# hbell99/DirectVoxGO

Measured on AMD Instinct MI355X. Metric: train rays/sec (8192-ray batch, 160^3 grid), higher is better.
Workload: dtype f32

## Files before the change

### directvoxgo_amd/_lib.py

```python
import ctypes
import os
import re

import torch

_HERE = os.path.dirname(os.path.abspath(__file__))
SO_PATH = os.environ.get('DVGO_HIP_SO') or os.path.join(_HERE, 'csrc', 'libdvgo_hip.so')
ABI_VERSION = 11
HEADER_PATH = os.path.join(os.path.dirname(_HERE), 'include', 'dvgo_hip.h')

_lib = None
_nargs = {}


class _Rec2(ctypes.Structure):
    _fields_ = [('step', ctypes.c_int32), ('exp_d', ctypes.c_float), ('alpha', ctypes.c_float), ('T', ctypes.c_float)]


_vp = ctypes.c_void_p
_i64 = ctypes.c_int64
_int = ctypes.c_int
_flt = ctypes.c_float


class _Pointer(ctypes.c_void_p):

    @staticmethod
    def from_param(x):
        if x is None or type(x) is _vp:
            return x
        if isinstance(x, torch.Tensor):
            return _vp(x.data_ptr())
        if isinstance(x, (ctypes.Array, _vp)):
            return x
        raise TypeError(f'expected a tensor, a ctypes array, a c_void_p or None, got {type(x).__name__}')


_SCALARS = {'int': ctypes.c_int, 'int32_t': ctypes.c_int32, 'int64_t': ctypes.c_int64, 'float': ctypes.c_float,
            'double': ctypes.c_double}


def declarations(text):
    text = re.sub(r'/\*.*?\*/', ' ', text, flags=re.S)
    text = re.sub(r'^\s*#.*$', ' ', text, flags=re.M)
    text = re.sub(r'typedef\s+struct\s*\{[^{}]*\}\s*\w+\s*;', ' ', text)
    text = re.sub(r'extern\s+"C"\s*\{|^\s*\}\s*$', ' ', text, flags=re.M)
    decls = {}
    for stmt in filter(None, (' '.join(s.split()) for s in text.split(';'))):
        m = re.fullmatch(r'(int|int64_t) (dvgo_\w+) ?\((.*)\)', stmt)
        if m is None or m.group(2) in decls:
            raise RuntimeError(f'dvgo_hip.h: cannot read the declaration `{stmt}`')
        argtypes = []
        for param in ([] if m.group(3).strip() == 'void' else m.group(3).split(',')):
            if re.fullmatch(r'\s*(const )?(unsigned )?\w+ ?\*( ?const ?\*)? ?\w+\s*', param):
                argtypes.append(_Pointer)
                continue
            words = param.split()
            if len(words) != 2 or words[0] not in _SCALARS or not words[1].isidentifier():
                raise RuntimeError(f'dvgo_hip.h: {m.group(2)}: cannot read the parameter `{param.strip()}`')
            argtypes.append(_SCALARS[words[0]])
        decls[m.group(2)] = (_SCALARS[m.group(1)], argtypes)
    return decls


def lib():
    global _lib
    if _lib is None:
        if not os.path.exists(SO_PATH):
            raise RuntimeError(
                f'{SO_PATH} is missing: build it with `python -m directvoxgo_amd.build` '
                '(hipcc --offload-arch=gfx950).  directvoxgo_amd has no CPU fallback.')
        if not os.path.exists(HEADER_PATH):
            raise RuntimeError(f'{HEADER_PATH} is missing: the calls into libdvgo_hip.so are typed from it '
                               '(run from a checkout: include/ beside directvoxgo_amd/)')
        handle = ctypes.CDLL(SO_PATH)
        handle.dvgo_abi_version.restype = ctypes.c_int
        v = handle.dvgo_abi_version()
        if v != ABI_VERSION:
            raise RuntimeError(f'libdvgo_hip.so ABI {v} != expected {ABI_VERSION}: rebuild')
        with open(HEADER_PATH) as f:
            decls = declarations(f.read())
        for name, (restype, argtypes) in decls.items():
            fn = getattr(handle, name, None)
            if fn is None:
                raise RuntimeError(f'{SO_PATH} does not export {name}, which include/dvgo_hip.h declares: rebuild')
            fn.restype, fn.argtypes = restype, argtypes
            _nargs[name] = len(argtypes)
        if os.environ.get('DVGO_SHADE_VARIANT'):
            handle.dvgo_shade_variant(int(os.environ['DVGO_SHADE_VARIANT']))
        _lib = handle
    return _lib


def check_input(x, name):
    if not x.is_cuda:
        raise RuntimeError(f'{name} must be a CUDA tensor')
    if not x.is_contiguous():
        raise RuntimeError(f'{name} must be contiguous')


def check_f32(x, name):
    if x.dtype != torch.float32:
        raise RuntimeError(f'{name} must be float32, got {x.dtype}')


def ptr(t):
    return _vp(t.data_ptr()) if t is not None else _vp(0)


def stream_of(t):
    return _vp(torch._C._cuda_getCurrentRawStream(t.device.index))


class _NoCtx:
    def __enter__(self):
        return self

    def __exit__(self, *exc):
        return False


_NOCTX = _NoCtx()


def device_of(t):
    if t.device.index == torch.cuda.current_device():
        return _NOCTX
    return torch.cuda.device_of(t)


_ERR = {-1: 'invalid argument', -2: 'size exceeds 32-bit launch range'}


_profile = None


def profile_start(names):
    global _profile
    _profile = {n: [] for n in names}


def profile_stop():
    global _profile
    prof, _profile = _profile, None
    torch.cuda.synchronize()
    return {n: (len(ev), sum(a.elapsed_time(b) for a, b in ev)) for n, ev in (prof or {}).items()}


def call(name, *args):
    handle = lib()
    if len(args) != _nargs.get(name):
        raise TypeError(f'{name}: {len(args)} arguments given, include/dvgo_hip.h declares {_nargs.get(name, "no such function")}')
    fn = getattr(handle, name)
    if _profile is not None and name in _profile:
        a, b = torch.cuda.Event(enable_timing=True), torch.cuda.Event(enable_timing=True)
        a.record()
        rc = fn(*args)
        b.record()
        _profile[name].append((a, b))
    else:
        rc = fn(*args)
    if rc != 0:
        raise RuntimeError(f'{name} failed: {_ERR.get(rc, "hipError %d" % rc)}')


def f3(x):
    if isinstance(x, torch.Tensor):
        x = x.detach().cpu().tolist()
    return (ctypes.c_float * 3)(*[float(v) for v in x])
```

### directvoxgo_amd/csrc/loss.hip

```cpp
#include "common.h"

__device__ __forceinline__ float block_sum_256(float v, float* red) {
#pragma unroll
  for (int d = 32; d >= 1; d >>= 1) v += __shfl_xor(v, d);
  const int lane = threadIdx.x & 63, w = threadIdx.x >> 6;
  if (lane == 0) red[w] = v;
  __syncthreads();
  const float t = red[0] + red[1] + red[2] + red[3];
  __syncthreads();
  return t;
}

__global__ void __launch_bounds__(256)
loss_rays_kernel(const float* __restrict__ rgb_marched, const float* __restrict__ alphainv_last,
                 const float* __restrict__ target, int64_t N, float inv_n_global, float w_main, float w_ent,
                 float* __restrict__ g_marched, float* __restrict__ g_last, float* __restrict__ loss_out) {
  __shared__ float red[4];
  const int64_t r = (int64_t)blockIdx.x * blockDim.x + threadIdx.x;
  float l = 0.0f;
  if (r < N) {
    float se = 0.0f;
#pragma unroll
    for (int c = 0; c < 3; ++c) {
      const float d = rgb_marched[3 * r + c] - target[3 * r + c];
      se = fmaf(d, d, se);
      g_marched[3 * r + c] = 2.0f * w_main * d * inv_n_global * (1.0f / 3.0f);
    }
    l = w_main * se * inv_n_global * (1.0f / 3.0f);
    if (w_ent > 0.0f) {
      const float x = alphainv_last[r];
      const float p = fminf(fmaxf(x, 1e-6f), 1.0f - 1e-6f);
      const float lp = logf(p), lq = logf(1.0f - p);
      l += w_ent * (-(p * lp + (1.0f - p) * lq)) * inv_n_global;
      const bool inside = (x >= 1e-6f) && (x <= 1.0f - 1e-6f);
      g_last[r] = inside ? w_ent * (lq - lp) * inv_n_global : 0.0f;
    } else {
      g_last[r] = 0.0f;
    }
  }
  const float t = block_sum_256(l, red);
  if (threadIdx.x == 0) atomicAdd(loss_out, t);
}

__global__ void __launch_bounds__(256)
loss_samples_kernel(const float* __restrict__ raw_rgb, const float* __restrict__ weights,
                    const int64_t* __restrict__ ray_id, const float* __restrict__ target, int64_t M_cap,
                    const int64_t* __restrict__ m_dev,
                    float inv_n_global, float w_per, float* __restrict__ g_raw_rgb, float* __restrict__ loss_out) {
  const int64_t M = m_dev ? (*m_dev < M_cap ? *m_dev : M_cap) : M_cap;
  __shared__ float red[4];
  float l = 0.0f;
  for (int64_t i = (int64_t)blockIdx.x * blockDim.x + threadIdx.x; i < M; i += (int64_t)gridDim.x * blockDim.x) {
    const int64_t r = ray_id[i];
    const float w = weights[i];
    float se = 0.0f;
#pragma unroll
    for (int c = 0; c < 3; ++c) {
      const float d = raw_rgb[3 * i + c] - target[3 * r + c];
      se = fmaf(d, d, se);
      g_raw_rgb[3 * i + c] = 2.0f * w_per * w * d * inv_n_global;
    }
    l += w_per * w * se * inv_n_global;
  }
  const float t = block_sum_256(l, red);
  if (threadIdx.x == 0) atomicAdd(loss_out, t);
}

__global__ void __launch_bounds__(256)
viewdir_embed_kernel(const float* __restrict__ viewdirs, const float* __restrict__ freq, int F, int64_t N,
                     float* __restrict__ emb) {
  const int E = 3 + 6 * F;
  const int64_t t = (int64_t)blockIdx.x * blockDim.x + threadIdx.x;
  if (t >= N * E) return;
  const int64_t r = t / E;
  const int e = (int)(t - r * E);
  float v;
  if (e < 3) v = viewdirs[3 * r + e];
  else {
    const int q = (e - 3) % (3 * F);
    const float a = viewdirs[3 * r + q / F] * freq[q % F];
    v = (e - 3 < 3 * F) ? sinf(a) : cosf(a);
  }
  emb[t] = v;
}

#define DVGO_MT_MAX 16
struct AdamMulti {
  float* p[DVGO_MT_MAX];
  const float* g[DVGO_MT_MAX];
  float* m[DVGO_MT_MAX];
  float* v[DVGO_MT_MAX];
  int64_t start[DVGO_MT_MAX + 1];
  int n;
};
__global__ void __launch_bounds__(256)
adam_multi_kernel(AdamMulti A, float step_size, const float* __restrict__ step_size_dev, float beta1, float beta2, float eps) {
  if (step_size_dev != nullptr) step_size = *step_size_dev;
  const int64_t t = (int64_t)blockIdx.x * blockDim.x + threadIdx.x;
  if (t >= A.start[A.n]) return;
  int k = 0;
  while (k + 1 < A.n && t >= A.start[k + 1]) ++k;
  const int64_t i = t - A.start[k];
  const float g = A.g[k][i];
  const float m = fmaf(beta1, A.m[k][i], (1.0f - beta1) * g);
  const float v = fmaf(beta2, A.v[k][i], ((1.0f - beta2) * g) * g);
  A.m[k][i] = m;
  A.v[k][i] = v;
  A.p[k][i] = A.p[k][i] - (step_size * m) / (sqrtf(v) + eps);
}

struct CopyMulti {
  const uint32_t* src[8];
  uint32_t* dst[8];
  int64_t start[9];
  int n;
};
__global__ void __launch_bounds__(256)
copy_multi_kernel(CopyMulti A) {
  const int64_t t = (int64_t)blockIdx.x * blockDim.x + threadIdx.x;
  if (t >= A.start[A.n]) return;
  int k = 0;
  while (k + 1 < A.n && t >= A.start[k + 1]) ++k;
  const int64_t i = t - A.start[k];
  A.dst[k][i] = A.src[k][i];
}

extern "C" {

int dvgo_copy_multi(void* const* dst, const void* const* src, const int64_t* n_dwords, int n_tensors, void* stream) {
  if (n_tensors < 0 || n_tensors > 8 || (n_tensors > 0 && (!dst || !src || !n_dwords))) return DVGO_EINVAL;
  CopyMulti A;
  A.n = n_tensors;
  int64_t tot = 0;
  for (int k = 0; k < n_tensors; ++k) {
    if (n_dwords[k] < 0 || (n_dwords[k] > 0 && (!dst[k] || !src[k]))) return DVGO_EINVAL;
    A.dst[k] = (uint32_t*)dst[k]; A.src[k] = (const uint32_t*)src[k];
    A.start[k] = tot;
    tot += n_dwords[k];
  }
  for (int k = n_tensors; k <= 8; ++k) A.start[k] = tot;
  if (tot == 0) return 0;
  if (!dvgo_fits(tot)) return DVGO_ERANGE;
  copy_multi_kernel<<<dvgo_blocks(tot, 256), 256, 0, (hipStream_t)stream>>>(A);
  DVGO_LAUNCH_CHECK();
  return 0;
}

int dvgo_loss_fwd_bwd(const float* rgb_marched, const float* alphainv_last, const float* target, int64_t N,
                      const float* raw_rgb, const float* weights, const int64_t* ray_id, int64_t M, const int64_t* m_dev,
                      int64_t n_rays_global, float w_main, float w_ent, float w_per, float* g_marched,
                      float* g_last, float* g_raw_rgb, float* loss_out, void* stream) {
  if (N < 0 || M < 0 || n_rays_global <= 0) return DVGO_EINVAL;
  if (!loss_out) return DVGO_EINVAL;
  hipStream_t s = (hipStream_t)stream;
  DVGO_HIP_TRY(hipMemsetAsync(loss_out, 0, sizeof(float), s));
  const float inv = 1.0f / (float)n_rays_global;
  if (N > 0) {
    if (!rgb_marched || !alphainv_last || !target || !g_marched || !g_last) return DVGO_EINVAL;
    loss_rays_kernel<<<dvgo_blocks(N, 256), 256, 0, s>>>(rgb_marched, alphainv_last, target, N, inv, w_main, w_ent,
                                                         g_marched, g_last, loss_out);
    DVGO_LAUNCH_CHECK();
  }
  if (M > 0 && w_per > 0.0f) {
    if (!raw_rgb || !weights || !ray_id || !g_raw_rgb) return DVGO_EINVAL;
    const int64_t nb = dvgo_blocks(M, 256);
    loss_samples_kernel<<<(int)(nb < 256 ? nb : (M >= (1 << 20) ? 1024 : 256)), 256, 0, s>>>(raw_rgb, weights, ray_id, target, M, m_dev, inv, w_per,
                                                            g_raw_rgb, loss_out);
    DVGO_LAUNCH_CHECK();
  }
  return 0;
}

int dvgo_viewdir_embed(const float* viewdirs, const float* freq, int n_freq, int64_t N, float* emb, void* stream) {
  if (N < 0 || n_freq < 0) return DVGO_EINVAL;
  if (N == 0) return 0;
  if (!viewdirs || !emb || (n_freq > 0 && !freq)) return DVGO_EINVAL;
  const int64_t total = N * (3 + 6 * n_freq);
  if (!dvgo_fits(total)) return DVGO_ERANGE;
  viewdir_embed_kernel<<<dvgo_blocks(total, 256), 256, 0, (hipStream_t)stream>>>(viewdirs, freq, n_freq, N, emb);
  DVGO_LAUNCH_CHECK();
  return 0;
}

int dvgo_adam_upd_multi(float* const* params, const float* const* grads, float* const* exp_avg,
                        float* const* exp_avg_sq, const int64_t* numel, int n_tensors, float step_size, float beta1,
                        float beta2, float eps, const float* step_size_dev, void* stream) {
  if (n_tensors < 0 || n_tensors > DVGO_MT_MAX) return DVGO_EINVAL;
  if (n_tensors == 0) return 0;
  if (!params || !grads || !exp_avg || !exp_avg_sq || !numel) return DVGO_EINVAL;
  AdamMulti A;
  A.n = n_tensors;
  int64_t tot = 0;
  for (int k = 0; k < n_tensors; ++k) {
    if (numel[k] < 0 || (numel[k] > 0 && (!params[k] || !grads[k] || !exp_avg[k] || !exp_avg_sq[k]))) return DVGO_EINVAL;
    A.p[k] = params[k]; A.g[k] = grads[k]; A.m[k] = exp_avg[k]; A.v[k] = exp_avg_sq[k];
    A.start[k] = tot;
    tot += numel[k];
  }
  for (int k = n_tensors; k <= DVGO_MT_MAX; ++k) A.start[k] = tot;
  if (tot == 0) return 0;
  adam_multi_kernel<<<dvgo_blocks(tot, 256), 256, 0, (hipStream_t)stream>>>(A, step_size, step_size_dev, beta1, beta2, eps);
  DVGO_LAUNCH_CHECK();
  return 0;
}

}
```

### directvoxgo_amd/csrc/shade.hip

```cpp
#include "common.h"
#include "x3.h"

#include <type_traits>


static int g_shade_experiment = 0;
static int g_shade_variant = 67;
extern "C" int dvgo_shade_wgrad_x3(const float* G1, const float* gz, const uint64_t* masks, const float* W3, const float* H1,
                                   const float* H2, const float* feat, int C, const float* emb, int E, const int64_t* ray_id,
                                   int64_t M, const int64_t* m_dev, int width, int diffuse, int n_parts, float* part, int form_b,
                                   void* stream);
extern "C" int dvgo_shade_bwd_x3(const float* g_rgb, const float* rgb, const uint64_t* masks, int64_t M, const int64_t* m_dev,
                                 const float* W1, const float* W2, const float* W3, int width, int d_in, int C, int diffuse,
                                 float* g_feat, float* G1, float* gz, void* scratch, int prebuilt, void* stream);

extern "C" int dvgo_shade_fwd_x3(const float* feat, int C, const float* emb, int E, const int64_t* ray_id, int64_t M, const int64_t* m_dev,
                                 const float* W1, const float* b1, const float* W2, const float* b2, const float* W3,
                                 const float* b3, int width, int d_in, int diffuse, float* rgb, float* H1, float* H2,
                                 uint64_t* masks, void* scratch, void* scratch_bwd, int experiment, void* stream);

#define SHADE_THREADS 768
#define SHADE_WAVES (SHADE_THREADS / 64)
#define SHADE_BWD_THREADS 1024
#define SHADE_BWD_WAVES (SHADE_BWD_THREADS / 64)

template <int WIDTH, int S1>
struct ShadeLds {
  static constexpr int T = WIDTH / 32;
  float w1a[T][S1][64];
  float w2a[T][T][16][64];
  float w3p[3][2][T * 16];
  float b1p[2][T * 16];
  float b2p[2][T * 16];
  float b3[4];
};

__device__ __forceinline__ int acc_feature(int t, int r, int h) { return 32 * t + (r & 3) + 8 * (r >> 2) + 4 * h; }

#define SHADE_STAGE_STRIDE 36
__device__ __forceinline__ void shade_store_tile(float* __restrict__ stage ,
                                                 const f32x16& acc, float* __restrict__ dst , int row_stride, int lane, int rows_valid) {
  const int smp = lane & 31, h = lane >> 5;
#pragma unroll
  for (int q = 0; q < 4; ++q)
    *reinterpret_cast<float4*>(stage + smp * SHADE_STAGE_STRIDE + 8 * q + 4 * h) =
        make_float4(acc[4 * q], acc[4 * q + 1], acc[4 * q + 2], acc[4 * q + 3]);
  const int c = lane & 7;
#pragma unroll
  for (int i = 0; i < 4; ++i) {
    const int r = (lane >> 3) + 8 * i;
    const float4 v = *reinterpret_cast<const float4*>(stage + r * SHADE_STAGE_STRIDE + 4 * c);
    if (r < rows_valid) *reinterpret_cast<float4*>(dst + (int64_t)r * row_stride + 4 * c) = v;
  }
}

template <int WIDTH, int S1>
__device__ __forceinline__ void shade_load_weights(ShadeLds<WIDTH, S1>& L, const float* __restrict__ W1,
                                                   const float* __restrict__ b1, const float* __restrict__ W2,
                                                   const float* __restrict__ b2, const float* __restrict__ W3,
                                                   const float* __restrict__ b3, int D_in) {
  constexpr int T = WIDTH / 32;
  const int tid = threadIdx.x, nt = blockDim.x;
  for (int i = tid; i < T * S1 * 64; i += nt) {
    const int l = i & 63, s = (i >> 6) % S1, t = (i >> 6) / S1;
    const int k = 2 * s + (l >> 5);
    (&L.w1a[0][0][0])[i] = (k < D_in) ? W1[(32 * t + (l & 31)) * D_in + k] : 0.0f;
  }
  for (int i = tid; i < T * T * 16 * 64; i += nt) {
    const int l = i & 63, r = (i >> 6) & 15, t = (i >> 10) % T, t2 = (i >> 10) / T;
    (&L.w2a[0][0][0][0])[i] = W2[(32 * t2 + (l & 31)) * WIDTH + acc_feature(t, r, l >> 5)];
  }
  for (int i = tid; i < 3 * 2 * T * 16; i += nt) {
    const int tr = i % (T * 16), h = (i / (T * 16)) & 1, c = i / (2 * T * 16);
    (&L.w3p[0][0][0])[i] = W3[c * WIDTH + acc_feature(tr >> 4, tr & 15, h)];
  }
  for (int i = tid; i < 2 * T * 16; i += nt) {
    const int tr = i % (T * 16), h = i / (T * 16);
    const int f = acc_feature(tr >> 4, tr & 15, h);
    (&L.b1p[0][0])[i] = b1[f];
    (&L.b2p[0][0])[i] = b2[f];
  }
  if (tid < 3) L.b3[tid] = b3[tid];
}

template <int WIDTH, int S1>
__device__ __forceinline__ void shade_tile_forward(const ShadeLds<WIDTH, S1>& L, const float (&x)[S1], int lane,
                                                   f32x16 (&acc1)[WIDTH / 32], float (&z)[3],
                                                   float* __restrict__ H2tile ,
                                                   float* __restrict__ stage, int rows_valid,
                                                   unsigned long long& mask2 ) {
  constexpr int T = WIDTH / 32;
  const int h = lane >> 5;
#pragma unroll
  for (int t = 0; t < T; ++t) {
#pragma unroll
    for (int r = 0; r < 16; ++r) acc1[t][r] = L.b1p[h][t * 16 + r];
#pragma unroll
    for (int s = 0; s < S1; ++s) acc1[t] = __builtin_amdgcn_mfma_f32_32x32x2f32(L.w1a[t][s][lane], x[s], acc1[t], 0, 0, 0);
#pragma unroll
    for (int r = 0; r < 16; ++r) acc1[t][r] = dvgo_relu(acc1[t][r]);
    __builtin_amdgcn_sched_barrier(0);
  }
  float p[3] = {0.0f, 0.0f, 0.0f};
  mask2 = 0ull;
#pragma unroll 1
  for (int t2 = 0; t2 < T; ++t2) {
    f32x16 acc2;
#pragma unroll
    for (int r = 0; r < 16; ++r) acc2[r] = L.b2p[h][t2 * 16 + r];
#pragma unroll
    for (int t = 0; t < T; ++t) {
#pragma unroll
      for (int r = 0; r < 16; ++r)
        acc2 = __builtin_amdgcn_mfma_f32_32x32x2f32(L.w2a[t2][t][r][lane], acc1[t][r], acc2, 0, 0, 0);
      __builtin_amdgcn_sched_barrier(0);
    }
#pragma unroll
    for (int r = 0; r < 16; ++r) acc2[r] = dvgo_relu(acc2[r]);
    if (H2tile != nullptr) {
      unsigned int bits = 0u;
#pragma unroll
      for (int r = 0; r < 16; ++r) bits |= dvgo_relu_bit(acc2[r]) << r;
      mask2 |= (unsigned long long)bits << (16 * t2);
      shade_store_tile(stage, acc2, H2tile + 32 * t2, WIDTH, lane, rows_valid);
    }
#pragma unroll
    for (int c = 0; c < 3; ++c) {
#pragma unroll
      for (int r = 0; r < 16; ++r) p[c] = fmaf(L.w3p[c][h][t2 * 16 + r], acc2[r], p[c]);
    }
  }
#pragma unroll
  for (int c = 0; c < 3; ++c) z[c] = p[c] + __shfl_xor(p[c], 32) + L.b3[c];
}

template <int S1>
__device__ __forceinline__ void shade_load_x(const float* __restrict__ feat, int C, int c_view0, int n_view,
                                             const float* __restrict__ emb, int E, int64_t row, int64_t ray,
                                             int lane, float (&x)[S1]) {
  const int h = lane >> 5;
  const float* fr = feat + row * C + c_view0;
  const float* er = emb + ray * E - n_view;
#pragma unroll
  for (int s = 0; s < S1; ++s) {
    const int k = 2 * s + h;
    float v = 0.0f;
    if (k < n_view) v = fr[k];
    else if (k < n_view + E) v = er[k];
    x[s] = v;
  }
}

template <int WIDTH, int S1, bool DIFFUSE>
__global__ void __launch_bounds__(SHADE_THREADS)
shade_fwd_kernel(const float* __restrict__ feat, int C, int c_view0, int n_view, const float* __restrict__ emb, int E,
                 const int64_t* __restrict__ ray_id, int64_t M_cap, const int64_t* __restrict__ m_dev, const float* __restrict__ W1,
                 const float* __restrict__ b1, const float* __restrict__ W2, const float* __restrict__ b2,
                 const float* __restrict__ W3, const float* __restrict__ b3, int D_in, float* __restrict__ rgb,
                 float* __restrict__ H1, float* __restrict__ H2, unsigned long long* __restrict__ masks, int experiment) {
  const int64_t M = m_dev ? (*m_dev < M_cap ? *m_dev : M_cap) : M_cap;
  constexpr int T = WIDTH / 32;
  __shared__ ShadeLds<WIDTH, S1> L;
  __shared__ __attribute__((aligned(16))) float s_stage[SHADE_WAVES][32 * SHADE_STAGE_STRIDE];
  shade_load_weights<WIDTH, S1>(L, W1, b1, W2, b2, W3, b3, D_in);
  __syncthreads();
  const int lane = threadIdx.x & 63, h = lane >> 5;
  float* stage = s_stage[threadIdx.x >> 6];
  const int64_t n_tiles = (M + 31) / 32;
  const int64_t gw = (int64_t)blockIdx.x * (blockDim.x >> 6) + (threadIdx.x >> 6);
  const int64_t nw = (int64_t)gridDim.x * (blockDim.x >> 6);
  for (int64_t tile = gw; tile < n_tiles; tile += nw) {
    const int64_t row = tile * 32 + (lane & 31);
    const bool valid = row < M;
    const int64_t rowc = valid ? row : (M - 1);
    float x[S1];
    if (experiment & 16) { for (int s = 0; s < S1; ++s) x[s] = 0.01f * (float)(lane + s); }
    else shade_load_x<S1>(feat, C, c_view0, n_view, emb, E, rowc, ray_id[rowc], lane, x);
    f32x16 acc1[T];
    float z[3];
    const int rows_valid = (int)(M - tile * 32 < 32 ? M - tile * 32 : 32);
    unsigned long long mask2;
    shade_tile_forward<WIDTH, S1>(L, x, lane, acc1, z, (H1 != nullptr && !(experiment & 32)) ? (H2 + tile * 32 * WIDTH) : nullptr,
                                  stage, rows_valid, mask2);
    if (valid) {
      if (h == 0) {
#pragma unroll
        for (int c = 0; c < 3; ++c) {
          const float zz = DIFFUSE ? z[c] + feat[row * C + c] : z[c];
          rgb[row * 3 + c] = 1.0f / (1.0f + expf(-zz));
        }
      }
      if (H1 != nullptr) {
        unsigned long long mask1 = 0ull;
#pragma unroll
        for (int t = 0; t < T; ++t) {
#pragma unroll
          for (int r = 0; r < 16; ++r) mask1 |= (unsigned long long)dvgo_relu_bit(acc1[t][r]) << (16 * t + r);
        }
        masks[(row * 2 + 0) * 2 + h] = mask1;
        masks[(row * 2 + 1) * 2 + h] = mask2;
      }
    }
    if (H1 != nullptr && !(experiment & 32)) {
#pragma unroll
      for (int t = 0; t < T; ++t) shade_store_tile(stage, acc1[t], H1 + tile * 32 * WIDTH + 32 * t, WIDTH, lane, rows_valid);
    }
  }
}

template <int WIDTH>
struct ShadeBwdLds {
  static constexpr int T = WIDTH / 32;
  float w2ta[T][T][16][64];
  float w1ta[T][16][64];
  float w3p[3][2][T * 16];
};

template <int WIDTH, bool DIFFUSE>
__global__ void __launch_bounds__(SHADE_BWD_THREADS)
shade_bwd_kernel(const float* __restrict__ g_rgb, const float* __restrict__ rgb,
                 const unsigned long long* __restrict__ masks, int64_t M_cap, const int64_t* __restrict__ m_dev,
                 const float* __restrict__ W1, const float* __restrict__ W2,
                 const float* __restrict__ W3, int D_in, int C, int c_view0, int n_view,
                 float* __restrict__ g_feat, float* __restrict__ G1, float* __restrict__ gz_out, int experiment) {
  const int64_t M = m_dev ? (*m_dev < M_cap ? *m_dev : M_cap) : M_cap;
  constexpr int T = WIDTH / 32;
  __shared__ ShadeBwdLds<WIDTH> L;
  __shared__ __attribute__((aligned(16))) float s_stage[SHADE_BWD_WAVES][32 * SHADE_STAGE_STRIDE];
  float* stage = s_stage[threadIdx.x >> 6];
  {
    const int tid = threadIdx.x, nt = blockDim.x;
    for (int i = tid; i < T * T * 16 * 64; i += nt) {
      const int l = i & 63, r = (i >> 6) & 15, t2 = (i >> 10) % T, tin = (i >> 10) / T;
      (&L.w2ta[0][0][0][0])[i] = W2[acc_feature(t2, r, l >> 5) * WIDTH + 32 * tin + (l & 31)];
    }
    for (int i = tid; i < T * 16 * 64; i += nt) {
      const int l = i & 63, r = (i >> 6) & 15, t = i >> 10;
      const int k = l & 31;
      (&L.w1ta[0][0][0])[i] = (k < D_in) ? W1[acc_feature(t, r, l >> 5) * D_in + k] : 0.0f;
    }
    for (int i = tid; i < 3 * 2 * T * 16; i += nt) {
      const int tr = i % (T * 16), h = (i / (T * 16)) & 1, c = i / (2 * T * 16);
      (&L.w3p[0][0][0])[i] = W3[c * WIDTH + acc_feature(tr >> 4, tr & 15, h)];
    }
  }
  __syncthreads();
  const int lane = threadIdx.x & 63, h = lane >> 5;
  const int64_t n_tiles = (M + 31) / 32;
  const int64_t gw = (int64_t)blockIdx.x * (blockDim.x >> 6) + (threadIdx.x >> 6);
  const int64_t nw = (int64_t)gridDim.x * (blockDim.x >> 6);
  for (int64_t tile = gw; tile < n_tiles; tile += nw) {
    const int64_t row = tile * 32 + (lane & 31);
    const bool valid = row < M;
    const int64_t rowc = valid ? row : (M - 1);
    float gz[3];
#pragma unroll
    for (int c = 0; c < 3; ++c) {
      const float o = rgb[rowc * 3 + c];
      gz[c] = valid ? g_rgb[rowc * 3 + c] * o * (1.0f - o) : 0.0f;
    }
    if (valid && h == 0) {
#pragma unroll
      for (int c = 0; c < 3; ++c) {
        gz_out[row * 3 + c] = gz[c];
        if (DIFFUSE) g_feat[row * C + c] = gz[c];
      }
    }
    const unsigned long long m1 = masks[(rowc * 2 + 0) * 2 + h];
    const unsigned long long m2 = masks[(rowc * 2 + 1) * 2 + h];
    f32x16 g2[T];
#pragma unroll
    for (int t2 = 0; t2 < T; ++t2) {
#pragma unroll
      for (int r = 0; r < 16; ++r) {
        const float v = fmaf(L.w3p[2][h][t2 * 16 + r], gz[2],
                             fmaf(L.w3p[1][h][t2 * 16 + r], gz[1], L.w3p[0][h][t2 * 16 + r] * gz[0]));
        g2[t2][r] = ((m2 >> (16 * t2 + r)) & 1ull) ? v : 0.0f;
      }
    }
    f32x16 gx;
#pragma unroll
    for (int r = 0; r < 16; ++r) gx[r] = 0.0f;
#pragma unroll 1
    for (int tin = 0; tin < T; ++tin) {
      f32x16 acc;
#pragma unroll
      for (int r = 0; r < 16; ++r) acc[r] = 0.0f;
#pragma unroll
      for (int t2 = 0; t2 < T; ++t2) {
#pragma unroll
        for (int r = 0; r < 16; ++r)
          acc = __builtin_amdgcn_mfma_f32_32x32x2f32(L.w2ta[tin][t2][r][lane], g2[t2][r], acc, 0, 0, 0);
        __builtin_amdgcn_sched_barrier(0);
      }
#pragma unroll
      for (int q = 0; q < 4; ++q) {
        const unsigned int mb = (unsigned int)(m1 >> (16 * tin + 4 * q)) & 15u;
        acc[4 * q + 0] = (mb & 1u) ? acc[4 * q + 0] : 0.0f;
        acc[4 * q + 1] = (mb & 2u) ? acc[4 * q + 1] : 0.0f;
        acc[4 * q + 2] = (mb & 4u) ? acc[4 * q + 2] : 0.0f;
        acc[4 * q + 3] = (mb & 8u) ? acc[4 * q + 3] : 0.0f;
      }
      if (!(experiment & 1))
        shade_store_tile(stage, acc, G1 + tile * 32 * WIDTH + 32 * tin, WIDTH, lane,
                         (int)(M - tile * 32 < 32 ? M - tile * 32 : 32));
#pragma unroll
      for (int r = 0; r < 16; ++r)
        gx = __builtin_amdgcn_mfma_f32_32x32x2f32(L.w1ta[tin][r][lane], acc[r], gx, 0, 0, 0);
    }
    if (valid) {
#pragma unroll
      for (int r = 0; r < 16; ++r) {
        const int k = (r & 3) + 8 * (r >> 2) + 4 * h;
        if (k < n_view) g_feat[row * C + c_view0 + k] = gx[r];
      }
    }
  }
}

template <int WIDTH>
struct ShadeWgradLds {
  float g1[1][32][WIDTH], h1[1][32][WIDTH], h2[1][32][WIDTH];
// ... 440 lines not shown
}
template <int OFF> __device__ __forceinline__ void lds_store_u32x4(unsigned a, u32x4 v) {
  asm volatile("ds_write_b128 %0, %1 offset:%2" :: "v"(a), "v"(v), "n"(OFF) : "memory");
}

template <int WIDTH>
struct ShadeWgradRingX3 : ShadeWgradRing<WIDTH> {
  u32x4 fb[WIDTH / 32 + 2][3][64];
};

template <int WIDTH>
__global__ void __launch_bounds__(2 * WIDTH, 2)
shade_wgrad_ring_x3_kernel(const float* __restrict__ G1, const float* __restrict__ gz, const unsigned int* __restrict__ masks,
                           const float* __restrict__ W3, const float* __restrict__ H1, const float* __restrict__ H2,
                           const float* __restrict__ feat, int C, int c_view0, int n_view, const float* __restrict__ emb, int E,
                           const int64_t* __restrict__ ray_id, int64_t M_cap, const int64_t* __restrict__ m_dev,
                           float* __restrict__ part, float* __restrict__ total, int total_size) {
#if defined(__HIP_DEVICE_COMPILE__)
  for (int i = blockIdx.x * blockDim.x + threadIdx.x; i < total_size; i += gridDim.x * blockDim.x) total[i] = 0.0f;
  int64_t M;
  {
    const int64_t m = m_dev ? (*m_dev < M_cap ? *m_dev : M_cap) : M_cap;
    M = ((int64_t)__builtin_amdgcn_readfirstlane((int)(m >> 32)) << 32) | (unsigned)__builtin_amdgcn_readfirstlane((int)m);
  }
  using Ring = ShadeWgradRingX3<WIDTH>;
  constexpr int T = WIDTH / 32, NW = T, NB = Ring::NB, NR = Ring::NR, TR = Ring::TR;
  static_assert(T == 4 || T == 2, "widths 128 and 64");
  constexpr int LPR = WIDTH / 4, RPI = 64 / LPR, IPW = TR / RPI / NW;
  constexpr int DW = NW == 4 ? 2 : NW, FPW = 4 / DW, EPW = 8 / DW;
  static_assert(IPW == 2 && NB == 2 && TR == 16, "double buffer of 16-row tiles: the wait at the top of a tile is vmcnt(0)");
  __shared__ __attribute__((aligned(16))) Ring L;
  const int tid = threadIdx.x, lane = tid & 63, h = lane >> 5, j = lane & 31;
  const int w = __builtin_amdgcn_readfirstlane(tid >> 6);
  const int dw = NW == 4 ? w - 2 : w;
  f32x16 aW2[T], aW1[2];
  float vW3[3] = {0.0f, 0.0f, 0.0f}, sgz[3] = {0.0f, 0.0f, 0.0f};
#pragma unroll
  for (int t = 0; t < T; ++t)
#pragma unroll
    for (int r = 0; r < 16; ++r) aW2[t][r] = 0.0f;
#pragma unroll
  for (int q = 0; q < 2; ++q)
#pragma unroll
    for (int r = 0; r < 16; ++r) aW1[q][r] = 0.0f;
  float sb1 = 0.0f, sb2 = 0.0f;
  const float w30 = W3[32 * w + j], w31 = W3[WIDTH + 32 * w + j], w32 = W3[2 * WIDTH + 32 * w + j];
  const int m_idx = 2 * ((j >> 2) & 1) + (w >> 1);
  const unsigned m_bit = 16 * (w & 1) + (j & 3) + 4 * (j >> 3);
  const int d_in = n_view + E;
  const int n_tiles = (int)((M + TR - 1) / TR);
  auto tile_of = [&](int k) { return (int)blockIdx.x + k * (int)gridDim.x; };
  const unsigned rows_b = (unsigned)(M * WIDTH * 4);
  const auto bG1 = __builtin_amdgcn_make_buffer_rsrc((void*)G1, 0, rows_b, 0x00020000);
  const auto bH1 = __builtin_amdgcn_make_buffer_rsrc((void*)H1, 0, rows_b, 0x00020000);
  const auto bH2 = __builtin_amdgcn_make_buffer_rsrc((void*)H2, 0, rows_b, 0x00020000);
  const auto bF = __builtin_amdgcn_make_buffer_rsrc((void*)feat, 0, (unsigned)(M * C * 4), 0x00020000);
  const auto bE = __builtin_amdgcn_make_buffer_rsrc((void*)emb, 0, DVGO_OOB, 0x00020000);
  const auto bGz = __builtin_amdgcn_make_buffer_rsrc((void*)gz, 0, (unsigned)(M * 12), 0x00020000);
  const auto bM = __builtin_amdgcn_make_buffer_rsrc((void*)masks, 0, (unsigned)(M * 32), 0x00020000);
  const auto bR = __builtin_amdgcn_make_buffer_rsrc((void*)ray_id, 0, (unsigned)(M * 8), 0x00020000);
  unsigned vo_bulk[IPW], vo_f[FPW], vo_ecol[EPW];
  int e_row[EPW];
#pragma unroll
  for (int i = 0; i < IPW; ++i) vo_bulk[i] = (unsigned)(((IPW * w + i) * RPI + lane / LPR) * WIDTH * 4 + 16 * (lane % LPR));
#pragma unroll
  for (int i = 0; i < FPW; ++i) {
    const int e = 64 * ((dw < 0 ? 0 : dw) + DW * i) + lane, row = e >> 4, col = e & 15;
    vo_f[i] = col < n_view ? (unsigned)((row * C + c_view0 + col) * 4) : DVGO_OOB;
  }
#pragma unroll
  for (int i = 0; i < EPW; ++i) {
    const int e = 64 * ((dw < 0 ? 0 : dw) + DW * i) + lane, col = e & 31;
    e_row[i] = e >> 5;
    vo_ecol[i] = col < E ? (unsigned)(col * 4) : DVGO_OOB;
  }
  const unsigned vo_gz = (lane & 3) < 3 ? (unsigned)(((lane >> 2) * 3 + (lane & 3)) * 4) : DVGO_OOB;
  const unsigned vo_m2 = (unsigned)(((lane >> 2) * 8 + 4 + (lane & 3)) * 4);
  const unsigned vo_rid = (unsigned)((lane & (TR - 1)) * 8);
  auto issue = [&](int t) {
    const int sl = t & (NB - 1);
    const unsigned r0 = (unsigned)__builtin_amdgcn_readfirstlane(tile_of(t) * TR);
#pragma unroll
    for (int i = 0; i < IPW; ++i) {
      const int rl = (IPW * w + i) * RPI;
      __builtin_amdgcn_raw_ptr_buffer_load_lds(bG1, (dvgo_lptr_t)&L.g1[sl][rl][0], 16, vo_bulk[i], r0 * (WIDTH * 4), 0, 0);
      __builtin_amdgcn_raw_ptr_buffer_load_lds(bH1, (dvgo_lptr_t)&L.h1[sl][rl][0], 16, vo_bulk[i], r0 * (WIDTH * 4), 0, 0);
      __builtin_amdgcn_raw_ptr_buffer_load_lds(bH2, (dvgo_lptr_t)&L.h2[sl][rl][0], 16, vo_bulk[i], r0 * (WIDTH * 4), 0, 0);
    }
    if (dw < 0) return;
#pragma unroll
    for (int i = 0; i < FPW; ++i)
      __builtin_amdgcn_raw_ptr_buffer_load_lds(bF, (dvgo_lptr_t)(&L.xf[sl][0][0] + 64 * (dw + DW * i)), 4, vo_f[i], r0 * (unsigned)(C * 4), 0, 0);
    unsigned rids[EPW];
#pragma unroll
    for (int i = 0; i < EPW; ++i) rids[i] = lds_u32<0>(lds_addr(&L.rid[t & (NR - 1)][e_row[i]]));
    asm volatile("s_waitcnt lgkmcnt(0)" : "+v"(rids[0]), "+v"(rids[1]), "+v"(rids[2]), "+v"(rids[3]));
#pragma unroll
    for (int i = 0; i < EPW; ++i)
      __builtin_amdgcn_raw_ptr_buffer_load_lds(bE, (dvgo_lptr_t)(&L.xe[sl][0][0] + 64 * (dw + DW * i)), 4,
                                               vo_ecol[i] + rids[i] * (unsigned)(E * 4), 0, 0, 0);
    const unsigned rn = (unsigned)__builtin_amdgcn_readfirstlane(tile_of(t + 2) * TR);
    const int rsl = (t + 2) & (NR - 1);
    auto small = [&](int which) {
      if (which == 0) __builtin_amdgcn_raw_ptr_buffer_load_lds(bGz, (dvgo_lptr_t)&L.gz[sl][0][0], 4, vo_gz, r0 * 12u, 0, 0);
      else if (which == 1) __builtin_amdgcn_raw_ptr_buffer_load_lds(bM, (dvgo_lptr_t)&L.m2[sl][0][0], 4, vo_m2, r0 * 32u, 0, 0);
      else __builtin_amdgcn_raw_ptr_buffer_load_lds(bR, (dvgo_lptr_t)&L.rid[rsl][0], 4, vo_rid, rn * 8u, 0, 0);
    };
    if (dw == 0) { small(0); small(1); } else small(2);
  };
  const unsigned a_gz = lds_addr(&L.gz[0][8 * h][0]), a_mw = lds_addr(&L.m2[0][8 * h][m_idx]);
  const unsigned a_g1 = lds_addr(&L.g1[0][8 * h][32 * w + j]), a_h1 = lds_addr(&L.h1[0][8 * h][32 * w + j]);
  const unsigned a_h2 = lds_addr(&L.h2[0][8 * h][32 * w + j]);
  const int xcol = 32 * (w & 1) + j;
  const bool x_in_f = xcol < n_view, x_ok = xcol < d_in;
  const unsigned a_x = x_in_f ? lds_addr(&L.xf[0][8 * h][xcol]) : lds_addr(&L.xe[0][8 * h][x_ok ? xcol - n_view : 0]);
  const unsigned a_fb = lds_addr(&L.fb[0][0][lane]);
  constexpr unsigned SLOT_ROWS = TR * WIDTH * 4, FB_TILE = 3 * 64 * 16, FB_PIECE = 64 * 16;
  if (tid < 64) {
#pragma unroll
    for (int t = 0; t < 2; ++t) {
      const int64_t row = (int64_t)tile_of(t) * TR + (tid & (TR - 1));
      L.rid[t][tid] = row < M ? (unsigned int)ray_id[row] : 0u;
    }
  }
  __syncthreads();
#pragma unroll
  for (int t = 0; t < NB - 1; ++t) issue(t);
  for (int k = 0; tile_of(k) < n_tiles; ++k) {
    const int sl = k & (NB - 1);
    asm volatile("s_waitcnt vmcnt(0)\n\ts_waitcnt lgkmcnt(0)\n\ts_barrier" ::: "memory");
    issue(k + NB - 1);
    const unsigned b_gz = a_gz + sl * (TR * 16), b_mw = a_mw + sl * (TR * 16), b_g1 = a_g1 + sl * SLOT_ROWS;
    const unsigned b_h1 = a_h1 + sl * SLOT_ROWS, b_h2 = a_h2 + sl * SLOT_ROWS;
    const unsigned b_x = a_x + sl * (x_in_f ? (unsigned)(TR * 16 * 4) : (unsigned)(TR * 32 * 4));
    dvgo_f32x4 gq[8];
    unsigned mw[8];
    float g1v[8], h1v[8], h2v[8], xv[8];
    constexpr int RS = WIDTH * 4 / 256;
    static_for<0, 4>([&](auto Ec) {
      constexpr int e = 2 * decltype(Ec)::value;
      const dvgo_f32x2 v = lds_f32_pair_st64<e * RS, (e + 1) * RS>(b_h1);
      h1v[e] = v.x; h1v[e + 1] = v.y;
    });
    if (w < 2) {
      if (x_in_f) static_for<0, 8>([&](auto Ec) { constexpr int e = decltype(Ec)::value; xv[e] = lds_f32<e * 16 * 4>(b_x); });
      else static_for<0, 8>([&](auto Ec) { constexpr int e = decltype(Ec)::value; xv[e] = lds_f32<e * 32 * 4>(b_x); });
    }
    static_for<0, 8>([&](auto Ec) {
      constexpr int e = decltype(Ec)::value;
      gq[e] = lds_f32x4<16 * e>(b_gz);
    });
    static_for<0, 4>([&](auto Ec) {
      constexpr int e = 2 * decltype(Ec)::value;
      const dvgo_f32x2 m = lds_f32_pair<4 * e, 4 * (e + 1)>(b_mw);
      mw[e] = __float_as_uint(m.x); mw[e + 1] = __float_as_uint(m.y);
      const dvgo_f32x2 a = lds_f32_pair_st64<e * RS, (e + 1) * RS>(b_g1);
      g1v[e] = a.x; g1v[e + 1] = a.y;
      const dvgo_f32x2 b = lds_f32_pair_st64<e * RS, (e + 1) * RS>(b_h2);
      h2v[e] = b.x; h2v[e + 1] = b.y;
    });
    asm volatile("s_waitcnt lgkmcnt(0)" : "+v"(h1v[0]), "+v"(h1v[1]), "+v"(h1v[2]), "+v"(h1v[3]), "+v"(h1v[4]), "+v"(h1v[5]),
                 "+v"(h1v[6]), "+v"(h1v[7]), "+v"(gq[0]), "+v"(gq[1]), "+v"(gq[2]), "+v"(gq[3]), "+v"(gq[4]), "+v"(gq[5]), "+v"(gq[6]),
                 "+v"(gq[7]));
    asm volatile("" : "+v"(mw[0]), "+v"(mw[1]), "+v"(mw[2]), "+v"(mw[3]), "+v"(mw[4]), "+v"(mw[5]), "+v"(mw[6]), "+v"(mw[7]),
                 "+v"(g1v[0]), "+v"(g1v[1]), "+v"(g1v[2]), "+v"(g1v[3]), "+v"(g1v[4]), "+v"(g1v[5]), "+v"(g1v[6]), "+v"(g1v[7]));
    asm volatile("" : "+v"(h2v[0]), "+v"(h2v[1]), "+v"(h2v[2]), "+v"(h2v[3]), "+v"(h2v[4]), "+v"(h2v[5]), "+v"(h2v[6]), "+v"(h2v[7]));
    {
      u32x4 p0, p1, p2;
      x3_split8(h1v, p0, p1, p2);
      lds_store_u32x4<0>(a_fb + w * FB_TILE, p0);
      lds_store_u32x4<FB_PIECE>(a_fb + w * FB_TILE, p1);
      lds_store_u32x4<2 * FB_PIECE>(a_fb + w * FB_TILE, p2);
      if (w < 2) {
        asm volatile("" : "+v"(xv[0]), "+v"(xv[1]), "+v"(xv[2]), "+v"(xv[3]), "+v"(xv[4]), "+v"(xv[5]), "+v"(xv[6]), "+v"(xv[7]));
#pragma unroll
        for (int e = 0; e < 8; ++e) xv[e] = x_ok ? xv[e] : 0.0f;
        x3_split8(xv, p0, p1, p2);
        lds_store_u32x4<0>(a_fb + (T + w) * FB_TILE, p0);
        lds_store_u32x4<FB_PIECE>(a_fb + (T + w) * FB_TILE, p1);
        lds_store_u32x4<2 * FB_PIECE>(a_fb + (T + w) * FB_TILE, p2);
      }
    }
    u32x4 a2f[3], a1f[3];
    {
      float a2[8];
#pragma unroll
      for (int e = 0; e < 8; ++e) {
        const float g2v = fmaf(w32, gq[e].z, fmaf(w31, gq[e].y, w30 * gq[e].x));
        a2[e] = __uint_as_float(__float_as_uint(g2v) & (unsigned)__builtin_amdgcn_sbfe((int)mw[e], m_bit, 1u));
        sb2 += a2[e]; sb1 += g1v[e];
        vW3[0] = fmaf(gq[e].x, h2v[e], vW3[0]); vW3[1] = fmaf(gq[e].y, h2v[e], vW3[1]); vW3[2] = fmaf(gq[e].z, h2v[e], vW3[2]);
      }
      if (w == 0) {
#pragma unroll
        for (int e = 0; e < 8; ++e) { sgz[0] += gq[e].x; sgz[1] += gq[e].y; sgz[2] += gq[e].z; }
      }
      x3_split8(a2, a2f[0], a2f[1], a2f[2]);
      x3_split8(g1v, a1f[0], a1f[1], a1f[2]);
    }
    asm volatile("s_waitcnt lgkmcnt(0)\n\ts_barrier" ::: "memory");
    u32x4 fr[2][2][3];
    auto read_pair = [&](auto Pc, u32x4 (&f)[2][3]) {
      constexpr int p = decltype(Pc)::value;
#pragma unroll
      for (int q = 0; q < 3; ++q) {
        f[0][q] = lds_u32x4<(2 * p) * FB_TILE>(a_fb + q * FB_PIECE);
        f[1][q] = lds_u32x4<(2 * p + 1) * FB_TILE>(a_fb + q * FB_PIECE);
      }
    };
    auto wait_pair = [&](u32x4 (&f)[2][3]) {
      asm volatile("s_waitcnt lgkmcnt(0)" : "+v"(f[0][0]), "+v"(f[0][1]), "+v"(f[0][2]), "+v"(f[1][0]), "+v"(f[1][1]), "+v"(f[1][2]));
    };
    auto mfma_pair = [&](f32x16& accA, f32x16& accB, const u32x4 (&a)[3], const u32x4 (&f)[2][3]) {
#define X3D_MF(ACC, A, B) ACC = __builtin_amdgcn_mfma_f32_32x32x16_bf16(__builtin_bit_cast(bf16x8, A), __builtin_bit_cast(bf16x8, B), ACC, 0, 0, 0)
      X3D_MF(accA, a[2], f[0][0]); X3D_MF(accB, a[2], f[1][0]);
      X3D_MF(accA, a[1], f[0][1]); X3D_MF(accB, a[1], f[1][1]);
      X3D_MF(accA, a[0], f[0][2]); X3D_MF(accB, a[0], f[1][2]);
      X3D_MF(accA, a[1], f[0][0]); X3D_MF(accB, a[1], f[1][0]);
      X3D_MF(accA, a[0], f[0][1]); X3D_MF(accB, a[0], f[1][1]);
      X3D_MF(accA, a[0], f[0][0]); X3D_MF(accB, a[0], f[1][0]);
#undef X3D_MF
    };
    constexpr int NP = T / 2 + 1;
    read_pair(std::integral_constant<int, 0>{}, fr[0]);
    static_for<0, NP>([&](auto Pc) {
      constexpr int p = decltype(Pc)::value;
      wait_pair(fr[p & 1]);
      if constexpr (p + 1 < NP) read_pair(std::integral_constant<int, p + 1>{}, fr[(p + 1) & 1]);
      if constexpr (p < T / 2) mfma_pair(aW2[2 * p], aW2[2 * p + 1], a2f, fr[p & 1]);
      else mfma_pair(aW1[0], aW1[1], a1f, fr[p & 1]);
      __builtin_amdgcn_sched_barrier(0);
    });
  }
  asm volatile("s_waitcnt vmcnt(0)" ::: "memory");
  float* p = part + (int64_t)blockIdx.x * (WIDTH * WIDTH + WIDTH * 64 + 32 * WIDTH + 3 * WIDTH);
  float* pW2 = p;
  float* pW1 = pW2 + WIDTH * WIDTH;
  float* pW3 = pW1 + WIDTH * 64;
  float* pb = pW3 + 32 * WIDTH;
#pragma unroll
  for (int r = 0; r < 16; ++r) {
    const int i = (r & 3) + 8 * (r >> 2) + 4 * h;
#pragma unroll
    for (int t = 0; t < T; ++t) pW2[(32 * w + i) * WIDTH + 32 * t + j] = aW2[t][r];
    pW1[(32 * w + i) * 64 + j] = aW1[0][r];
    pW1[(32 * w + i) * 64 + 32 + j] = aW1[1][r];
  }
#pragma unroll
  for (int c = 0; c < 3; ++c) {
    const float v = vW3[c] + __shfl_xor(vW3[c], 32);
    if (h == 0) pW3[c * WIDTH + 32 * w + j] = v;
    sgz[c] += __shfl_xor(sgz[c], 32);
  }
  sb1 += __shfl_xor(sb1, 32); sb2 += __shfl_xor(sb2, 32);
  if (h == 0) {
    pb[32 * w + j] = sb1;
    pb[WIDTH + 32 * w + j] = sb2;
    if (j < 8) pb[2 * WIDTH + 8 * w + j] = (w == 0 && j < 3) ? sgz[j] : 0.0f;
    if (T == 2 && j >= 16) pb[2 * WIDTH + 16 * w + j] = 0.0f;
  }
#endif
}
#undef DVGO_OOB

#define SHADE_REDUCE_SLICES 16
__global__ void __launch_bounds__(256)
shade_wgrad_reduce_kernel(const float* __restrict__ part, int n_parts, int n, int W, int d_in, float* __restrict__ out) {
  const int i = blockIdx.x * blockDim.x + threadIdx.x;
  if (i >= n) return;
  int o;
  const int nW2 = W * W, nW1 = W * 64, nW3 = 32 * W;
  if (i < nW2) o = i;
  else if (i < nW2 + nW1) {
    const int r = (i - nW2) >> 6, c = (i - nW2) & 63;
    o = c < d_in ? nW2 + r * d_in + c : -1;
  } else if (i < nW2 + nW1 + nW3) {
    const int e = i - nW2 - nW1;
    o = e < 3 * W ? nW2 + W * d_in + e : -1;
  } else {
    const int e = i - nW2 - nW1 - nW3, base = nW2 + W * d_in + 3 * W;
    if (e < 2 * W) o = base + e;
    else {
      const int c = e - 2 * W;
      o = c < 3 ? base + 2 * W + c : (c >= 8 && c < 11) ? base + 2 * W + c - 8 : -1;
    }
  }
  if (o < 0) return;
  const int per = (n_parts + SHADE_REDUCE_SLICES - 1) / SHADE_REDUCE_SLICES;
  const int p0 = blockIdx.y * per, p1 = min(n_parts, p0 + per);
  float a0 = 0.0f, a1 = 0.0f, a2 = 0.0f, a3 = 0.0f;
  int p = p0;
  for (; p + 4 <= p1; p += 4) {
    a0 += part[(int64_t)p * n + i];
    a1 += part[(int64_t)(p + 1) * n + i];
    a2 += part[(int64_t)(p + 2) * n + i];
    a3 += part[(int64_t)(p + 3) * n + i];
  }
  for (; p < p1; ++p) a0 += part[(int64_t)p * n + i];
  if (p1 > p0) atomicAdd(out + o, (a0 + a1) + (a2 + a3));
}

extern "C" {

int dvgo_shade_fwd(const float* feat, int C, const float* emb, int E, const int64_t* ray_id, int64_t M, const int64_t* m_dev,
                   const float* W1, const float* b1, const float* W2, const float* b2, const float* W3,
                   const float* b3, int width, int d_in, int diffuse, float* rgb, float* H1, float* H2,
                   uint64_t* masks, void* scratch, void* scratch_bwd, void* stream) {
  if (M < 0 || C <= 0 || E < 0) return DVGO_EINVAL;
  if (M == 0) return 0;
  if (!feat || !emb || !ray_id || !W1 || !b1 || !W2 || !b2 || !W3 || !b3 || !rgb) return DVGO_EINVAL;
  if ((H1 == nullptr) != (H2 == nullptr) || (H1 == nullptr) != (masks == nullptr)) return DVGO_EINVAL;
  const int c_view0 = diffuse ? 3 : 0;
  const int n_view = C - c_view0;
  if (n_view < 0 || d_in != n_view + E) return DVGO_EINVAL;
  if ((width != 128 && width != 64) || d_in > 40) return DVGO_ERANGE;
  if ((g_shade_variant & 1) && scratch != nullptr)
    return dvgo_shade_fwd_x3(feat, C, emb, E, ray_id, M, m_dev, W1, b1, W2, b2, W3, b3, width, d_in, diffuse, rgb, H1, H2, masks,
                             scratch, (g_shade_variant & 2) ? scratch_bwd : nullptr, g_shade_experiment, stream);
  hipStream_t s = (hipStream_t)stream;
  const int64_t n_tiles = (M + 31) / 32;
  const int64_t cap = width == 128 ? 256 : 512;
  int blocks = (int)((n_tiles + SHADE_WAVES - 1) / SHADE_WAVES < cap ? (n_tiles + SHADE_WAVES - 1) / SHADE_WAVES : cap);
#define DVGO_SHADE(W, S1, DIFF)                                                                           \
  shade_fwd_kernel<W, S1, DIFF><<<blocks, SHADE_THREADS, 0, s>>>(feat, C, c_view0, n_view, emb, E, ray_id, M, m_dev, W1, b1, W2, \
                                                          b2, W3, b3, d_in, rgb, H1, H2, (unsigned long long*)masks, g_shade_experiment)
  if (width == 128) {
    if (d_in <= 36) { if (diffuse) DVGO_SHADE(128, 18, true); else DVGO_SHADE(128, 18, false); }
    else            { if (diffuse) DVGO_SHADE(128, 20, true); else DVGO_SHADE(128, 20, false); }
  } else {
    if (d_in <= 12) { if (diffuse) DVGO_SHADE(64, 6, true); else DVGO_SHADE(64, 6, false); }
    else            { if (diffuse) DVGO_SHADE(64, 20, true); else DVGO_SHADE(64, 20, false); }
  }
#undef DVGO_SHADE
  DVGO_LAUNCH_CHECK();
  return 0;
}

int dvgo_shade_experiment(int flags) { g_shade_experiment = flags; return 0; }

int dvgo_shade_variant(int flags) { const int old = g_shade_variant; if (flags >= 0) g_shade_variant = flags; return old; }

int dvgo_shade_bwd(const float* g_rgb, const float* rgb, const uint64_t* masks, int64_t M, const int64_t* m_dev,
                   const float* W1, const float* W2, const float* W3, int width, int d_in, int C, int diffuse,
                   float* g_feat, float* G1, float* gz, void* scratch, int prebuilt, void* stream) {
  if (M < 0 || C <= 0) return DVGO_EINVAL;
  if (M == 0) return 0;
  if (!g_rgb || !rgb || !masks || !W1 || !W2 || !W3 || !g_feat || !G1 || !gz) return DVGO_EINVAL;
  const int c_view0 = diffuse ? 3 : 0;
  const int n_view = C - c_view0;
  if ((width != 128 && width != 64) || n_view < 0 || n_view > 32 || d_in < n_view) return DVGO_ERANGE;
  if ((g_shade_variant & 2) && scratch != nullptr)
    return dvgo_shade_bwd_x3(g_rgb, rgb, masks, M, m_dev, W1, W2, W3, width, d_in, C, diffuse, g_feat, G1, gz, scratch, prebuilt, stream);
  hipStream_t s = (hipStream_t)stream;
  const int64_t n_tiles = (M + 31) / 32;
  const int64_t cap = width == 128 ? 256 : 512;
  int blocks = (int)((n_tiles + SHADE_BWD_WAVES - 1) / SHADE_BWD_WAVES < cap ? (n_tiles + SHADE_BWD_WAVES - 1) / SHADE_BWD_WAVES : cap);
#define DVGO_SHADE_BWD(W, DIFF)                                                                                                       \
  shade_bwd_kernel<W, DIFF><<<blocks, SHADE_BWD_THREADS, 0, s>>>(g_rgb, rgb, (const unsigned long long*)masks, M, m_dev, W1, W2, W3, d_in, C, c_view0, \
                                                            n_view, g_feat, G1, gz, g_shade_experiment)
  if (width == 128) { if (diffuse) DVGO_SHADE_BWD(128, true); else DVGO_SHADE_BWD(128, false); }
  else              { if (diffuse) DVGO_SHADE_BWD(64, true); else DVGO_SHADE_BWD(64, false); }
#undef DVGO_SHADE_BWD
  DVGO_LAUNCH_CHECK();
  return 0;
}

int dvgo_shade_wgrad(const float* G1, const float* gz, const uint64_t* masks, const float* W3, const float* H1,
                     const float* H2, const float* feat, int C, const float* emb, int E, const int64_t* ray_id, int64_t M,
                     const int64_t* m_dev, int width, int diffuse, int n_parts, float* part, float* total, void* stream) {
  if (M < 0 || n_parts <= 0 || C <= 0 || E < 0) return DVGO_EINVAL;
  if (!G1 || !gz || !masks || !W3 || !H1 || !H2 || !feat || !emb || !ray_id || !part || !total) return DVGO_EINVAL;
  const int c_view0 = diffuse ? 3 : 0;
  const int n_view = C - c_view0;
  if ((width != 128 && width != 64) || n_view < 0 || n_view + E > 40) return DVGO_ERANGE;
  bool ring = false;
  if (g_shade_variant & (4 | 32)) {
    const int form_b = (g_shade_variant & 32) ? 2 : (g_shade_variant & 16) ? 1 : 0;
    if (!form_b && n_parts > 256) n_parts = 256;
    const int rc = dvgo_shade_wgrad_x3(G1, gz, masks, W3, H1, H2, feat, C, emb, E, ray_id, M, m_dev, width, diffuse, n_parts, part,
                                       form_b, stream);
    if (rc != 0) return rc;
  } else if (!(g_shade_variant & 8) && n_view <= 16 && E <= 32 && (n_view + E <= 32 || (n_view % 4 == 0 && n_view >= 8)) &&
             M * width * 4 < ((int64_t)1 << 31) && M * C * 4 < ((int64_t)1 << 31)) {
    if (n_parts > 512) n_parts = 512;
    ring = true;
    const int tsz = width * width + width * (n_view + E) + 5 * width + 3;
    if ((g_shade_variant & 64) && width == 128)
      shade_wgrad_ring_x3_kernel<128><<<n_parts, 256, 0, (hipStream_t)stream>>>(
          G1, gz, (const unsigned int*)masks, W3, H1, H2, feat, C, c_view0, n_view, emb, E, ray_id, M, m_dev, part, total, tsz);
    else if (g_shade_variant & 64)
      shade_wgrad_ring_x3_kernel<64><<<n_parts, 128, 0, (hipStream_t)stream>>>(
          G1, gz, (const unsigned int*)masks, W3, H1, H2, feat, C, c_view0, n_view, emb, E, ray_id, M, m_dev, part, total, tsz);
    else if (width == 128)
      shade_wgrad_ring_kernel<128><<<n_parts, 256, 0, (hipStream_t)stream>>>(
          G1, gz, (const unsigned int*)masks, W3, H1, H2, feat, C, c_view0, n_view, emb, E, ray_id, M, m_dev, part, total, tsz);
    else
      shade_wgrad_ring_kernel<64><<<n_parts, 128, 0, (hipStream_t)stream>>>(
          G1, gz, (const unsigned int*)masks, W3, H1, H2, feat, C, c_view0, n_view, emb, E, ray_id, M, m_dev, part, total, tsz);
  } else if (width == 128)
    shade_wgrad_kernel<128><<<n_parts, 256, 0, (hipStream_t)stream>>>(
        G1, gz, (const unsigned int*)masks, W3, H1, H2, feat, C, c_view0, n_view, emb, E, ray_id, M, m_dev, part);
  else
    shade_wgrad_kernel<64><<<n_parts, 128, 0, (hipStream_t)stream>>>(
        G1, gz, (const unsigned int*)masks, W3, H1, H2, feat, C, c_view0, n_view, emb, E, ray_id, M, m_dev, part);
  DVGO_LAUNCH_CHECK();
  const int psize = width * width + width * 64 + 32 * width + 3 * width;
  const int d_in = n_view + E;
  const int tsize = width * width + width * d_in + 3 * width + 2 * width + 3;
  if (!ring && hipMemsetAsync(total, 0, (size_t)tsize * sizeof(float), (hipStream_t)stream) != hipSuccess) return DVGO_EINVAL;
  shade_wgrad_reduce_kernel<<<dim3((psize + 255) / 256, SHADE_REDUCE_SLICES), 256, 0, (hipStream_t)stream>>>(part, n_parts, psize,
                                                                                                       width, d_in, total);
  DVGO_LAUNCH_CHECK();
  return 0;
}

}
```

### directvoxgo_amd/csrc/shade_x3.hip

```cpp
#include "common.h"
#include "x3.h"

#ifndef X3_THREADS
#define X3_THREADS 512
#endif
#define X3_WAVES (X3_THREADS / 64)
#ifndef X3_BWD_THREADS
#define X3_BWD_THREADS 512
#endif
#define X3_BWD_WAVES (X3_BWD_THREADS / 64)
#define X3_STAGE_ROWS 16
#define X3_STAGE_STRIDE 36

__device__ __forceinline__ int x3_acc_feature(int t, int r, int h) { return 32 * t + (r & 3) + 8 * (r >> 2) + 4 * h; }

__device__ __forceinline__ void x3_split1(float v, unsigned short& s0, unsigned short& s1, unsigned short& s2) {
  const unsigned int h = x3_pack(v, 0.f) & 0xffffu;
  const float r = v - __uint_as_float(h << 16);
  const unsigned int m = x3_pack(r, 0.f) & 0xffffu;
  const float q = r - __uint_as_float(m << 16);
  s0 = (unsigned short)h; s1 = (unsigned short)m; s2 = (unsigned short)(x3_pack(q, 0.f) & 0xffffu);
}

template <int WIDTH, int KS1>
struct X3Img {
  static constexpr int T = WIDTH / 32;
  u32x4 w1s[T][KS1][3][64];
  u32x4 w2s[T][2 * T][3][64];
  float w3p[3][2][T * 16];
  float b1p[2][T * 16];
  float b2p[2][T * 16];
  float b3[4];
};

template <int WIDTH, int KS1>
struct X3Lds : X3Img<WIDTH, KS1> {
  float stage[X3_WAVES][X3_STAGE_ROWS * X3_STAGE_STRIDE];
};

template <typename Img>
__device__ __forceinline__ void x3_copy_image(Img* __restrict__ dst , const void* __restrict__ src) {
  static_assert(sizeof(Img) % 16 == 0, "16-byte pieces");
  const u32x4* g = reinterpret_cast<const u32x4*>(src);
  u32x4* l = reinterpret_cast<u32x4*>(dst);
  for (int i = threadIdx.x; i < (int)(sizeof(Img) / 16); i += blockDim.x) l[i] = g[i];
}

__device__ __forceinline__ void x3_store_tile(float* __restrict__ stage, const f32x16& acc, float* __restrict__ dst, int row_stride,
                                              int lane, int rows_valid) {
  const int smp = lane & 31, h = lane >> 5;
#pragma unroll
  for (int half = 0; half < 2; ++half) {
    if ((smp >> 4) == half) {
#pragma unroll
      for (int q = 0; q < 4; ++q)
        *reinterpret_cast<float4*>(stage + (smp & 15) * X3_STAGE_STRIDE + 8 * q + 4 * h) =
            make_float4(acc[4 * q], acc[4 * q + 1], acc[4 * q + 2], acc[4 * q + 3]);
    }
    const int c = lane & 7;
#pragma unroll
    for (int i = 0; i < 2; ++i) {
      const int rl = (lane >> 3) + 8 * i;
      const float4 v = *reinterpret_cast<const float4*>(stage + rl * X3_STAGE_STRIDE + 4 * c);
      const int r = 16 * half + rl;
      if (r < rows_valid) *reinterpret_cast<float4*>(dst + (int64_t)r * row_stride + 4 * c) = v;
    }
  }
}

template <int WIDTH, int KS1>
__device__ __forceinline__ void
x3_prep_fwd_body(X3Img<WIDTH, KS1>* __restrict__ Lp, const float* __restrict__ W1, const float* __restrict__ b1,
                 const float* __restrict__ W2, const float* __restrict__ b2, const float* __restrict__ W3,
                 const float* __restrict__ b3, int D_in, const int tid, const int nt) {
  constexpr int T = WIDTH / 32;
  X3Img<WIDTH, KS1>& L = *Lp;
  for (int i = tid; i < T * KS1 * 64 * 8; i += nt) {
    const int j = i & 7, l = (i >> 3) & 63, s = (i >> 9) % KS1, t = (i >> 9) / KS1;
    const int k = 16 * s + 8 * (l >> 5) + j;
    const float v = (k < D_in) ? W1[(32 * t + (l & 31)) * D_in + k] : 0.0f;
    unsigned short p0, p1, p2;
    x3_split1(v, p0, p1, p2);
    reinterpret_cast<unsigned short*>(&L.w1s[t][s][0][l])[j] = p0;
    reinterpret_cast<unsigned short*>(&L.w1s[t][s][1][l])[j] = p1;
    reinterpret_cast<unsigned short*>(&L.w1s[t][s][2][l])[j] = p2;
  }
  for (int i = tid; i < T * 2 * T * 64 * 8; i += nt) {
    const int j = i & 7, l = (i >> 3) & 63, ks = (i >> 9) % (2 * T), t2 = (i >> 9) / (2 * T);
    const int k = 16 * ks + 8 * (j >> 2) + 4 * (l >> 5) + (j & 3);
    const float v = W2[(32 * t2 + (l & 31)) * WIDTH + k];
    unsigned short p0, p1, p2;
    x3_split1(v, p0, p1, p2);
    reinterpret_cast<unsigned short*>(&L.w2s[t2][ks][0][l])[j] = p0;
    reinterpret_cast<unsigned short*>(&L.w2s[t2][ks][1][l])[j] = p1;
    reinterpret_cast<unsigned short*>(&L.w2s[t2][ks][2][l])[j] = p2;
  }
  for (int i = tid; i < 3 * 2 * T * 16; i += nt) {
    const int tr = i % (T * 16), h = (i / (T * 16)) & 1, c = i / (2 * T * 16);
    (&L.w3p[0][0][0])[i] = W3[c * WIDTH + x3_acc_feature(tr >> 4, tr & 15, h)];
  }
  for (int i = tid; i < 2 * T * 16; i += nt) {
    const int tr = i % (T * 16), h = i / (T * 16);
    const int f = x3_acc_feature(tr >> 4, tr & 15, h);
    (&L.b1p[0][0])[i] = b1[f];
    (&L.b2p[0][0])[i] = b2[f];
  }
  if (tid < 4) L.b3[tid] = tid < 3 ? b3[tid] : 0.0f;
}

template <int WIDTH, int KS1, bool DIFFUSE>
__global__ void __launch_bounds__(X3_THREADS)
shade_fwd_x3_kernel(const float* __restrict__ feat, int C, int c_view0, int n_view, const float* __restrict__ emb, int E,
                    const int64_t* __restrict__ ray_id, int64_t M_cap, const int64_t* __restrict__ m_dev,
                    const void* __restrict__ image, float* __restrict__ rgb,
                    float* __restrict__ H1, float* __restrict__ H2, unsigned long long* __restrict__ masks, int experiment) {
  const int64_t M = m_dev ? (*m_dev < M_cap ? *m_dev : M_cap) : M_cap;
  constexpr int T = WIDTH / 32;
  __shared__ __attribute__((aligned(16))) X3Lds<WIDTH, KS1> L;
  x3_copy_image<X3Img<WIDTH, KS1>>(&L, image);
  __syncthreads();
  const int lane = threadIdx.x & 63, h = lane >> 5;
  float* stage = L.stage[threadIdx.x >> 6];
  const bool train = H1 != nullptr;
  const int64_t n_tiles = (M + 31) / 32;
  const int64_t gw = (int64_t)blockIdx.x * (blockDim.x >> 6) + (threadIdx.x >> 6);
  const int64_t nw = (int64_t)gridDim.x * (blockDim.x >> 6);
  const int d_in = n_view + E;
  const int64_t last = M > 0 ? M - 1 : 0;
  auto row_of = [&](int64_t tile) { const int64_t r = tile * 32 + (lane & 31); return r < M ? r : last; };
  float xin[KS1][8];
  auto load_inputs = [&](int64_t tile, int64_t rid) {
    const float* fr = feat + row_of(tile) * C + c_view0;
    const float* er = emb + rid * E - n_view;
#pragma unroll
    for (int s = 0; s < KS1; ++s)
#pragma unroll
      for (int j = 0; j < 8; ++j) {
        const int k = 16 * s + 8 * h + j;
        const int kc = k < d_in ? k : d_in - 1;
        xin[s][j] = *((kc < n_view) ? fr + kc : er + kc);
      }
  };
  int64_t rid_n = 0;
  if (gw < n_tiles) { load_inputs(gw, ray_id[row_of(gw)]); rid_n = ray_id[row_of(gw + nw)]; }
  for (int64_t tile = gw; tile < n_tiles; tile += nw) {
    const int64_t row = tile * 32 + (lane & 31);
    const bool valid = row < M;
    const int rows_valid = (int)(M - tile * 32 < 32 ? M - tile * 32 : 32);
    u32x4 x3[KS1][3];
#pragma unroll
    for (int s = 0; s < KS1; ++s) {
      float v[8];
#pragma unroll
      for (int j = 0; j < 8; ++j) v[j] = (16 * s + 8 * h + j) < d_in ? xin[s][j] : 0.0f;
      x3_split8(v, x3[s][0], x3[s][1], x3[s][2]);
    }
    load_inputs(tile + nw, rid_n);
    rid_n = ray_id[row_of(tile + 2 * nw)];
    u32x4 h3[2 * T][3];
    unsigned long long mask1 = 0ull;
#pragma unroll
    for (int t = 0; t < T; ++t) {
      f32x16 acc;
#pragma unroll
      for (int r = 0; r < 16; ++r) acc[r] = L.b1p[h][t * 16 + r];
#pragma unroll
      for (int s = 0; s < KS1; ++s)
        x3_mfma6(acc, L.w1s[t][s][0][lane], L.w1s[t][s][1][lane], L.w1s[t][s][2][lane], x3[s][0], x3[s][1], x3[s][2]);
#pragma unroll
      for (int r = 0; r < 16; ++r) acc[r] = dvgo_relu(acc[r]);
      if (train) {
        unsigned int bits = 0u;
#pragma unroll
        for (int r = 0; r < 16; ++r) bits |= dvgo_relu_bit(acc[r]) << r;
        mask1 |= (unsigned long long)bits << (16 * t);
        if (!(experiment & 512)) x3_store_tile(stage, acc, H1 + tile * 32 * WIDTH + 32 * t, WIDTH, lane, rows_valid);
      }
#pragma unroll
      for (int s2 = 0; s2 < 2; ++s2) {
        float v[8];
#pragma unroll
        for (int j = 0; j < 8; ++j) v[j] = acc[8 * s2 + j];
        x3_split8(v, h3[2 * t + s2][0], h3[2 * t + s2][1], h3[2 * t + s2][2]);
      }
      __builtin_amdgcn_sched_barrier(0);
    }
    float p[3] = {0.0f, 0.0f, 0.0f};
    unsigned long long mask2 = 0ull;
#pragma unroll 1
    for (int t2 = 0; t2 < T; ++t2) {
      f32x16 acc2;
#pragma unroll
      for (int r = 0; r < 16; ++r) acc2[r] = L.b2p[h][t2 * 16 + r];
      u32x4 a[2][3];
#pragma unroll
      for (int q = 0; q < 3; ++q) a[0][q] = L.w2s[t2][0][q][lane];
#pragma unroll
      for (int ks = 0; ks < 2 * T; ++ks) {
        if (ks + 1 < 2 * T) {
#pragma unroll
          for (int q = 0; q < 3; ++q) a[(ks + 1) & 1][q] = L.w2s[t2][ks + 1][q][lane];
        }
        x3_mfma6(acc2, a[ks & 1][0], a[ks & 1][1], a[ks & 1][2], h3[ks][0], h3[ks][1], h3[ks][2]);
        __builtin_amdgcn_sched_barrier(0);
      }
#pragma unroll
      for (int r = 0; r < 16; ++r) acc2[r] = dvgo_relu(acc2[r]);
      if (train) {
        unsigned int bits = 0u;
#pragma unroll
        for (int r = 0; r < 16; ++r) bits |= dvgo_relu_bit(acc2[r]) << r;
        mask2 |= (unsigned long long)bits << (16 * t2);
        if (!(experiment & 512)) x3_store_tile(stage, acc2, H2 + tile * 32 * WIDTH + 32 * t2, WIDTH, lane, rows_valid);
      }
#pragma unroll
      for (int c = 0; c < 3; ++c) {
#pragma unroll
        for (int r = 0; r < 16; ++r) p[c] = fmaf(L.w3p[c][h][t2 * 16 + r], acc2[r], p[c]);
      }
    }
    float z[3];
#pragma unroll
    for (int c = 0; c < 3; ++c) z[c] = p[c] + __shfl_xor(p[c], 32) + L.b3[c];
    if (valid) {
      if (h == 0) {
#pragma unroll
        for (int c = 0; c < 3; ++c) {
          const float zz = DIFFUSE ? z[c] + feat[row * C + c] : z[c];
          rgb[row * 3 + c] = 1.0f / (1.0f + expf(-zz));
        }
      }
      if (train) {
        masks[(row * 2 + 0) * 2 + h] = mask1;
        masks[(row * 2 + 1) * 2 + h] = mask2;
      }
    }
  }
}

template <int WIDTH>
struct X3BwdImg {
  static constexpr int T = WIDTH / 32;
  u32x4 w2t[T][2 * T][3][64];
  u32x4 w1t[2 * T][3][64];
  float w3p[3][2][T * 16];
};

template <int WIDTH>
struct X3BwdLds : X3BwdImg<WIDTH> {
  float stage[X3_BWD_WAVES][X3_STAGE_ROWS * X3_STAGE_STRIDE];
};

template <int WIDTH>
__device__ __forceinline__ void
x3_prep_bwd_body(X3BwdImg<WIDTH>* __restrict__ Lp, const float* __restrict__ W1, const float* __restrict__ W2,
                 const float* __restrict__ W3, int D_in, const int tid, const int nt) {
  constexpr int T = WIDTH / 32;
  X3BwdImg<WIDTH>& L = *Lp;
  for (int i = tid; i < T * 2 * T * 64 * 8; i += nt) {
    const int j = i & 7, l = (i >> 3) & 63, ks = (i >> 9) % (2 * T), tin = (i >> 9) / (2 * T);
    const int f_out = 16 * ks + 8 * (j >> 2) + 4 * (l >> 5) + (j & 3);
    unsigned short p0, p1, p2;
    x3_split1(W2[f_out * WIDTH + 32 * tin + (l & 31)], p0, p1, p2);
    reinterpret_cast<unsigned short*>(&L.w2t[tin][ks][0][l])[j] = p0;
    reinterpret_cast<unsigned short*>(&L.w2t[tin][ks][1][l])[j] = p1;
    reinterpret_cast<unsigned short*>(&L.w2t[tin][ks][2][l])[j] = p2;
  }
  for (int i = tid; i < 2 * T * 64 * 8; i += nt) {
    const int j = i & 7, l = (i >> 3) & 63, ks = i >> 9;
    const int f = 16 * ks + 8 * (j >> 2) + 4 * (l >> 5) + (j & 3), k = l & 31;
    unsigned short p0, p1, p2;
    x3_split1((k < D_in) ? W1[f * D_in + k] : 0.0f, p0, p1, p2);
    reinterpret_cast<unsigned short*>(&L.w1t[ks][0][l])[j] = p0;
    reinterpret_cast<unsigned short*>(&L.w1t[ks][1][l])[j] = p1;
    reinterpret_cast<unsigned short*>(&L.w1t[ks][2][l])[j] = p2;
  }
  for (int i = tid; i < 3 * 2 * T * 16; i += nt) {
    const int tr = i % (T * 16), h = (i / (T * 16)) & 1, c = i / (2 * T * 16);
    (&L.w3p[0][0][0])[i] = W3[c * WIDTH + x3_acc_feature(tr >> 4, tr & 15, h)];
  }
}

template <int WIDTH, int KS1>
__global__ void __launch_bounds__(256)
x3_prep_fwd_kernel(X3Img<WIDTH, KS1>* __restrict__ Lp, X3BwdImg<WIDTH>* __restrict__ Lb, const float* __restrict__ W1,
                   const float* __restrict__ b1, const float* __restrict__ W2, const float* __restrict__ b2,
                   const float* __restrict__ W3, const float* __restrict__ b3, int D_in) {
  if (blockIdx.x < 32) x3_prep_fwd_body<WIDTH, KS1>(Lp, W1, b1, W2, b2, W3, b3, D_in, blockIdx.x * blockDim.x + threadIdx.x, 32 * blockDim.x);
  else x3_prep_bwd_body<WIDTH>(Lb, W1, W2, W3, D_in, (blockIdx.x - 32) * blockDim.x + threadIdx.x, 32 * blockDim.x);
}

template <int WIDTH>
__global__ void __launch_bounds__(256)
x3_prep_bwd_kernel(X3BwdImg<WIDTH>* __restrict__ Lp, const float* __restrict__ W1, const float* __restrict__ W2,
                   const float* __restrict__ W3, int D_in) {
  x3_prep_bwd_body<WIDTH>(Lp, W1, W2, W3, D_in, blockIdx.x * blockDim.x + threadIdx.x, gridDim.x * blockDim.x);
}

template <int WIDTH, bool DIFFUSE>
__global__ void __launch_bounds__(X3_BWD_THREADS)
shade_bwd_x3_kernel(const float* __restrict__ g_rgb, const float* __restrict__ rgb,
                    const unsigned long long* __restrict__ masks, int64_t M_cap, const int64_t* __restrict__ m_dev,
                    const void* __restrict__ image, int C, int c_view0,
                    int n_view, float* __restrict__ g_feat, float* __restrict__ G1, float* __restrict__ gz_out) {
  const int64_t M = m_dev ? (*m_dev < M_cap ? *m_dev : M_cap) : M_cap;
  constexpr int T = WIDTH / 32;
  __shared__ __attribute__((aligned(16))) X3BwdLds<WIDTH> L;
  x3_copy_image<X3BwdImg<WIDTH>>(&L, image);
  __syncthreads();
  const int lane = threadIdx.x & 63, h = lane >> 5;
  float* stage = L.stage[threadIdx.x >> 6];
  const int64_t n_tiles = (M + 31) / 32;
  const int64_t gw = (int64_t)blockIdx.x * (blockDim.x >> 6) + (threadIdx.x >> 6);
  const int64_t nw = (int64_t)gridDim.x * (blockDim.x >> 6);
  const int64_t last = M > 0 ? M - 1 : 0;
  float o_n[3], g_n[3];
  unsigned long long m1_n = 0ull, m2_n = 0ull;
  auto load_rows = [&](int64_t tile) {
    const int64_t r = tile * 32 + (lane & 31);
    const int64_t rc = r < M ? r : last;
#pragma unroll
    for (int c = 0; c < 3; ++c) { o_n[c] = rgb[rc * 3 + c]; g_n[c] = g_rgb[rc * 3 + c]; }
    m1_n = masks[(rc * 2 + 0) * 2 + h];
    m2_n = masks[(rc * 2 + 1) * 2 + h];
  };
  if (gw < n_tiles) load_rows(gw);
  for (int64_t tile = gw; tile < n_tiles; tile += nw) {
    const int64_t row = tile * 32 + (lane & 31);
    const bool valid = row < M;
    const int rows_valid = (int)(M - tile * 32 < 32 ? M - tile * 32 : 32);
    float gz[3];
#pragma unroll
    for (int c = 0; c < 3; ++c) gz[c] = valid ? g_n[c] * o_n[c] * (1.0f - o_n[c]) : 0.0f;
    const unsigned long long m1 = m1_n, m2 = m2_n;
    load_rows(tile + nw);
    if (valid && h == 0) {
#pragma unroll
      for (int c = 0; c < 3; ++c) {
        gz_out[row * 3 + c] = gz[c];
        if (DIFFUSE) g_feat[row * C + c] = gz[c];
      }
    }
    u32x4 g3[2 * T][3];
#pragma unroll
    for (int t2 = 0; t2 < T; ++t2) {
#pragma unroll
      for (int s2 = 0; s2 < 2; ++s2) {
        float v[8];
#pragma unroll
        for (int j = 0; j < 8; ++j) {
          const int r = 8 * s2 + j;
          const float w = fmaf(L.w3p[2][h][t2 * 16 + r], gz[2],
                               fmaf(L.w3p[1][h][t2 * 16 + r], gz[1], L.w3p[0][h][t2 * 16 + r] * gz[0]));
          v[j] = ((m2 >> (16 * t2 + r)) & 1ull) ? w : 0.0f;
        }
        x3_split8(v, g3[2 * t2 + s2][0], g3[2 * t2 + s2][1], g3[2 * t2 + s2][2]);
      }
    }
    f32x16 gx;
#pragma unroll
    for (int r = 0; r < 16; ++r) gx[r] = 0.0f;
#pragma unroll 1
    for (int tin = 0; tin < T; ++tin) {
      f32x16 acc;
#pragma unroll
      for (int r = 0; r < 16; ++r) acc[r] = 0.0f;
#pragma unroll
      for (int ks = 0; ks < 2 * T; ++ks) {
        x3_mfma6(acc, L.w2t[tin][ks][0][lane], L.w2t[tin][ks][1][lane], L.w2t[tin][ks][2][lane], g3[ks][0], g3[ks][1], g3[ks][2]);
        if (ks & 1) __builtin_amdgcn_sched_barrier(0);
      }
#pragma unroll
      for (int q = 0; q < 4; ++q) {
        const unsigned int mb = (unsigned int)(m1 >> (16 * tin + 4 * q)) & 15u;
        acc[4 * q + 0] = (mb & 1u) ? acc[4 * q + 0] : 0.0f;
        acc[4 * q + 1] = (mb & 2u) ? acc[4 * q + 1] : 0.0f;
        acc[4 * q + 2] = (mb & 4u) ? acc[4 * q + 2] : 0.0f;
        acc[4 * q + 3] = (mb & 8u) ? acc[4 * q + 3] : 0.0f;
      }
      x3_store_tile(stage, acc, G1 + tile * 32 * WIDTH + 32 * tin, WIDTH, lane, rows_valid);
#pragma unroll
      for (int s2 = 0; s2 < 2; ++s2) {
        float v[8];
#pragma unroll
        for (int j = 0; j < 8; ++j) v[j] = acc[8 * s2 + j];
        u32x4 b0, b1, b2;
        x3_split8(v, b0, b1, b2);
        const int ks = 2 * tin + s2;
        x3_mfma6(gx, L.w1t[ks][0][lane], L.w1t[ks][1][lane], L.w1t[ks][2][lane], b0, b1, b2);
      }
    }
    if (valid) {
#pragma unroll
      for (int r = 0; r < 16; ++r) {
        const int k = (r & 3) + 8 * (r >> 2) + 4 * h;
        if (k < n_view) g_feat[row * C + c_view0 + k] = gx[r];
      }
    }
  }
}

template <int WIDTH>
struct X3WgradLds {
  static constexpr int T = WIDTH / 32;
  float g1[2][32][WIDTH], h1[2][32][WIDTH], h2[2][32][WIDTH];
  float x[2][32][40];
  float gz[2][32][4];
  unsigned int m2[2][32][2][2];
  u32x4 fb[T + 1][2][3][64];
};

typedef const __attribute__((address_space(1))) void* x3_gptr_t;
typedef __attribute__((address_space(3))) void* x3_lptr_t;

template <int WIDTH>
__global__ void __launch_bounds__(WIDTH * 4)
shade_wgrad_x3_kernel(const float* __restrict__ G1, const float* __restrict__ gz, const unsigned int* __restrict__ masks,
                      const float* __restrict__ W3, const float* __restrict__ H1, const float* __restrict__ H2,
                      const float* __restrict__ feat, int C, int c_view0, int n_view, const float* __restrict__ emb, int E,
                      const int64_t* __restrict__ ray_id, int64_t M_cap, const int64_t* __restrict__ m_dev,
                      float* __restrict__ part ) {
  const int64_t M = m_dev ? (*m_dev < M_cap ? *m_dev : M_cap) : M_cap;
  constexpr int T = WIDTH / 32;
  constexpr int NW = 2 * T;
  constexpr int NT = NW * 64;
  constexpr int TPR = NT / 32;
  constexpr int NXI = 40 / TPR > 0 ? (40 + TPR - 1) / TPR : 1;
  constexpr int LPR = WIDTH / 4;
  constexpr int RPI = 64 / LPR;
  constexpr int IPW = 32 / RPI / NW;
  __shared__ __attribute__((aligned(16))) X3WgradLds<WIDTH> L;
  const int tid = threadIdx.x, lane = tid & 63, h = lane >> 5, i = lane & 31, w = tid >> 6;
  const int ot = w >> 1, ks = w & 1;
  f32x16 aW2[T], aW1;
#pragma unroll
  for (int t = 0; t < T; ++t)
#pragma unroll
    for (int r = 0; r < 16; ++r) aW2[t][r] = 0.0f;
#pragma unroll
  for (int r = 0; r < 16; ++r) aW1[r] = 0.0f;
  float vW3[3] = {0.0f, 0.0f, 0.0f}, vW1[8];
#pragma unroll
  for (int kk = 0; kk < 8; ++kk) vW1[kk] = 0.0f;
  float sb1 = 0.0f, sb2 = 0.0f, gz_acc = 0.0f;
  const float w30 = W3[32 * ot + i], w31 = W3[WIDTH + 32 * ot + i], w32 = W3[2 * WIDTH + 32 * ot + i];
  const int m_half = (i >> 2) & 1, m_word = ot >> 1, m_bit = 16 * (ot & 1) + (i & 3) + 4 * (i >> 3);
  const int d_in = n_view + E;
  const int64_t n_tiles = (M + 31) / 32;

  float px[NXI], pgz;
  unsigned int pm2;
  bool pvalid, pgvalid;
  const int xrow = tid / TPR, xcol = tid - xrow * TPR;
  auto issue = [&](int64_t tile, int buf) {
    const int64_t r0 = tile * 32;
    {
      const int64_t row = r0 + xrow;
      const int64_t rc = row < M ? row : M - 1;
      const float* fr = feat + rc * C + c_view0;
      const float* er = emb + ray_id[rc] * E - n_view;
#pragma unroll
      for (int q = 0; q < NXI; ++q) {
        const int k = xcol + TPR * q;
        const int kc = k < d_in ? k : d_in - 1;
        px[q] = *((kc < n_view) ? fr + kc : er + kc);
      }
      pvalid = row < M;
    }
    {
      const int64_t row = r0 + ((tid & 127) >> 2);
      const int64_t rc = row < M ? row : M - 1;
      pgz = gz[rc * 3 + ((tid & 3) < 3 ? (tid & 3) : 0)];
      pgvalid = (tid & 3) < 3 && row < M;
      pm2 = masks[rc * 8 + 4 + (tid & 3)];
    }
#pragma unroll
    for (int q = 0; q < IPW; ++q) {
      const int rl = (IPW * w + q) * RPI;
      const int64_t row = r0 + rl + lane / LPR;
      const int64_t off = (row < M ? row : M - 1) * WIDTH + 4 * (lane % LPR);
      __builtin_amdgcn_global_load_lds((x3_gptr_t)(G1 + off), (x3_lptr_t)&L.g1[buf][rl][0], 16, 0, 0);
      __builtin_amdgcn_global_load_lds((x3_gptr_t)(H1 + off), (x3_lptr_t)&L.h1[buf][rl][0], 16, 0, 0);
      __builtin_amdgcn_global_load_lds((x3_gptr_t)(H2 + off), (x3_lptr_t)&L.h2[buf][rl][0], 16, 0, 0);
    }
  };

  int buf = 0;
// ... 317 lines not shown
  constexpr int T = WIDTH / 32;
  const int lane = threadIdx.x & 63, h = lane >> 5, i = lane & 31;
  const int ot = __builtin_amdgcn_readfirstlane(threadIdx.x >> 6);
  const unsigned int Mu = (unsigned int)M;
  const auto bH1 = __builtin_amdgcn_make_buffer_rsrc((void*)H1, 0, Mu * (WIDTH * 4u), 0x00020000);
  const auto bH2 = __builtin_amdgcn_make_buffer_rsrc((void*)H2, 0, Mu * (WIDTH * 4u), 0x00020000);
  const auto bGz = __builtin_amdgcn_make_buffer_rsrc((void*)gz, 0, Mu * 12u, 0x00020000);
  const auto bM = __builtin_amdgcn_make_buffer_rsrc((void*)masks, 0, Mu * 32u, 0x00020000);
  f32x16 aW2[T];
#pragma unroll
  for (int t = 0; t < T; ++t)
#pragma unroll
    for (int r = 0; r < 16; ++r) aW2[t][r] = 0.0f;
  float vW3[3] = {0.0f, 0.0f, 0.0f}, g3[3] = {0.0f, 0.0f, 0.0f}, sb2 = 0.0f;
  const float w30 = W3[32 * ot + i], w31 = W3[WIDTH + 32 * ot + i], w32 = W3[2 * WIDTH + 32 * ot + i];
  const unsigned int m_bit = 16 * (ot & 1) + (i & 3) + 4 * (i >> 3);
  int vo_h = (8 * h * WIDTH + i) * 4;
  int vo_hw = (8 * h * WIDTH + T * i) * 4;
  int vo_gz = 8 * h * 12;
  int vo_m = (8 * h * 8 + 4 + 2 * ((i >> 2) & 1) + (ot >> 1)) * 4;
  const int n_ks = (int)((M + 15) >> 4);
  float rh1[T][8], rh2[8];
  u32x3 rgz[8];
  unsigned int rm[8];
  auto ld_small = [&](int k) {
#pragma unroll
    for (int e = 0; e < 8; ++e) {
      rgz[e] = __builtin_amdgcn_raw_buffer_load_b96(bGz, vo_gz + e * 12, k * (16 * 12), 0);
      rm[e] = __builtin_amdgcn_raw_buffer_load_b32(bM, vo_m + e * 32, k * (16 * 32), 0);
      rh2[e] = __builtin_bit_cast(float, __builtin_amdgcn_raw_buffer_load_b32(bH2, vo_h + e * (WIDTH * 4), k * (16 * WIDTH * 4) + ot * 128, 0));
    }
  };
  auto ld_h1 = [&](int e, int k) {
    if constexpr (T == 4) {
      const u32x4 v = __builtin_amdgcn_raw_buffer_load_b128(bH1, vo_hw + e * (WIDTH * 4), k * (16 * WIDTH * 4), 0);
#pragma unroll
      for (int t = 0; t < T; ++t) rh1[t][e] = __uint_as_float(v[t]);
    } else {
      const u32x2 v = __builtin_amdgcn_raw_buffer_load_b64(bH1, vo_hw + e * (WIDTH * 4), k * (16 * WIDTH * 4), 0);
#pragma unroll
      for (int t = 0; t < T; ++t) rh1[t][e] = __uint_as_float(v[t]);
    }
  };
  int ks = blockIdx.x;
  if (ks < n_ks) {
    __builtin_amdgcn_sched_barrier(0);
    ld_small(ks);
    __builtin_amdgcn_sched_barrier(0);
#pragma unroll
    for (int e = 0; e < 8; ++e) ld_h1(e, ks);
    __builtin_amdgcn_sched_barrier(0);
  }
  for (; ks < n_ks; ks += gridDim.x) {
    const int kn = ks + (int)gridDim.x < n_ks ? ks + (int)gridDim.x : n_ks - 1;
    asm volatile("" : "+v"(vo_h), "+v"(vo_hw), "+v"(vo_gz), "+v"(vo_m));
    float a2[8];
#pragma unroll
    for (int e = 0; e < 8; ++e) {
      const float g0 = __uint_as_float(rgz[e][0]), g1 = __uint_as_float(rgz[e][1]), g2 = __uint_as_float(rgz[e][2]);
      const float g2v = fmaf(w32, g2, fmaf(w31, g1, w30 * g0));
      a2[e] = __uint_as_float(__float_as_uint(g2v) & (unsigned int)__builtin_amdgcn_sbfe((int)rm[e], m_bit, 1u));
      sb2 += a2[e];
      const float hv = rh2[e];
      vW3[0] = fmaf(g0, hv, vW3[0]); vW3[1] = fmaf(g1, hv, vW3[1]); vW3[2] = fmaf(g2, hv, vW3[2]);
    }
    if (ot == 0) {
      asm volatile("" : "+v"(g3[0]), "+v"(g3[1]), "+v"(g3[2]));
#pragma unroll
      for (int e = 0; e < 8; ++e) {
        g3[0] += __uint_as_float(rgz[e][0]); g3[1] += __uint_as_float(rgz[e][1]); g3[2] += __uint_as_float(rgz[e][2]);
      }
    }
    asm volatile("" : "+v"(a2[0]), "+v"(a2[1]), "+v"(a2[2]), "+v"(a2[3]), "+v"(a2[4]), "+v"(a2[5]), "+v"(a2[6]), "+v"(a2[7]),
                      "+v"(vW3[0]), "+v"(vW3[1]), "+v"(vW3[2]), "+v"(sb2), "+v"(g3[0]), "+v"(g3[1]), "+v"(g3[2]));
    if (!(EXP & 2)) ld_small(kn);
    __builtin_amdgcn_sched_barrier(0);
    u32x4 a2f[3];
    x3_split8(a2, a2f[0], a2f[1], a2f[2]);
    u32x4 bf[2][3];
    {
      float v[8];
#pragma unroll
      for (int e = 0; e < 8; ++e) v[e] = rh1[0][e];
      x3_split8_free(v, bf[0][0], bf[0][1], bf[0][2]);
    }
#pragma unroll
    for (int t = 0; t < T; ++t) {
      if (t + 1 < T) {
        float v[8];
#pragma unroll
        for (int e = 0; e < 8; ++e) v[e] = rh1[t + 1][e];
        if (!(EXP & 4)) x3_split8_free(v, bf[(t + 1) & 1][0], bf[(t + 1) & 1][1], bf[(t + 1) & 1][2]);
        else {
#pragma unroll
          for (int q = 0; q < 3; ++q)
#pragma unroll
            for (int c = 0; c < 4; ++c) bf[(t + 1) & 1][q][c] = __float_as_uint(v[(c + q) & 7]) ^ __float_as_uint(v[c + 4]);
        }
      }
      if (!(EXP & 1)) x3_mfma6(aW2[t], a2f[0], a2f[1], a2f[2], bf[t & 1][0], bf[t & 1][1], bf[t & 1][2]);
      else { aW2[t][0] += __uint_as_float(bf[t & 1][0][0] ^ bf[t & 1][1][1] ^ bf[t & 1][2][2] ^ a2f[0][0] ^ a2f[1][0] ^ a2f[2][0]); }
      if (t + 1 < T) {
#pragma unroll
        for (int g = 0; g < 6; ++g) {
          __builtin_amdgcn_sched_group_barrier(0x008, 1, 0);
          __builtin_amdgcn_sched_group_barrier(0x002, 8, 0);
        }
      }
      __builtin_amdgcn_sched_barrier(0);
      if (t + 2 == T) {
        asm volatile("" : "+v"(bf[(t + 1) & 1][0]), "+v"(bf[(t + 1) & 1][1]), "+v"(bf[(t + 1) & 1][2]));
        if (!(EXP & 2)) {
#pragma unroll
          for (int e = 0; e < 8; ++e) ld_h1(e, kn);
        }
        __builtin_amdgcn_sched_barrier(0);
      }
    }
  }
  float* p = part + (int64_t)blockIdx.x * X3C_PART(WIDTH);
  float* pW2 = p;
  float* pW3 = pW2 + WIDTH * WIDTH + WIDTH * 64;
  float* pb = pW3 + 32 * WIDTH;
#pragma unroll
  for (int r = 0; r < 16; ++r) {
    const int oi = (r & 3) + 8 * (r >> 2) + 4 * h;
#pragma unroll
    for (int t = 0; t < T; ++t) pW2[(32 * ot + oi) * WIDTH + T * i + t] = aW2[t][r];
  }
#pragma unroll
  for (int c = 0; c < 3; ++c) {
    float v = vW3[c];
    v += __shfl_xor(v, 32);
    if (h == 0) pW3[c * WIDTH + 32 * ot + i] = v;
  }
  float s2 = sb2;
  s2 += __shfl_xor(s2, 32);
  if (h == 0) pb[WIDTH + 32 * ot + i] = s2;
  if (ot == 0) {
#pragma unroll
    for (int c = 0; c < 3; ++c) {
      const float v = g3[c] + __shfl_xor(g3[c], 32);
      if (lane == 0) pb[2 * WIDTH + c] = v;
    }
  }
  for (int q = threadIdx.x; q < WIDTH; q += WIDTH * 2)
    if (q >= 3) pb[2 * WIDTH + q] = 0.0f;
#endif
}

template <int WIDTH>
__global__ void __launch_bounds__(256, 2)
shade_wgrad_c1_kernel(const float* __restrict__ G1, const float* __restrict__ feat, int C, int c_view0, int n_view,
                      const float* __restrict__ emb, int E, const int64_t* __restrict__ ray_id, int64_t M_cap,
                      const int64_t* __restrict__ m_dev, float* __restrict__ part) {
#if defined(__HIP_DEVICE_COMPILE__)
  const int64_t M = m_dev ? (*m_dev < M_cap ? *m_dev : M_cap) : M_cap;
  constexpr int T = WIDTH / 32, TA = T / 2;
  __shared__ float red[2][TA * 2 * 16 * 64 + 64 * TA];
  const int lane = threadIdx.x & 63, h = lane >> 5, i = lane & 31;
  const int w = __builtin_amdgcn_readfirstlane(threadIdx.x >> 6);
  const int half = w & 1, grp = w >> 1;
  const unsigned int Mu = (unsigned int)M;
  const auto bG1 = __builtin_amdgcn_make_buffer_rsrc((void*)G1, 0, Mu * (WIDTH * 4u), 0x00020000);
  const auto bF = __builtin_amdgcn_make_buffer_rsrc((void*)feat, 0, Mu * (unsigned int)(C * 4), 0x00020000);
  const auto bE = __builtin_amdgcn_make_buffer_rsrc((void*)emb, 0, 0x80000000u, 0x00020000);
  const auto bR = __builtin_amdgcn_make_buffer_rsrc((void*)ray_id, 0, Mu * 8u, 0x00020000);
  f32x16 aW1[TA][2];
  float sb1[TA];
#pragma unroll
  for (int t = 0; t < TA; ++t) {
    sb1[t] = 0.0f;
#pragma unroll
    for (int q = 0; q < 2; ++q)
#pragma unroll
      for (int r = 0; r < 16; ++r) aW1[t][q][r] = 0.0f;
  }
  const int d_in = n_view + E;
  const bool from_feat = i < n_view;
  const int kf = i < n_view ? i : (n_view > 0 ? n_view - 1 : 0);
  const int ke0 = (i < n_view ? n_view : (i < d_in ? i : d_in - 1)) - n_view;
  const int ke1 = (32 + i < d_in ? 32 + i : d_in - 1) - n_view;
  int vo_g = (8 * h * WIDTH + T * i + TA * half) * 4;
  int vo_f = (8 * h * C + c_view0 + kf) * 4;
  int vo_r = 8 * h * 8;
  const int n_ks = (int)((M + 15) >> 4);
  const int stride = 2 * (int)gridDim.x;
  float rg[TA][8], rf[8], re0[8], re1[8];
  int rid[8];
  auto ld_rid = [&](int k) {
#pragma unroll
    for (int e = 0; e < 8; ++e) rid[e] = __builtin_amdgcn_raw_buffer_load_b32(bR, vo_r + e * 8, k * (16 * 8), 0);
  };
  auto ld_g = [&](int k) {
#pragma unroll
    for (int e = 0; e < 8; ++e) {
      if constexpr (TA == 2) {
        const u32x2 v = __builtin_amdgcn_raw_buffer_load_b64(bG1, vo_g + e * (WIDTH * 4), k * (16 * WIDTH * 4), 0);
        rg[0][e] = __uint_as_float(v[0]); rg[1][e] = __uint_as_float(v[1]);
      } else {
        rg[0][e] = __builtin_bit_cast(float, __builtin_amdgcn_raw_buffer_load_b32(bG1, vo_g + e * (WIDTH * 4), k * (16 * WIDTH * 4), 0));
      }
    }
  };
  auto ld_x = [&](int k) {
#pragma unroll
    for (int e = 0; e < 8; ++e) {
      rf[e] = __builtin_bit_cast(float, __builtin_amdgcn_raw_buffer_load_b32(bF, vo_f + e * (C * 4), k * (16 * C * 4), 0));
      const int vo_e = rid[e] * (E * 4);
      re0[e] = __builtin_bit_cast(float, __builtin_amdgcn_raw_buffer_load_b32(bE, vo_e + ke0 * 4, 0, 0));
      re1[e] = __builtin_bit_cast(float, __builtin_amdgcn_raw_buffer_load_b32(bE, vo_e + ke1 * 4, 0, 0));
    }
  };
  auto clampk = [&](int k) { return k < n_ks ? k : (n_ks > 0 ? n_ks - 1 : 0); };
  int ks = 2 * (int)blockIdx.x + grp;
  if (ks < n_ks) {
    __builtin_amdgcn_sched_barrier(0);
    ld_rid(ks);
    __builtin_amdgcn_sched_barrier(0);
    ld_g(ks);
    __builtin_amdgcn_sched_barrier(0);
    ld_x(ks);
    __builtin_amdgcn_sched_barrier(0);
    ld_rid(clampk(ks + stride));
    __builtin_amdgcn_sched_barrier(0);
  }
  for (; ks < n_ks; ks += stride) {
    const int kn = clampk(ks + stride), kn2 = clampk(ks + 2 * stride);
    asm volatile("" : "+v"(vo_g), "+v"(vo_f), "+v"(vo_r));
    u32x4 af[TA][3];
#pragma unroll
    for (int t = 0; t < TA; ++t) {
      float a1[8];
#pragma unroll
      for (int e = 0; e < 8; ++e) { a1[e] = rg[t][e]; sb1[t] += a1[e]; }
      x3_split8_free(a1, af[t][0], af[t][1], af[t][2]);
    }
    if constexpr (TA == 2)
      asm volatile("" : "+v"(af[0][0]), "+v"(af[0][1]), "+v"(af[0][2]), "+v"(af[1][0]), "+v"(af[1][1]), "+v"(af[1][2]), "+v"(sb1[0]), "+v"(sb1[1]));
    else
      asm volatile("" : "+v"(af[0][0]), "+v"(af[0][1]), "+v"(af[0][2]), "+v"(sb1[0]));
    ld_g(kn);
    __builtin_amdgcn_sched_barrier(0);
    u32x4 b0, b1, b2, c0, c1, c2;
    {
      float x0[8], x1[8];
#pragma unroll
      for (int e = 0; e < 8; ++e) { x0[e] = from_feat ? rf[e] : re0[e]; x1[e] = re1[e]; }
      x3_split8(x0, b0, b1, b2);
      x3_split8(x1, c0, c1, c2);
    }
    asm volatile("" : "+v"(b0), "+v"(b1), "+v"(b2), "+v"(c0), "+v"(c1), "+v"(c2));
    ld_x(kn);
    __builtin_amdgcn_sched_barrier(0);
    ld_rid(kn2);
    __builtin_amdgcn_sched_barrier(0);
#pragma unroll
    for (int t = 0; t < TA; ++t) {
      x3_mfma6(aW1[t][0], af[t][0], af[t][1], af[t][2], b0, b1, b2);
      x3_mfma6(aW1[t][1], af[t][0], af[t][1], af[t][2], c0, c1, c2);
    }
  }
  if (grp == 1) {
#pragma unroll
    for (int t = 0; t < TA; ++t) {
#pragma unroll
      for (int q = 0; q < 2; ++q)
#pragma unroll
        for (int r = 0; r < 16; ++r) red[half][((t * 2 + q) * 16 + r) * 64 + lane] = aW1[t][q][r];
      red[half][TA * 2 * 16 * 64 + 64 * t + lane] = sb1[t];
    }
  }
  __syncthreads();
  if (grp == 0) {
    float* p = part + (int64_t)blockIdx.x * X3C_PART(WIDTH);
    float* pW1 = p + WIDTH * WIDTH;
    float* pb = pW1 + WIDTH * 64 + 32 * WIDTH;
#pragma unroll
    for (int t = 0; t < TA; ++t) {
      const int tile = TA * half + t;
#pragma unroll
      for (int r = 0; r < 16; ++r) {
        const int oi = (r & 3) + 8 * (r >> 2) + 4 * h;
#pragma unroll
        for (int q = 0; q < 2; ++q)
          pW1[(T * oi + tile) * 64 + 32 * q + i] = aW1[t][q][r] + red[half][((t * 2 + q) * 16 + r) * 64 + lane];
      }
      float s1 = sb1[t] + red[half][TA * 2 * 16 * 64 + 64 * t + lane];
      s1 += __shfl_xor(s1, 32);
      if (h == 0) pb[T * i + tile] = s1;
    }
  }
#endif
}

extern "C" {

int64_t dvgo_shade_scratch_bytes(int width) {
  if (width == 128) return (int64_t)sizeof(X3Img<128, 3>) > (int64_t)sizeof(X3BwdImg<128>) ? sizeof(X3Img<128, 3>) : sizeof(X3BwdImg<128>);
  if (width == 64) return (int64_t)sizeof(X3Img<64, 3>) > (int64_t)sizeof(X3BwdImg<64>) ? sizeof(X3Img<64, 3>) : sizeof(X3BwdImg<64>);
  return 0;
}

int dvgo_shade_fwd_x3(const float* feat, int C, const float* emb, int E, const int64_t* ray_id, int64_t M, const int64_t* m_dev,
                      const float* W1, const float* b1, const float* W2, const float* b2, const float* W3,
                      const float* b3, int width, int d_in, int diffuse, float* rgb, float* H1, float* H2,
                      uint64_t* masks, void* scratch, void* scratch_bwd, int experiment, void* stream) {
  if (M < 0 || C <= 0 || E < 0) return DVGO_EINVAL;
  if (M == 0) return 0;
  if (!feat || !emb || !ray_id || !W1 || !b1 || !W2 || !b2 || !W3 || !b3 || !rgb || !scratch) return DVGO_EINVAL;
  if ((H1 == nullptr) != (H2 == nullptr) || (H1 == nullptr) != (masks == nullptr)) return DVGO_EINVAL;
  const int c_view0 = diffuse ? 3 : 0;
  const int n_view = C - c_view0;
  if (n_view < 0 || d_in != n_view + E) return DVGO_EINVAL;
  if ((width != 128 && width != 64) || d_in > 48) return DVGO_ERANGE;
  hipStream_t s = (hipStream_t)stream;
  const int64_t n_tiles = (M + 31) / 32;
  const int64_t cap = 256;
  const int blocks = (int)((n_tiles + X3_WAVES - 1) / X3_WAVES < cap ? (n_tiles + X3_WAVES - 1) / X3_WAVES : cap);
#define DVGO_SHADE_X3(W, KS, DIFF)                                                                                       \
  do {                                                                                                                   \
    x3_prep_fwd_kernel<W, KS><<<scratch_bwd ? 64 : 32, 256, 0, s>>>((X3Img<W, KS>*)scratch, (X3BwdImg<W>*)scratch_bwd, W1, b1, W2, b2, W3, b3, d_in); \
    shade_fwd_x3_kernel<W, KS, DIFF><<<blocks, X3_THREADS, 0, s>>>(feat, C, c_view0, n_view, emb, E, ray_id, M, m_dev, scratch, rgb, \
                                                                    H1, H2, (unsigned long long*)masks, experiment);     \
  } while (0)
  if (width == 128) {
    if (diffuse) DVGO_SHADE_X3(128, 3, true); else DVGO_SHADE_X3(128, 3, false);
  } else {
    if (d_in <= 16) { if (diffuse) DVGO_SHADE_X3(64, 1, true); else DVGO_SHADE_X3(64, 1, false); }
    else            { if (diffuse) DVGO_SHADE_X3(64, 3, true); else DVGO_SHADE_X3(64, 3, false); }
  }
#undef DVGO_SHADE_X3
  DVGO_LAUNCH_CHECK();
  return 0;
}

int dvgo_shade_bwd_x3(const float* g_rgb, const float* rgb, const uint64_t* masks, int64_t M, const int64_t* m_dev,
                      const float* W1, const float* W2, const float* W3, int width, int d_in, int C, int diffuse,
                      float* g_feat, float* G1, float* gz, void* scratch, int prebuilt, void* stream) {
  if (M < 0 || C <= 0) return DVGO_EINVAL;
  if (M == 0) return 0;
  if (!g_rgb || !rgb || !masks || !W1 || !W2 || !W3 || !g_feat || !G1 || !gz || !scratch) return DVGO_EINVAL;
  const int c_view0 = diffuse ? 3 : 0;
  const int n_view = C - c_view0;
  if ((width != 128 && width != 64) || n_view < 0 || n_view > 32 || d_in < n_view) return DVGO_ERANGE;
  hipStream_t s = (hipStream_t)stream;
  const int64_t n_tiles = (M + 31) / 32;
  const int64_t cap = 256;
  const int blocks = (int)((n_tiles + X3_BWD_WAVES - 1) / X3_BWD_WAVES < cap ? (n_tiles + X3_BWD_WAVES - 1) / X3_BWD_WAVES : cap);
#define DVGO_SHADE_BWD_X3(W, DIFF)                                                                                        \
  do {                                                                                                                    \
    if (!prebuilt) x3_prep_bwd_kernel<W><<<32, 256, 0, s>>>((X3BwdImg<W>*)scratch, W1, W2, W3, d_in);                   \
    shade_bwd_x3_kernel<W, DIFF><<<blocks, X3_BWD_THREADS, 0, s>>>(g_rgb, rgb, (const unsigned long long*)masks, M, m_dev, scratch, C, \
                                                                c_view0, n_view, g_feat, G1, gz);                         \
  } while (0)
  if (width == 128) { if (diffuse) DVGO_SHADE_BWD_X3(128, true); else DVGO_SHADE_BWD_X3(128, false); }
  else              { if (diffuse) DVGO_SHADE_BWD_X3(64, true); else DVGO_SHADE_BWD_X3(64, false); }
#undef DVGO_SHADE_BWD_X3
  DVGO_LAUNCH_CHECK();
  return 0;
}

int dvgo_shade_wgrad_x3(const float* G1, const float* gz, const uint64_t* masks, const float* W3, const float* H1,
                        const float* H2, const float* feat, int C, const float* emb, int E, const int64_t* ray_id, int64_t M,
                        const int64_t* m_dev, int width, int diffuse, int n_parts, float* part, int form_b, void* stream) {
  if (M < 0 || n_parts <= 0 || C <= 0 || E < 0) return DVGO_EINVAL;
  if (!G1 || !gz || !masks || !W3 || !H1 || !H2 || !feat || !emb || !ray_id || !part) return DVGO_EINVAL;
  const int c_view0 = diffuse ? 3 : 0;
  const int n_view = C - c_view0;
  if ((width != 128 && width != 64) || n_view < 0 || n_view + E > 40) return DVGO_ERANGE;
  if (form_b == 2) {
    if (M * width * 4 >= ((int64_t)1 << 32) || M * C * 4 >= ((int64_t)1 << 32) || M * 32 >= ((int64_t)1 << 32)) return DVGO_ERANGE;
    if (width == 128) {
      shade_wgrad_c2_kernel<128><<<n_parts, 256, 0, (hipStream_t)stream>>>(gz, (const unsigned int*)masks, W3, H1, H2, M, m_dev, part);
      shade_wgrad_c1_kernel<128><<<n_parts, 256, 0, (hipStream_t)stream>>>(G1, feat, C, c_view0, n_view, emb, E, ray_id, M, m_dev, part);
    } else {
      shade_wgrad_c2_kernel<64><<<n_parts, 128, 0, (hipStream_t)stream>>>(gz, (const unsigned int*)masks, W3, H1, H2, M, m_dev, part);
      shade_wgrad_c1_kernel<64><<<n_parts, 256, 0, (hipStream_t)stream>>>(G1, feat, C, c_view0, n_view, emb, E, ray_id, M, m_dev, part);
    }
  } else if (form_b && width == 128)
    shade_wgrad_x3b_kernel<128><<<n_parts, 256, 0, (hipStream_t)stream>>>(G1, gz, (const unsigned int*)masks, W3, H1, H2, feat, C,
                                                                          c_view0, n_view, emb, E, ray_id, M, m_dev, part);
  else if (form_b)
    shade_wgrad_x3b_kernel<64><<<n_parts, 128, 0, (hipStream_t)stream>>>(G1, gz, (const unsigned int*)masks, W3, H1, H2, feat, C,
                                                                         c_view0, n_view, emb, E, ray_id, M, m_dev, part);
  else if (width == 128)
    shade_wgrad_x3_kernel<128><<<n_parts, 512, 0, (hipStream_t)stream>>>(G1, gz, (const unsigned int*)masks, W3, H1, H2, feat, C,
                                                                         c_view0, n_view, emb, E, ray_id, M, m_dev, part);
  else
    shade_wgrad_x3_kernel<64><<<n_parts, 256, 0, (hipStream_t)stream>>>(G1, gz, (const unsigned int*)masks, W3, H1, H2, feat, C,
                                                                        c_view0, n_view, emb, E, ray_id, M, m_dev, part);
  DVGO_LAUNCH_CHECK();
  return 0;
}

}
```

### directvoxgo_amd/csrc/x3.h

```cpp
#pragma once
#include "common.h"

using f32x16 = __attribute__((ext_vector_type(16))) float;
using bf16x8 = __attribute__((ext_vector_type(8))) __bf16;
using u32x4 = __attribute__((ext_vector_type(4))) unsigned int;

__device__ __forceinline__ unsigned int x3_pack(float a, float b) {
  typedef __attribute__((ext_vector_type(2))) __bf16 bf16x2;
  typedef __attribute__((ext_vector_type(2))) float f32x2;
  f32x2 v; v[0] = a; v[1] = b;
  return __builtin_bit_cast(unsigned int, __builtin_convertvector(v, bf16x2));
}

__device__ __forceinline__ void x3_split8(const float (&v)[8], u32x4& s0, u32x4& s1, u32x4& s2) {
#pragma unroll
  for (int p = 0; p < 4; ++p) {
    const float a = v[2 * p], b = v[2 * p + 1];
    const unsigned int h = x3_pack(a, b);
    const float ra = a - __uint_as_float(h << 16), rb = b - __uint_as_float(h & 0xffff0000u);
    const unsigned int m = x3_pack(ra, rb);
    const float qa = ra - __uint_as_float(m << 16), qb = rb - __uint_as_float(m & 0xffff0000u);
    s0[p] = h; s1[p] = m; s2[p] = x3_pack(qa, qb);
  }
}

__device__ __forceinline__ float x3_sub(float a, float b) {
  float r;
  asm("v_sub_f32 %0, %1, %2" : "=v"(r) : "v"(a), "v"(b));
  return r;
}
__device__ __forceinline__ void x3_split8_free(const float (&v)[8], u32x4& s0, u32x4& s1, u32x4& s2) {
#pragma unroll
  for (int p = 0; p < 4; ++p) {
    const float a = v[2 * p], b = v[2 * p + 1];
    const unsigned int h = x3_pack(a, b);
    const float ra = x3_sub(a, __uint_as_float(h << 16)), rb = x3_sub(b, __uint_as_float(h & 0xffff0000u));
    const unsigned int m = x3_pack(ra, rb);
    const float qa = x3_sub(ra, __uint_as_float(m << 16)), qb = x3_sub(rb, __uint_as_float(m & 0xffff0000u));
    s0[p] = h; s1[p] = m; s2[p] = x3_pack(qa, qb);
  }
}

__device__ __forceinline__ void x3_mfma6(f32x16& acc, const u32x4 a0, const u32x4 a1, const u32x4 a2, const u32x4 b0,
                                         const u32x4 b1, const u32x4 b2) {
#define X3_MF(A, B) acc = __builtin_amdgcn_mfma_f32_32x32x16_bf16(__builtin_bit_cast(bf16x8, A), __builtin_bit_cast(bf16x8, B), acc, 0, 0, 0)
  X3_MF(a2, b0); X3_MF(a1, b1); X3_MF(a0, b2);
  X3_MF(a1, b0); X3_MF(a0, b1);
  X3_MF(a0, b0);
#undef X3_MF
}
```

### directvoxgo_amd/shade.py

```python

import torch
import torch.nn as nn

from . import _lib as L
from ._lib import _i64, _int, ptr, stream_of

N_PARTS = 512


class defer_wgrad:
    _active = None
    _streams = {}

    def __init__(self, side_stream=True):
        self.side_stream = side_stream

    def __enter__(self):
        self.pending = []
        defer_wgrad._active = self
        return self

    def __exit__(self, *exc):
        defer_wgrad._active = None
        return False

    def submit(self, params, fn, device):
        if not self.side_stream:
            self.pending.append((params, fn, None, None))
            return
        side = defer_wgrad._streams.get(device)
        if side is None:
            side = defer_wgrad._streams[device] = torch.cuda.Stream(device=device)
        main = torch.cuda.current_stream(device)
        side.wait_stream(main)
        with torch.cuda.stream(side):
            grads = fn()
            done = torch.cuda.Event()
            done.record(side)
        self.pending.append((params, fn, grads, done))

    @torch.no_grad()
    def flush(self):
        for params, fn, grads, done in self.pending:
            if grads is None:
                grads = fn()
            else:
                torch.cuda.current_stream(grads[0].device).wait_event(done)
            for p, g in zip(params, grads):
                if p.requires_grad:
                    p.grad = g if p.grad is None else p.grad + g
        self.pending = []


@torch.no_grad()
def viewdir_embed(viewdirs, viewfreq):
    N, F = viewdirs.shape[0], viewfreq.shape[0]
    emb = torch.empty((N, 3 + 6 * F), dtype=torch.float32, device=viewdirs.device)
    with L.device_of(viewdirs):
        L.call('dvgo_viewdir_embed', ptr(viewdirs.contiguous()), ptr(viewfreq), _int(F), _i64(N), ptr(emb),
               stream_of(viewdirs))
    return emb


def head_layers(rgbnet):
    layers = head_layers_any_din(rgbnet)
    if layers is None or layers[0].in_features > 40:
        return None
    return layers


def _scratch(width, device):
    lib = L.lib()
    n = int(lib.dvgo_shade_scratch_bytes(int(width)))
    return torch.empty(n, dtype=torch.uint8, device=device) if n > 0 else None


def _unpack_record(tot, width, d_in):
    o = 0
    gW2 = tot[o:o + width * width].view(width, width); o += width * width
    gW1 = tot[o:o + width * d_in].view(width, d_in); o += width * d_in
    gW3 = tot[o:o + 3 * width].view(3, width); o += 3 * width
    gb1, gb2, gb3 = tot[o:o + width], tot[o + width:o + 2 * width], tot[o + 2 * width:o + 2 * width + 3]
    return gW1, gb1, gW2, gb2, gW3, gb3


def _weight_grads(params, wgrad, device, k, n, g_first=None):
    grads = [g_first] + [None] * (n - 1)
    if defer_wgrad._active is not None:
        defer_wgrad._active.submit(params, wgrad, device)
    else:
        grads[k:k + 6] = wgrad()
    return tuple(grads)


class _Shade(torch.autograd.Function):
    @staticmethod
    def forward(ctx, feat, emb, ray_id, W1, b1, W2, b2, W3, b3, diffuse, train, m_dev):
        M, C = feat.shape
        E = emb.shape[1]
        width, d_in = W1.shape
        feat, emb = feat.contiguous(), emb.contiguous()
        train = bool(train) and any(ctx.needs_input_grad)
        rgb = torch.empty((M, 3), dtype=torch.float32, device=feat.device)
        H1 = torch.empty((M, width), dtype=torch.float32, device=feat.device) if train else None
        H2 = torch.empty((M, width), dtype=torch.float32, device=feat.device) if train else None
        masks = torch.empty((M, 4), dtype=torch.int64, device=feat.device) if train else None
        scratch = _scratch(width, feat.device)
        scratch_bwd = _scratch(width, feat.device) if (train and (L.lib().dvgo_shade_variant(-1) & 2)) else None
        with L.device_of(feat):
            L.call('dvgo_shade_fwd', ptr(feat), _int(C), ptr(emb), _int(E), ptr(ray_id), _i64(M), ptr(m_dev), ptr(W1.contiguous()),
                   ptr(b1.contiguous()), ptr(W2.contiguous()), ptr(b2.contiguous()), ptr(W3.contiguous()),
                   ptr(b3.contiguous()), _int(width), _int(d_in), _int(1 if diffuse else 0), ptr(rgb), ptr(H1), ptr(H2),
                   ptr(masks), ptr(scratch), ptr(scratch_bwd), stream_of(feat))
        ctx.scratch_bwd = scratch_bwd if (train and (L.lib().dvgo_shade_variant(-1) & 1)) else None
        if train:
            ctx.save_for_backward(feat, emb, ray_id, W1, W2, W3, rgb, H1, H2, masks)
            ctx.diffuse = diffuse
            ctx.m_dev = m_dev
            ctx.params = (W1, b1, W2, b2, W3, b3)
            ctx.w_versions = (W1._version, W2._version, W3._version)
        return rgb

    @staticmethod
    @torch.autograd.function.once_differentiable
    def backward(ctx, g_rgb):
        feat, emb, ray_id, W1, W2, W3, rgb, H1, H2, masks = ctx.saved_tensors
        diffuse, m_dev = ctx.diffuse, ctx.m_dev
        M, C = feat.shape
        width, d_in = W1.shape
        g_feat = torch.empty_like(feat)
        G1 = torch.empty_like(H1)
        gz = torch.empty_like(rgb)
        prebuilt = ctx.scratch_bwd is not None and W1._version == ctx.w_versions[0] and W2._version == ctx.w_versions[1] \
            and W3._version == ctx.w_versions[2]
        scratch = ctx.scratch_bwd if prebuilt else _scratch(width, feat.device)
        ctx.scratch_bwd = None
        with L.device_of(feat):
            L.call('dvgo_shade_bwd', ptr(g_rgb.contiguous()), ptr(rgb), ptr(masks), _i64(M), ptr(m_dev), ptr(W1.contiguous()),
                   ptr(W2.contiguous()), ptr(W3.contiguous()), _int(width), _int(d_in), _int(C), _int(1 if diffuse else 0),
                   ptr(g_feat), ptr(G1), ptr(gz), ptr(scratch), _int(1 if prebuilt else 0), stream_of(feat))

        def wgrad():
            n_parts = max(1, min(N_PARTS, (M + 255) // 256))
            psize = width * width + width * 64 + 32 * width + 3 * width
            part = torch.empty((n_parts, psize), dtype=torch.float32, device=feat.device)
            tsize = width * width + width * d_in + 5 * width + 3
            tot = torch.empty(tsize, dtype=torch.float32, device=feat.device)
            with L.device_of(feat):
                L.call('dvgo_shade_wgrad', ptr(G1), ptr(gz), ptr(masks), ptr(W3.contiguous()), ptr(H1), ptr(H2), ptr(feat), _int(C), ptr(emb),
                       _int(emb.shape[1]), ptr(ray_id), _i64(M), ptr(m_dev), _int(width), _int(1 if diffuse else 0), _int(n_parts),
                       ptr(part), ptr(tot), stream_of(feat))
            return _unpack_record(tot, width, d_in)

        return _weight_grads(ctx.params, wgrad, feat.device, 3, 12, g_feat if ctx.needs_input_grad[0] else None)


def shade(rgbnet, feat, emb, ray_id, diffuse, m_dev=None):
    layers = head_layers(rgbnet)
    if layers is None or not feat.is_cuda:
        return None
    l1, l2, l3 = layers
    c0 = 3 if diffuse else 0
    if l1.in_features != feat.shape[1] - c0 + emb.shape[1]:
        return None
    return _Shade.apply(feat, emb, ray_id, l1.weight, l1.bias, l2.weight, l2.bias, l3.weight, l3.bias, diffuse,
                        torch.is_grad_enabled(), m_dev)


def posenc_supported(rgbnet, n_freq, emb_dim):
    layers = head_layers_any_din(rgbnet)
    return (layers is not None and layers[0].out_features == 128 and 1 <= n_freq
            and layers[0].in_features == 3 + 6 * n_freq + emb_dim <= 96)


def head_layers_any_din(rgbnet):
    if not isinstance(rgbnet, nn.Sequential) or len(rgbnet) != 4:
        return None
    a, r, mid, c = rgbnet
    if not (isinstance(a, nn.Linear) and isinstance(r, nn.ReLU) and isinstance(c, nn.Linear)):
        return None
    if not (isinstance(mid, nn.Sequential) and len(mid) == 2 and isinstance(mid[0], nn.Linear) and isinstance(mid[1], nn.ReLU)):
        return None
    width = a.out_features
    if width not in (128, 64) or mid[0].in_features != width or mid[0].out_features != width or c.in_features != width \
            or c.out_features != 3:
        return None
    return a, mid[0], c


class _ShadePosenc(torch.autograd.Function):

    @staticmethod
    def forward(ctx, pts, emb, ray_id, freq, W1, b1, W2, b2, W3, b3, train):
        M = pts.shape[0]
        P, E = freq.shape[0], emb.shape[1]
        width, d_in = W1.shape
        pts, emb, freq = pts.contiguous(), emb.contiguous(), freq.contiguous()
        train = bool(train) and any(ctx.needs_input_grad)
        dev = pts.device
        rgb = torch.empty((M, 3), dtype=torch.float32, device=dev)
        H1 = torch.empty((M, width), dtype=torch.float32, device=dev) if train else None
        H2 = torch.empty((M, width), dtype=torch.float32, device=dev) if train else None
        masks = torch.empty((M, 4), dtype=torch.int64, device=dev) if train else None
        with L.device_of(pts):
            L.call('dvgo_shade_pe_fwd', ptr(pts), ptr(freq), _int(P), ptr(emb), _int(E), ptr(ray_id), _i64(M), ptr(W1.contiguous()),
                   ptr(b1.contiguous()), ptr(W2.contiguous()), ptr(b2.contiguous()), ptr(W3.contiguous()), ptr(b3.contiguous()),
                   _int(width), _int(d_in), ptr(rgb), ptr(H1), ptr(H2), ptr(masks), stream_of(pts))
        if train:
            ctx.save_for_backward(pts, emb, ray_id, freq, W2, W3, rgb, H1, H2, masks)
            ctx.params = (W1, b1, W2, b2, W3, b3)
            ctx.d_in = d_in
        return rgb

    @staticmethod
    @torch.autograd.function.once_differentiable
    def backward(ctx, g_rgb):
        pts, emb, ray_id, freq, W2, W3, rgb, H1, H2, masks = ctx.saved_tensors
        M, width, d_in = pts.shape[0], H1.shape[1], ctx.d_in
        G1 = torch.empty_like(H1)
        gz = torch.empty_like(rgb)
        with L.device_of(pts):
            L.call('dvgo_shade_pe_bwd', ptr(g_rgb.contiguous()), ptr(rgb), ptr(masks), _i64(M), ptr(W2.contiguous()),
                   ptr(W3.contiguous()), _int(width), ptr(G1), ptr(gz), stream_of(pts))

        def wgrad():
            rec = int(L.lib().dvgo_shade_pe_record_size(width, d_in))
            n_parts = max(1, min(N_PARTS, (M + 31) // 32))
            part = torch.empty((n_parts, rec), dtype=torch.float32, device=pts.device)
            tot = torch.empty(rec, dtype=torch.float32, device=pts.device)
            with L.device_of(pts):
                L.call('dvgo_shade_pe_wgrad', ptr(G1), ptr(gz), ptr(masks), ptr(W3.contiguous()), ptr(H1), ptr(H2), ptr(pts),
                       ptr(freq), _int(freq.shape[0]), ptr(emb), _int(emb.shape[1]), ptr(ray_id), _i64(M), _int(width),
                       _int(d_in), _int(n_parts), ptr(part), ptr(tot), stream_of(pts))
            return _unpack_record(tot, width, d_in)

        return _weight_grads(ctx.params, wgrad, pts.device, 4, 11)


def shade_posenc(rgbnet, pts, emb, ray_id, posfreq):
    if not pts.is_cuda or not posenc_supported(rgbnet, posfreq.shape[0], emb.shape[1]):
        return None
    l1, l2, l3 = head_layers_any_din(rgbnet)
    return _ShadePosenc.apply(pts, emb, ray_id, posfreq, l1.weight, l1.bias, l2.weight, l2.bias, l3.weight, l3.bias,
                              torch.is_grad_enabled())


@torch.no_grad()
def march_positions(start, dirs, ray_id, step_id, stepdist):
    M = ray_id.shape[0]
    pts = torch.empty((M, 3), dtype=torch.float32, device=start.device)
    with L.device_of(start):
        L.call('dvgo_march_positions', ptr(start), ptr(dirs), ptr(ray_id), ptr(step_id), _i64(M), L._flt(float(stepdist)), ptr(pts),
               stream_of(start))
    return pts
```

### directvoxgo_amd/voxel_model.py

```python
import numpy as np
import torch
import torch.nn as nn
import torch.nn.functional as F

from .fused import composite, composite_depth, fused_march
from .ops import Alphas2Weights, MaskCache, Raw2Alpha, grid_sample, segment_coo, total_variation_add_grad
from .shade import shade, shade_posenc, viewdir_embed


def _as_f32(x):
    return torch.as_tensor(np.asarray(x, dtype=np.float32) if not isinstance(x, torch.Tensor) else x.detach().cpu(),
                           dtype=torch.float32)


class _LinearSplitK(torch.autograd.Function):
    CHUNK = 8192

    @staticmethod
    def forward(ctx, x, weight, bias):
        ctx.save_for_backward(x, weight)
        return torch.addmm(bias, x, weight.t())

    @staticmethod
    def backward(ctx, g):
        x, weight = ctx.saved_tensors
        g = g.contiguous()
        gx = g @ weight if ctx.needs_input_grad[0] else None
        M, chunk = x.shape[0], _LinearSplitK.CHUNK
        main = (M // chunk) * chunk
        gw = None
        if main:
            S = main // chunk
            gw = torch.bmm(g[:main].view(S, chunk, -1).transpose(1, 2), x[:main].view(S, chunk, -1)).sum(0)
        if main < M:
            tail = g[main:].t() @ x[main:]
            gw = tail if gw is None else gw + tail
        return gx, gw, g.sum(0)


def mlp_forward(net, x):
    for mod in net:
        if isinstance(mod, nn.Sequential):
            x = mlp_forward(mod, x)
        elif isinstance(mod, nn.Linear) and x.shape[0] >= 4 * _LinearSplitK.CHUNK and x.requires_grad | mod.weight.requires_grad:
            x = _LinearSplitK.apply(x.contiguous(), mod.weight, mod.bias)
        else:
            x = mod(x)
    return x


def make_rgbnet(dim0, width, depth):
    net = nn.Sequential(
        nn.Linear(dim0, width), nn.ReLU(inplace=True),
        *[nn.Sequential(nn.Linear(width, width), nn.ReLU(inplace=True)) for _ in range(depth - 2)],
        nn.Linear(width, 3))
    nn.init.constant_(net[-1].bias, 0)
    return net


def _freqs(n):
    return torch.FloatTensor([(2 ** i) for i in range(n)])


def _posenc(x, freq):
    emb = (x.unsqueeze(-1) * freq).flatten(-2)
    return torch.cat([x, emb.sin(), emb.cos()], -1)


def _result(alphainv_last, weights, rgb_marched, alpha, rgb, ray_id):
    return {'alphainv_last': alphainv_last, 'weights': weights, 'rgb_marched': rgb_marched,
            'raw_alpha': alpha, 'raw_rgb': rgb, 'ray_id': ray_id}


class VoxelModel(nn.Module):

    rgbnet_direct = True
    uses_posenc = False

    def can_keep_count_on_device(self):
        return False

    def _set_box(self, xyz_min, xyz_max):
        xyz_min, xyz_max = _as_f32(xyz_min), _as_f32(xyz_max)
        self.register_buffer('xyz_min', xyz_min.clone())
        self.register_buffer('xyz_max', xyz_max.clone())
        self._xyz_min_cpu, self._xyz_max_cpu = xyz_min.clone(), xyz_max.clone()

    def _alloc_k0(self, ws, device=None):
        g = torch.zeros([1, self.k0_dim, *ws], device=device)
        if self.channels_last and self.k0_dim > 1:
            g = g.contiguous(memory_format=torch.channels_last_3d)
        return g

    def _grid_xyz(self, ws, device):
        return torch.stack(torch.meshgrid(
            *[torch.linspace(float(self._xyz_min_cpu[a]), float(self._xyz_max_cpu[a]), ws[a], device=device)
              for a in range(3)], indexing='ij'), -1)

    def _resize_grids(self):
        ws = tuple(int(v) for v in self.world_size)
        self.density = nn.Parameter(F.interpolate(self.density.data, size=ws, mode='trilinear', align_corners=True))
        k0 = F.interpolate(self.k0.data.contiguous(), size=ws, mode='trilinear', align_corners=True)
        if self.channels_last and self.k0_dim > 1:
            k0 = k0.contiguous(memory_format=torch.channels_last_3d)
        self.k0 = nn.Parameter(k0)
        return ws

    def _pooled_alpha(self):
        return F.max_pool3d(self.activate_density(self.density), kernel_size=3, padding=1, stride=1)

    def _alpha_mask(self):
        return self._pooled_alpha()[0, 0] > self.fast_color_thres

    def _coarse_mask(self, ws, device):
        coarse = MaskCache(path=self.mask_cache_path, mask_cache_thres=self.mask_cache_thres).to(device)
        return coarse(self._grid_xyz(ws, device))

    def _set_mask_cache(self, mask):
        self.mask_cache = MaskCache(path=None, mask=mask.cpu(), xyz_min=self._xyz_min_cpu,
                                    xyz_max=self._xyz_max_cpu).to(self.density.device)
        self._cfg_cache = {}

    def _init_mask_cache(self, ws, mask_cache_path, mask_cache_thres):
        self.mask_cache_path, self.mask_cache_thres = mask_cache_path, mask_cache_thres
        if mask_cache_path:
            mask = self._coarse_mask(ws, torch.device('cuda', torch.cuda.current_device()))
        else:
            mask = torch.ones(ws, dtype=torch.bool)
        self._set_mask_cache(mask)

    def _init_colour(self, ws, rgbnet_dim, feat_dim, viewbase_pe, rgbnet_width, rgbnet_depth):
        if rgbnet_dim <= 0:
            self.k0_dim, self.rgbnet = 3, None
        else:
            self.k0_dim = rgbnet_dim
            self.register_buffer('viewfreq', _freqs(viewbase_pe))
            self.rgbnet = make_rgbnet(feat_dim + (3 + 3 * viewbase_pe * 2), rgbnet_width, rgbnet_depth)
        self.k0 = nn.Parameter(self._alloc_k0(ws))

    def _fused_head(self, viewdirs):
        return self.fused and self.fused_shade and viewdirs.is_cuda and viewdirs.dim() == 2

    def _shade(self, k0, viewdirs, ray_id, m_dev=None):
        if self.rgbnet is None:
            return torch.sigmoid(k0)
        if self.rgbnet_direct:
            k0_view = k0
        else:
            k0_view = k0[:, 3:]
            k0_diffuse = k0[:, :3]
        if self._fused_head(viewdirs):
            rgb = shade(self.rgbnet, k0, viewdir_embed(viewdirs, self.viewfreq), ray_id, diffuse=not self.rgbnet_direct,
                        m_dev=m_dev)
            if rgb is not None:
                return rgb
        assert m_dev is None, 'capacity mode needs the fused colour head'
        viewdirs_emb = _posenc(viewdirs, self.viewfreq).flatten(0, -2)[ray_id]
        rgb_logit = mlp_forward(self.rgbnet, torch.cat([k0_view, viewdirs_emb], -1))
        if self.rgbnet_direct:
            return torch.sigmoid(rgb_logit)
        return torch.sigmoid(rgb_logit + k0_diffuse)

    def _shade_posenc(self, pts, viewdirs, ray_id):
        if self._fused_head(viewdirs):
            rgb = shade_posenc(self.rgbnet, pts, viewdir_embed(viewdirs, self.viewfreq), ray_id, self.posfreq)
            if rgb is not None:
                return rgb
        viewdirs_emb = _posenc(viewdirs, self.viewfreq).flatten(0, -2)[ray_id]
        return torch.sigmoid(mlp_forward(self.rgbnet, torch.cat([_posenc(pts, self.posfreq), viewdirs_emb], -1)))

    def _tv_weights(self, weight):
        w = weight * float(self.world_size.max()) / 128
        return w, w, w

    def density_total_variation_add_grad(self, weight, dense_mode, x_range=None):
        total_variation_add_grad(self.density, self.density.grad, *self._tv_weights(weight), dense_mode, x_range)

    def k0_total_variation_add_grad(self, weight, dense_mode, x_range=None):
        total_variation_add_grad(self.k0, self.k0.grad, *self._tv_weights(weight), dense_mode, x_range)

    def activate_density(self, density, interval=None):
        interval = interval if interval is not None else self.voxel_size_ratio
        shape = density.shape
        return Raw2Alpha.apply(density.flatten().contiguous(), self.act_shift, interval).reshape(shape)

    def grid_sampler(self, xyz, *grids, **_unused):
        ret = [grid_sample(g, xyz, self.xyz_min, self.xyz_max) for g in grids]
        return ret[0] if len(ret) == 1 else ret

    def forward(self, rays_o, rays_d, viewdirs, global_step=None, **render_kwargs):
        assert len(rays_o.shape) == 2 and rays_o.shape[-1] == 3, 'Only suuport point queries in [N, 3] format'
        if self.fused:
            cfg = self._march_cfg(render_kwargs['near'], render_kwargs['far'], render_kwargs['stepsize'])
            return self._forward_fused(rays_o, rays_d, viewdirs, cfg, **render_kwargs)
        ray_pts, ray_id, step_id = self.sample_ray(rays_o=rays_o, rays_d=rays_d, is_train=global_step is not None,
                                                   **render_kwargs)
        if self.mask_cache is not None:
            mask = self.mask_cache(ray_pts)
            ray_pts, ray_id, step_id = ray_pts[mask], ray_id[mask], step_id[mask]
        return self._forward_unfused(len(rays_o), viewdirs, render_kwargs['stepsize'], render_kwargs['bg'],
                                     render_kwargs.get('render_depth', False), ray_pts, ray_id, step_id)

    def _forward_fused(self, rays_o, rays_d, viewdirs, cfg, bg, render_depth=False, _capacity=False, **_unused):
        N = len(rays_o)
        _capacity = bool(_capacity) and self.can_keep_count_on_device() and viewdirs.is_cuda and viewdirs.dim() == 2
        if self.uses_posenc:
            weights, alpha, alphainv_last, pts, ray_id, step_id, off3 = fused_march(
                self.density, self.k0.detach()[:, :0], rays_o, rays_d, cfg, positions=True)
            m_dev = None
            rgb = self._shade_posenc(pts, viewdirs, ray_id)
        else:
            weights, alpha, alphainv_last, k0, ray_id, step_id, off3 = fused_march(
                self.density, self.k0, rays_o, rays_d, cfg, capacity=_capacity)
            m_dev = off3[N:] if _capacity else None
            rgb = self._shade(k0, viewdirs, ray_id, m_dev)
        rgb_marched = composite(weights, rgb, alphainv_last, ray_id, off3, bg, m_dev)
        ret = _result(alphainv_last, weights, rgb_marched, alpha, rgb, ray_id)
        if _capacity:
            ret['n_samples'] = m_dev
        if render_depth:
            ret['depth'] = composite_depth(weights.detach(), step_id, off3, N)
        return ret

    def _forward_unfused(self, N, viewdirs, stepsize, bg, render_depth, pts, ray_id, *carried):
        alpha = self.activate_density(self.grid_sampler(pts, self.density), stepsize * self.voxel_size_ratio)
        if self.fast_color_thres > 0:
            mask = alpha > self.fast_color_thres
            pts, ray_id, *carried = [x[mask] for x in (pts, ray_id, *carried)]
            alpha = alpha[mask]
        weights, alphainv_last = Alphas2Weights.apply(alpha, ray_id, N)
        if self.fast_color_thres > 0:
            mask = weights > self.fast_color_thres
            weights, alpha = weights[mask], alpha[mask]
            pts, ray_id, *carried = [x[mask] for x in (pts, ray_id, *carried)]
        if self.uses_posenc:
            rgb = self._shade_posenc(pts, viewdirs, ray_id)
        else:
            rgb = self._shade(self.grid_sampler(pts, self.k0), viewdirs, ray_id)
        return self._sum_rays(N, weights, alpha, alphainv_last, rgb, ray_id, bg, render_depth, *carried)

    def _sum_rays(self, N, weights, alpha, alphainv_last, rgb, ray_id, bg, render_depth, step_id):
        rgb_marched = segment_coo(src=(weights.unsqueeze(-1) * rgb), index=ray_id,
                                  out=torch.zeros([N, 3], device=weights.device), reduce='sum')
        rgb_marched = rgb_marched + alphainv_last.unsqueeze(-1) * bg
        ret = _result(alphainv_last, weights, rgb_marched, alpha, rgb, ray_id)
        if render_depth:
            with torch.no_grad():
                ret['depth'] = segment_coo(src=(weights * step_id), index=ray_id,
                                           out=torch.zeros([N], device=weights.device), reduce='sum')
        return ret
```

### include/dvgo_hip.h

```cpp
#ifndef DVGO_HIP_H
#define DVGO_HIP_H

#include <stdint.h>

#ifdef __cplusplus
extern "C" {
#endif

#define DVGO_EINVAL (-1)
#define DVGO_ERANGE (-2)

#define DVGO_ABI_VERSION 11
int dvgo_abi_version(void);

#define DVGO_TUNE_FEAT_BWD    0
#define DVGO_TUNE_DENSITY_BWD 1
#define DVGO_TUNE_DENSITY_FWD 2
#define DVGO_TUNE_GATHER      3
#define DVGO_TUNE_EXPERIMENT  4
#define DVGO_TUNE_COUNT       8
int dvgo_set_tuning(int key, int value);

int dvgo_infer_t_minmax(const float* rays_o, const float* rays_d,
                        const float* xyz_min, const float* xyz_max,
                        float near, float far, int64_t n_rays,
                        float* t_min, float* t_max, void* stream);

int dvgo_infer_n_samples(const float* t_min, const float* t_max, float stepdist,
                         int64_t n_rays, int64_t* n_samples, void* stream);

int dvgo_infer_ray_start_dir(const float* rays_o, const float* rays_d, const float* t_min,
                             int64_t n_rays, float* rays_start, float* rays_dir, void* stream);

int dvgo_sample_pts_prepare(const float* rays_o, const float* rays_d,
                            const float* xyz_min, const float* xyz_max,
                            float near, float far, float stepdist, int64_t n_rays,
                            float* t_min, float* t_max,
                            int64_t* n_steps,
                            int64_t* n_steps_cumsum,
                            float* rays_start, float* rays_dir,
                            void* stream);

int dvgo_sample_pts_fill(const float* rays_start, const float* rays_dir,
                         const float* xyz_min, const float* xyz_max,
                         const int64_t* n_steps_cumsum, int64_t n_rays,
                         float stepdist, int64_t total_len,
                         float* rays_pts,
                         uint8_t* mask_outbbox,
                         int64_t* ray_id, int64_t* step_id,
                         void* stream);

int dvgo_sample_ndc_pts_on_rays(const float* rays_o, const float* rays_d,
                                const float* xyz_min, const float* xyz_max,
                                int n_samples, int64_t n_rays,
                                float* rays_pts, uint8_t* mask_outbbox, void* stream);

int dvgo_maskcache_lookup(const uint8_t* world, const float* xyz,
                          const float* xyz2ijk_scale, const float* xyz2ijk_shift,
                          int sz_i, int sz_j, int sz_k, int64_t n_pts,
                          uint8_t* out, void* stream);

int dvgo_raw2alpha(const float* density, float shift, float interval, int64_t n_pts,
                   float* exp_d, float* alpha, void* stream);
int dvgo_raw2alpha_backward(const float* exp_d, const float* grad_back, float interval,
                            int64_t n_pts, float* grad, void* stream);

int dvgo_alpha2weight(const float* alpha, const int64_t* ray_id, int64_t n_pts, int64_t n_rays,
                      float* weight, float* T, float* alphainv_last,
                      int64_t* i_start, int64_t* i_end, void* stream);
int dvgo_alpha2weight_backward(const float* alpha, const float* weight, const float* T,
                               const float* alphainv_last, const int64_t* i_start,
                               const int64_t* i_end, int64_t n_rays, int64_t n_pts,
                               const float* grad_weights, const float* grad_last,
                               float* grad , void* stream);

int dvgo_grid_sample_fwd(const float* grid, int C, int X, int Y, int Z,
                         int64_t sC, int64_t sX, int64_t sY, int64_t sZ,
                         const float* xyz, const float* xyz_min, const float* xyz_max,
                         int64_t M, float* out, void* stream);
int dvgo_grid_sample_bwd(const float* grad_out, int C, int X, int Y, int Z,
                         int64_t sC, int64_t sX, int64_t sY, int64_t sZ,
                         const float* xyz, const float* xyz_min, const float* xyz_max,
                         int64_t M, float* grad_grid, void* stream);

int dvgo_segment_sum(const float* src, const int64_t* index, int64_t M, int C,
                     int64_t N, float* out, void* stream);

typedef struct { int32_t step; float exp_d; float alpha; float T; } dvgo_rec2_t;

int dvgo_march_density(float* rays_start, float* rays_dir,
                       int64_t* n_steps, const int64_t* n_steps_cumsum, int64_t rec_stride,
                       int64_t n_rays,
                       const float* xyz_min, const float* xyz_max, float stepdist,
                       const uint8_t* mask, int mX, int mY, int mZ,
                       const float* xyz2ijk_scale, const float* xyz2ijk_shift,
                       const float* density, int X, int Y, int Z,
                       float act_shift, float interval, float fast_color_thres,
                       dvgo_rec2_t* rec2,
                       int32_t* n2, int32_t* n3, float* alphainv_last,
                       int32_t* brick_cnt ,
                       const float* rays_o, const float* rays_d, float near, float far
                                          ,
                       int32_t* tail_ticket ,
                       int64_t* off3, int n_bricks, int32_t* brick_off, int32_t* brick_cursor, int32_t* extra_off,
                       int32_t* active, int32_t* extra_brick, int n_extra_max, int slice_len,
                       void* stream);

int dvgo_march_hit(const float* rays_start, const float* rays_dir, const int64_t* n_steps, int64_t n_rays,
                   const float* xyz_min, const float* xyz_max, float stepdist,
                   const uint8_t* mask, int mX, int mY, int mZ,
                   const float* xyz2ijk_scale, const float* xyz2ijk_shift, uint8_t* hit, void* stream);

int dvgo_exclusive_scan_i32(const int32_t* counts, int64_t n, int64_t* offsets, void* stream);

int dvgo_march_gather(const dvgo_rec2_t* rec2, const int32_t* n2, const int64_t* n_steps, const int64_t* n_steps_cumsum,
                      int64_t rec_stride, const int64_t* off3, int64_t n_rays, int64_t M3,
                      const float* rays_start, const float* rays_dir, float stepdist,
                      const float* xyz_min, const float* xyz_max,
                      const float* k0, int C, int X, int Y, int Z,
                      int64_t sC, int64_t sX, int64_t sY, int64_t sZ,
                      int64_t* ray_id, int64_t* step_id, float* weights, float* alpha,
                      float* feat, void* stream);

int dvgo_march_composite(const float* weights, const float* rgb ,
                         const int64_t* step_id, const int64_t* off3, int64_t n_rays,
                         const float* alphainv_last, float bg,
                         float* rgb_marched , float* depth ,
                         void* stream);

int dvgo_march_composite_bwd(const float* grad_rgb_marched , const float* weights,
                             const float* rgb, const int64_t* ray_id, int64_t M3, const int64_t* m_dev, int64_t n_rays,
                             float bg, float* grad_weights , float* grad_rgb ,
                             float* grad_last, int accumulate, void* stream);

int dvgo_march_feat_bwd(const float* grad_feat, const float* grad_extra, const int64_t* ray_id, const int64_t* step_id,
                        int64_t M3, const float* rays_start, const float* rays_dir, float stepdist,
                        const float* xyz_min, const float* xyz_max,
                        int C, int X, int Y, int Z, int64_t sC, int64_t sX, int64_t sY, int64_t sZ,
                        float* grad_k0, void* stream);

int dvgo_march_density_bwd(const dvgo_rec2_t* rec2, const int32_t* n2, const int64_t* n_steps,
                           const int64_t* n_steps_cumsum, int64_t rec_stride, const int64_t* off3,
                           int64_t n_rays,
                           const float* rays_start, const float* rays_dir, float stepdist,
                           const float* xyz_min, const float* xyz_max,
                           const float* alphainv_last, float interval,
                           const float* grad_weights , const float* grad_last ,
                           int X, int Y, int Z, float* grad_density, int64_t grad_stride, float* grad_kept,
                           int32_t* brick_cursor, void* brick_recs,
                           void* stream);

int dvgo_march_ray_bwd(const dvgo_rec2_t* rec2, const int32_t* n2, const int64_t* n_steps,
                       const int64_t* n_steps_cumsum, int64_t rec_stride, const int64_t* off3, int64_t n_rays,
                       const float* rays_start, const float* rays_dir, float stepdist,
                       const float* xyz_min, const float* xyz_max, const float* alphainv_last, float interval,
                       const float* rays_o, const float* rays_d, float near, float far,
                       const float* density, int X, int Y, int Z,
                       const float* k0, int C, int64_t sC, int64_t sX, int64_t sY, int64_t sZ,
                       const float* grad_weights , const float* grad_last ,
                       const float* grad_feat , float* grad_o, float* grad_d, void* stream);

int dvgo_n_bricks(int X, int Y, int Z);
int dvgo_brick_slice(void);
int dvgo_brick_scan(int32_t* brick_cnt, int n_bricks, int32_t* brick_off, int32_t* brick_cursor, int32_t* extra_off,
                    int32_t* active, int32_t* extra_brick , int n_extra_max, int slice_len, void* stream);
int dvgo_march_scans(const int32_t* n3, int64_t n_rays, int64_t* off3, int32_t* brick_cnt, int n_bricks,
                     int32_t* brick_off, int32_t* brick_cursor, int32_t* extra_off, int32_t* active, int32_t* extra_brick,
                     int n_extra_max, int slice_len, void* stream);
int dvgo_brick_accumulate(const int32_t* brick_off, const int32_t* extra_off, const int32_t* active,
                          const int32_t* extra_brick, int32_t* arrive, float* scratch, int64_t n_extra_max, int slice_len,
                          const void* recs, const float* rays_start, const float* rays_dir,
                          float stepdist, const float* xyz_min, const float* xyz_max, const float* grad_feat,
                          int C, int X, int Y, int Z, float* grad_k0, float* grad_density,
                          float* p_k0, float* m_k0, float* v_k0, float step_size_k0, int masked_k0,
                          float* p_density, float* m_density, float* v_density, float step_size_density,
                          int masked_density, float beta1, float beta2, float eps,
                          const float* step_sizes_dev ,
                          float* tiles, int tiles_mode
                                      ,
                          void* stream);

int dvgo_grid_grad_split(const float* G, int64_t n_vox, int row_stride, int C, float* grad_k0, float* grad_density,
                         void* stream);

int dvgo_view_weight_accumulate(const float* rays_o, const float* rays_d, int64_t n_rays, const float* xyz_min,
                                const float* xyz_max, float near, float far, float step, int n_samples, int X, int Y,
                                int Z, float* acc, void* stream);
int dvgo_view_count_commit(float* acc, float* count, int64_t n_vox, void* stream);
int dvgo_rays_of_view(int H, int W, const float* K4, const float* c2w, int inverse_y, int flip_x, int flip_y, int center,
                      int ndc, float ndc_focal, float ndc_near, int64_t p0, int64_t n,
                      float* rays_o, float* rays_d, float* viewdirs, void* stream);
int dvgo_maskout_near_cam(float* density, const float* grid_x, const float* grid_y, const float* grid_z, int X, int Y, int Z,
                          const float* cam_o, int n_cam, float near, float value, void* stream);

int dvgo_shade_fwd(const float* feat, int C, const float* emb, int E, const int64_t* ray_id, int64_t M, const int64_t* m_dev,
                   const float* W1, const float* b1, const float* W2, const float* b2,
                   const float* W3, const float* b3, int width, int d_in, int diffuse,
                   float* rgb, float* H1, float* H2, uint64_t* masks,
                   void* scratch ,
                   void* scratch_bwd ,
                   void* stream);

int64_t dvgo_shade_scratch_bytes(int width);
int dvgo_shade_variant(int flags);

int dvgo_shade_bwd(const float* g_rgb, const float* rgb, const uint64_t* masks, int64_t M, const int64_t* m_dev,
                   const float* W1, const float* W2, const float* W3, int width, int d_in, int C, int diffuse,
                   float* g_feat, float* G1, float* gz, void* scratch,
                   int prebuilt ,
                   void* stream);

int dvgo_shade_wgrad(const float* G1, const float* gz, const uint64_t* masks, const float* W3,
                     const float* H1, const float* H2, const float* feat, int C, const float* emb, int E, const int64_t* ray_id, int64_t M,
                     const int64_t* m_dev, int width, int diffuse, int n_parts, float* part, float* total, void* stream);

int dvgo_march_positions(const float* rays_start, const float* rays_dir, const int64_t* ray_id, const int64_t* step_id,
                         int64_t M, float stepdist, float* pts, void* stream);
int dvgo_shade_pe_fwd(const float* pts, const float* freq, int P, const float* emb, int E, const int64_t* ray_id, int64_t M,
                      const float* W1, const float* b1, const float* W2, const float* b2, const float* W3, const float* b3,
                      int width, int d_in, float* rgb, float* H1, float* H2, uint64_t* masks, void* stream);
int dvgo_shade_pe_bwd(const float* g_rgb, const float* rgb, const uint64_t* masks, int64_t M, const float* W2,
                      const float* W3, int width, float* G1, float* gz, void* stream);
int64_t dvgo_shade_pe_record_size(int width, int d_in);
int dvgo_shade_pe_wgrad(const float* G1, const float* gz, const uint64_t* masks, const float* W3, const float* H1,
                        const float* H2, const float* pts, const float* freq, int P, const float* emb, int E,
                        const int64_t* ray_id, int64_t M, int width, int d_in, int n_parts, float* part, float* total,
                        void* stream);

int dvgo_adam_upd(float* param, const float* grad, float* exp_avg, float* exp_avg_sq,
                  const float* perlr , int64_t n, float step_size,
                  float beta1, float beta2, float eps, int mode, void* stream);

int dvgo_adam_rows(const float* G, int64_t n_vox, int row_stride, int C,
                   float* p_k0, float* m_k0, float* v_k0, float step_size_k0, int mode_k0,
                   float* p_density, float* m_density, float* v_density, float step_size_density, int mode_density,
                   float beta1, float beta2, float eps, void* stream);

int dvgo_total_variation_add_grad(const float* param, float* grad, float wx, float wy, float wz,
                                  int64_t C, int64_t sz_i, int64_t sz_j, int64_t sz_k,
                                  int64_t sC, int64_t sI, int64_t sJ, int64_t sK,
                                  int dense_mode, void* stream);
int dvgo_total_variation_add_grad_slab(const float* param, float* grad, float wx, float wy, float wz,
                                       int64_t C, int64_t sz_i, int64_t sz_j, int64_t sz_k, int64_t sC,
                                       int64_t sI, int64_t sJ, int64_t sK, int dense_mode, int64_t i_lo, int64_t i_hi,
                                       void* stream);

int dvgo_loss_fwd_bwd(const float* rgb_marched, const float* alphainv_last, const float* target, int64_t N,
                      const float* raw_rgb, const float* weights, const int64_t* ray_id, int64_t M, const int64_t* m_dev,
                      int64_t n_rays_global, float w_main, float w_ent, float w_per,
                      float* g_marched, float* g_last, float* g_raw_rgb, float* loss_out, void* stream);
int dvgo_copy_multi(void* const* dst, const void* const* src, const int64_t* n_dwords, int n_tensors, void* stream);
int dvgo_viewdir_embed(const float* viewdirs, const float* freq, int n_freq, int64_t N, float* emb, void* stream);
int dvgo_adam_upd_multi(float* const* params, const float* const* grads, float* const* exp_avg,
                        float* const* exp_avg_sq, const int64_t* numel, int n_tensors, float step_size,
                        float beta1, float beta2, float eps,
                        const float* step_size_dev , void* stream);

int64_t dvgo_image_metrics_workspace_bytes(int64_t n, int H, int W, int filter_size);
int dvgo_image_metrics(const float* img0, const float* img1, int64_t n, int H, int W, const double* taps, int filter_size,
                       double c1, double c2, double* ssim_sum, double* sse, float* ssim_map,
                       void* workspace, int64_t workspace_bytes, void* stream);

int dvgo_mesh_field(const float* density, int X, int Y, int Z, const uint8_t* mask, int MX, int MY, int MZ,
                    const float* mask_scale, const float* mask_shift, int Rx, int Ry, int Rz, const float* g0,
                    const float* gs, const float* box_min, const float* spacing, int copy, float iso, float* field,
                    void* stream);
int dvgo_mesh_count(const float* field, int Px, int Py, int Pz, float iso, uint8_t* edge_mask, uint32_t* partials,
                    uint32_t* bases, void* stream);
int dvgo_mesh_emit(const float* field, const uint8_t* edge_mask, const uint32_t* bases, int Px, int Py, int Pz,
                   float iso, const float* box_min, const float* spacing, int64_t n_verts, int64_t n_faces,
                   float* verts, float* normals, int32_t* faces, void* stream);

int dvgo_contract_count(const float* rays_o, const float* rays_d, int64_t n_rays, const float* center,
                        const float* radius, const float* t_tab, int n_max, float bg_len, int l2, float thres,
                        const uint8_t* mask, int mi, int mj, int mk, const float* mask_scale,
                        const float* mask_shift, int32_t* counts, void* stream);
int dvgo_contract_emit(const float* rays_o, const float* rays_d, int64_t n_rays, const float* center,
                       const float* radius, const float* t_tab, int n_max, float bg_len, int l2, float thres,
                       const uint8_t* mask, int mi, int mj, int mk, const float* mask_scale, const float* mask_shift,
                       const int64_t* offsets, float* q, int64_t* ray_id, int64_t* step_id, float* t,
                       void* stream);
int dvgo_distortion_fwd_bwd(const float* w, const float* s, const int64_t* ray_id, int64_t m, int64_t n_rays,
                            int64_t n_norm, int n_max, float* grad, double* partials, unsigned int* ticket,
                            float* loss, void* stream);

int dvgo_triplane_fwd(const float* xy, int H_xy, int W_xy, int64_t sC_xy, int64_t sH_xy, int64_t sW_xy,
                      const float* yz, int H_yz, int W_yz, int64_t sC_yz, int64_t sH_yz, int64_t sW_yz,
                      const float* zx, int H_zx, int W_zx, int64_t sC_zx, int64_t sH_zx, int64_t sW_zx,
                      int C, const float* xyz, const float* xyz_min, const float* xyz_max, int64_t M, int sum,
                      float* out, void* stream);
int dvgo_triplane_bwd(const float* grad_out,
                      float* g_xy, int H_xy, int W_xy, int64_t sC_xy, int64_t sH_xy, int64_t sW_xy,
                      float* g_yz, int H_yz, int W_yz, int64_t sC_yz, int64_t sH_yz, int64_t sW_yz,
                      float* g_zx, int H_zx, int W_zx, int64_t sC_zx, int64_t sH_zx, int64_t sW_zx,
                      int C, const float* xyz, const float* xyz_min, const float* xyz_max, int64_t M, int sum,
                      int run, void* stream);

int dvgo_grid_sample_bwd_xyz(const float* grid, int C, int X, int Y, int Z,
                             int64_t sC, int64_t sX, int64_t sY, int64_t sZ,
                             const float* grad_out, const float* xyz, const float* xyz_min, const float* xyz_max,
                             int64_t M, float* grad_xyz, void* stream);

int dvgo_liif_gather(const float* xy, int H_xy, int W_xy, int64_t sC_xy, int64_t sH_xy, int64_t sW_xy,
                     const float* yz, int H_yz, int W_yz, int64_t sC_yz, int64_t sH_yz, int64_t sW_yz,
                     const float* zx, int H_zx, int W_zx, int64_t sC_zx, int64_t sH_zx, int64_t sW_zx,
                     int C, const float* xyz, const float* xyz_min, const float* xyz_max, int64_t M,
                     int Wx, int Wy, int Wz, int cell_decode, int local_ensemble, float* inp, float* wgt, void* stream);
int dvgo_liif_scatter(const float* grad_inp,
                      float* g_xy, int H_xy, int W_xy, int64_t sC_xy, int64_t sH_xy, int64_t sW_xy,
                      float* g_yz, int H_yz, int W_yz, int64_t sC_yz, int64_t sH_yz, int64_t sW_yz,
                      float* g_zx, int H_zx, int W_zx, int64_t sC_zx, int64_t sH_zx, int64_t sW_zx,
                      int C, const float* xyz, const float* xyz_min, const float* xyz_max, int64_t M,
                      int Wx, int Wy, int Wz, int cell_decode, int local_ensemble, int run, void* stream);
int dvgo_liif_blend_fwd(const float* pred, const float* wgt, int C, int64_t M, int E, int sum, float* out, void* stream);
int dvgo_liif_blend_bwd(const float* grad_out, const float* wgt, int C, int64_t M, int E, int sum, float* grad_pred,
                        void* stream);

int dvgo_plane_rows_fwd(const float* xy, int H_xy, int W_xy, int64_t sC_xy, int64_t sH_xy, int64_t sW_xy,
                        const float* yz, int H_yz, int W_yz, int64_t sC_yz, int64_t sH_yz, int64_t sW_yz,
                        const float* zx, int H_zx, int W_zx, int64_t sC_zx, int64_t sH_zx, int64_t sW_zx,
                        int C, const float* xyz, const float* xyz_min, const float* xyz_max, int64_t M,
                        int Wx, int Wy, int Wz, int P, int cell_decode, float* inp, void* stream);
int dvgo_plane_rows_bwd(const float* grad_inp,
                        float* g_xy, int H_xy, int W_xy, int64_t sC_xy, int64_t sH_xy, int64_t sW_xy,
                        float* g_yz, int H_yz, int W_yz, int64_t sC_yz, int64_t sH_yz, int64_t sW_yz,
                        float* g_zx, int H_zx, int W_zx, int64_t sC_zx, int64_t sH_zx, int64_t sW_zx,
                        int C, const float* xyz, const float* xyz_min, const float* xyz_max, int64_t M,
                        int Wx, int Wy, int Wz, int P, int cell_decode, int run, void* stream);

int dvgo_vm_fwd(const float* xy, int H_xy, int W_xy, int64_t sC_xy, int64_t sH_xy, int64_t sW_xy,
                const float* yz, int H_yz, int W_yz, int64_t sC_yz, int64_t sH_yz, int64_t sW_yz,
                const float* zx, int H_zx, int W_zx, int64_t sC_zx, int64_t sH_zx, int64_t sW_zx,
                const float* l_xy, int N_xy, int64_t lC_xy, int64_t lN_xy,
                const float* l_yz, int N_yz, int64_t lC_yz, int64_t lN_yz,
                const float* l_zx, int N_zx, int64_t lC_zx, int64_t lN_zx,
                int R, const float* xyz, const float* xyz_min, const float* xyz_max, int64_t M, float* out, void* stream);
int dvgo_vm_bwd(const float* grad_out,
                const float* xy, int H_xy, int W_xy, int64_t sC_xy, int64_t sH_xy, int64_t sW_xy,
                const float* yz, int H_yz, int W_yz, int64_t sC_yz, int64_t sH_yz, int64_t sW_yz,
                const float* zx, int H_zx, int W_zx, int64_t sC_zx, int64_t sH_zx, int64_t sW_zx,
                const float* l_xy, int N_xy, int64_t lC_xy, int64_t lN_xy,
                const float* l_yz, int N_yz, int64_t lC_yz, int64_t lN_yz,
                const float* l_zx, int N_zx, int64_t lC_zx, int64_t lN_zx,
                float* g_xy, float* g_yz, float* g_zx, float* gl_xy, float* gl_yz, float* gl_zx,
                int R, const float* xyz, const float* xyz_min, const float* xyz_max, int64_t M, int run, int mode,
                void* stream);

int dvgo_plane_reg_add_grad(const float* const* params, float* const* grads, const int64_t* sizes,
                            const int64_t* strides, const float* weights, int n_tensors, int dense_mode, void* stream);

#define DVGO_HASH_MAX_LEVELS 32
int dvgo_hash_fwd(const float* table, int F, int L, const int32_t* res, const int64_t* offsets, const float* xyz,
                  const float* xyz_min, const float* xyz_max, int64_t M, float* out, void* stream);
int dvgo_hash_bwd(const float* grad_out, float* grad_table, int F, int L, const int32_t* res, const int64_t* offsets,
                  const float* xyz, const float* xyz_min, const float* xyz_max, int64_t M, int run, int mode, void* stream);

#ifdef __cplusplus
}
#endif
#endif
```

Baseline: 3.159 million.

## Precompute per-ray bf16x3 embedding fragments for fused shading forward

The view-direction embedding kernel now also writes, once per ray, the three-way bf16 split fragments of the MLP input. The x3 shading forward kernel loads these fragments by ray id instead of gathering and splitting the embedding for every sample. Only the feature slice is split per sample, using vector loads. This removes repeated per-sample split arithmetic and scattered embedding loads, at the cost of an extra fragment buffer, more layout constraints (16-byte alignment, n_view limits) and wave-level syncs in the tile store.

```diff
diff --git a/directvoxgo_amd/_lib.py b/directvoxgo_amd/_lib.py
--- a/directvoxgo_amd/_lib.py
+++ b/directvoxgo_amd/_lib.py
@@ -147,17 +147,21 @@
     return {n: (len(ev), sum(a.elapsed_time(b) for a, b in ev)) for n, ev in (prof or {}).items()}
 
 
+_TIMED_AS = {'dvgo_shade_fwd_frags': 'dvgo_shade_fwd'}
+
+
 def call(name, *args):
     handle = lib()
     if len(args) != _nargs.get(name):
         raise TypeError(f'{name}: {len(args)} arguments given, include/dvgo_hip.h declares {_nargs.get(name, "no such function")}')
     fn = getattr(handle, name)
-    if _profile is not None and name in _profile:
+    timed = _TIMED_AS.get(name, name)
+    if _profile is not None and timed in _profile:
         a, b = torch.cuda.Event(enable_timing=True), torch.cuda.Event(enable_timing=True)
         a.record()
         rc = fn(*args)
         b.record()
-        _profile[name].append((a, b))
+        _profile[timed].append((a, b))
     else:
         rc = fn(*args)
     if rc != 0:
diff --git a/directvoxgo_amd/csrc/loss.hip b/directvoxgo_amd/csrc/loss.hip
--- a/directvoxgo_amd/csrc/loss.hip
+++ b/directvoxgo_amd/csrc/loss.hip
@@ -1,4 +1,5 @@
 #include "common.h"
+#include "x3.h"
 
 __device__ __forceinline__ float block_sum_256(float v, float* red) {
 #pragma unroll
@@ -66,6 +67,14 @@
   if (threadIdx.x == 0) atomicAdd(loss_out, t);
 }
 
+__device__ __forceinline__ float viewdir_embed_value(const float* __restrict__ viewdirs, const float* __restrict__ freq, int F,
+                                                     int64_t r, int e) {
+  if (e < 3) return viewdirs[3 * r + e];
+  const int q = (e - 3) % (3 * F);
+  const float a = viewdirs[3 * r + q / F] * freq[q % F];
+  return (e - 3 < 3 * F) ? sinf(a) : cosf(a);
+}
+
 __global__ void __launch_bounds__(256)
 viewdir_embed_kernel(const float* __restrict__ viewdirs, const float* __restrict__ freq, int F, int64_t N,
                      float* __restrict__ emb) {
@@ -73,15 +82,31 @@
   const int64_t t = (int64_t)blockIdx.x * blockDim.x + threadIdx.x;
   if (t >= N * E) return;
   const int64_t r = t / E;
-  const int e = (int)(t - r * E);
-  float v;
-  if (e < 3) v = viewdirs[3 * r + e];
-  else {
-    const int q = (e - 3) % (3 * F);
-    const float a = viewdirs[3 * r + q / F] * freq[q % F];
-    v = (e - 3 < 3 * F) ? sinf(a) : cosf(a);
-  }
-  emb[t] = v;
+  emb[t] = viewdir_embed_value(viewdirs, freq, F, r, (int)(t - r * E));
+}
+
+template <bool COMPUTE>
+__global__ void __launch_bounds__(256)
+embed_frags_kernel(const float* __restrict__ viewdirs, const float* __restrict__ freq, int F, const float* __restrict__ emb_in,
+                   int E, int64_t N, int n_view, int ks1, float* __restrict__ emb, unsigned int* __restrict__ frags) {
+  const int64_t t = (int64_t)blockIdx.x * blockDim.x + threadIdx.x;
+  if (t >= N * ks1 * 8) return;
+  const int64_t r = t / (8 * ks1);
+  const int k0 = 2 * (int)(t - r * 8 * ks1);
+  float v[2];
+#pragma unroll
+  for (int j = 0; j < 2; ++j) {
+    const int e = k0 + j - n_view;
+    v[j] = 0.0f;
+    if (e >= 0 && e < E) {
+      if (COMPUTE) emb[r * E + e] = v[j] = viewdir_embed_value(viewdirs, freq, F, r, e);
+      else v[j] = emb_in[r * E + e];
+    }
+  }
+  unsigned int w0, w1, w2;
+  x3_split2(v[0], v[1], w0, w1, w2);
+  unsigned int* f = frags + ((t >> 2) * 3) * 4 + (t & 3);
+  f[0] = w0; f[4] = w1; f[8] = w2;
 }
 
 #define DVGO_MT_MAX 16
@@ -182,6 +207,33 @@
   return 0;
 }
 
+static bool embed_frags_ok(int64_t N, int E, int n_view, int ks1, const void* emb, const void* frags) {
+  return N >= 0 && E >= 0 && n_view >= 0 && (ks1 == 1 || ks1 == 3) && n_view + E <= 16 * ks1 && (N == 0 || (emb && frags)) &&
+         (((uintptr_t)frags) & 15u) == 0;
+}
+
+int dvgo_viewdir_embed_frags(const float* viewdirs, const float* freq, int n_freq, int64_t N, int n_view, int ks1, float* emb,
+                             void* frags, void* stream) {
+  if (n_freq < 0 || !embed_frags_ok(N, 3 + 6 * n_freq, n_view, ks1, emb, frags)) return DVGO_EINVAL;
+  if (N == 0) return 0;
+  if (!viewdirs || (n_freq > 0 && !freq)) return DVGO_EINVAL;
+  if (!dvgo_fits(N * ks1 * 8)) return DVGO_ERANGE;
+  embed_frags_kernel<true><<<dvgo_blocks(N * ks1 * 8, 256), 256, 0, (hipStream_t)stream>>>(viewdirs, freq, n_freq, nullptr, 3 + 6 * n_freq, N,
+                                                                                         n_view, ks1, emb, (unsigned int*)frags);
+  DVGO_LAUNCH_CHECK();
+  return 0;
+}
+
+int dvgo_shade_embed_frags(const float* emb, int E, int64_t N, int n_view, int ks1, void* frags, void* stream) {
+  if (!embed_frags_ok(N, E, n_view, ks1, emb, frags)) return DVGO_EINVAL;
+  if (N == 0) return 0;
+  if (!dvgo_fits(N * ks1 * 8)) return DVGO_ERANGE;
+  embed_frags_kernel<false><<<dvgo_blocks(N * ks1 * 8, 256), 256, 0, (hipStream_t)stream>>>(nullptr, nullptr, 0, emb, E, N, n_view, ks1, nullptr,
+                                                                                          (unsigned int*)frags);
+  DVGO_LAUNCH_CHECK();
+  return 0;
+}
+
 int dvgo_adam_upd_multi(float* const* params, const float* const* grads, float* const* exp_avg,
                         float* const* exp_avg_sq, const int64_t* numel, int n_tensors, float step_size, float beta1,
                         float beta2, float eps, const float* step_size_dev, void* stream) {
diff --git a/directvoxgo_amd/csrc/shade.hip b/directvoxgo_amd/csrc/shade.hip
--- a/directvoxgo_amd/csrc/shade.hip
+++ b/directvoxgo_amd/csrc/shade.hip
@@ -14,10 +14,10 @@
                                  const float* W1, const float* W2, const float* W3, int width, int d_in, int C, int diffuse,
                                  float* g_feat, float* G1, float* gz, void* scratch, int prebuilt, void* stream);
 
-extern "C" int dvgo_shade_fwd_x3(const float* feat, int C, const float* emb, int E, const int64_t* ray_id, int64_t M, const int64_t* m_dev,
-                                 const float* W1, const float* b1, const float* W2, const float* b2, const float* W3,
-                                 const float* b3, int width, int d_in, int diffuse, float* rgb, float* H1, float* H2,
-                                 uint64_t* masks, void* scratch, void* scratch_bwd, int experiment, void* stream);
+extern "C" int dvgo_shade_fwd_x3f(const float* feat, int C, const float* emb, int E, const void* frags, const int64_t* ray_id,
+                                  int64_t M, const int64_t* m_dev, const float* W1, const float* b1, const float* W2, const float* b2,
+                                  const float* W3, const float* b3, int width, int d_in, int diffuse, float* rgb, float* H1,
+                                  float* H2, uint64_t* masks, void* scratch, void* scratch_bwd, int experiment, void* stream);
 
 #define SHADE_THREADS 768
 #define SHADE_WAVES (SHADE_THREADS / 64)
@@ -1064,10 +1064,10 @@
 
 extern "C" {
 
-int dvgo_shade_fwd(const float* feat, int C, const float* emb, int E, const int64_t* ray_id, int64_t M, const int64_t* m_dev,
-                   const float* W1, const float* b1, const float* W2, const float* b2, const float* W3,
-                   const float* b3, int width, int d_in, int diffuse, float* rgb, float* H1, float* H2,
-                   uint64_t* masks, void* scratch, void* scratch_bwd, void* stream) {
+int dvgo_shade_fwd_frags(const float* feat, int C, const float* emb, int E, const void* emb_frags, const int64_t* ray_id, int64_t M,
+                         const int64_t* m_dev, const float* W1, const float* b1, const float* W2, const float* b2, const float* W3,
+                         const float* b3, int width, int d_in, int diffuse, float* rgb, float* H1, float* H2,
+                         uint64_t* masks, void* scratch, void* scratch_bwd, void* stream) {
   if (M < 0 || C <= 0 || E < 0) return DVGO_EINVAL;
   if (M == 0) return 0;
   if (!feat || !emb || !ray_id || !W1 || !b1 || !W2 || !b2 || !W3 || !b3 || !rgb) return DVGO_EINVAL;
@@ -1077,8 +1077,9 @@
   if (n_view < 0 || d_in != n_view + E) return DVGO_EINVAL;
   if ((width != 128 && width != 64) || d_in > 40) return DVGO_ERANGE;
   if ((g_shade_variant & 1) && scratch != nullptr)
-    return dvgo_shade_fwd_x3(feat, C, emb, E, ray_id, M, m_dev, W1, b1, W2, b2, W3, b3, width, d_in, diffuse, rgb, H1, H2, masks,
-                             scratch, (g_shade_variant & 2) ? scratch_bwd : nullptr, g_shade_experiment, stream);
+    return dvgo_shade_fwd_x3f(feat, C, emb, E, (g_shade_variant & 128) ? nullptr : emb_frags, ray_id, M, m_dev, W1, b1, W2, b2, W3, b3,
+                              width, d_in, diffuse, rgb, H1, H2, masks, scratch, (g_shade_variant & 2) ? scratch_bwd : nullptr,
+                              g_shade_experiment, stream);
   hipStream_t s = (hipStream_t)stream;
   const int64_t n_tiles = (M + 31) / 32;
   const int64_t cap = width == 128 ? 256 : 512;
@@ -1096,6 +1097,14 @@
 #undef DVGO_SHADE
   DVGO_LAUNCH_CHECK();
   return 0;
+}
+
+int dvgo_shade_fwd(const float* feat, int C, const float* emb, int E, const int64_t* ray_id, int64_t M, const int64_t* m_dev,
+                   const float* W1, const float* b1, const float* W2, const float* b2, const float* W3,
+                   const float* b3, int width, int d_in, int diffuse, float* rgb, float* H1, float* H2,
+                   uint64_t* masks, void* scratch, void* scratch_bwd, void* stream) {
+  return dvgo_shade_fwd_frags(feat, C, emb, E, nullptr, ray_id, M, m_dev, W1, b1, W2, b2, W3, b3, width, d_in, diffuse, rgb, H1, H2,
+                              masks, scratch, scratch_bwd, stream);
 }
 
 int dvgo_shade_experiment(int flags) { g_shade_experiment = flags; return 0; }
diff --git a/directvoxgo_amd/csrc/shade_x3.hip b/directvoxgo_amd/csrc/shade_x3.hip
--- a/directvoxgo_amd/csrc/shade_x3.hip
+++ b/directvoxgo_amd/csrc/shade_x3.hip
@@ -46,6 +46,12 @@
   for (int i = threadIdx.x; i < (int)(sizeof(Img) / 16); i += blockDim.x) l[i] = g[i];
 }
 
+__device__ __forceinline__ void x3_wave_sync() {
+  __builtin_amdgcn_fence(__ATOMIC_RELEASE, "wavefront");
+  __builtin_amdgcn_wave_barrier();
+  __builtin_amdgcn_fence(__ATOMIC_ACQUIRE, "wavefront");
+}
+
 __device__ __forceinline__ void x3_store_tile(float* __restrict__ stage, const f32x16& acc, float* __restrict__ dst, int row_stride,
                                               int lane, int rows_valid) {
   const int smp = lane & 31, h = lane >> 5;
@@ -57,6 +63,7 @@
         *reinterpret_cast<float4*>(stage + (smp & 15) * X3_STAGE_STRIDE + 8 * q + 4 * h) =
             make_float4(acc[4 * q], acc[4 * q + 1], acc[4 * q + 2], acc[4 * q + 3]);
     }
+    x3_wave_sync();
     const int c = lane & 7;
 #pragma unroll
     for (int i = 0; i < 2; ++i) {
@@ -65,6 +72,7 @@
       const int r = 16 * half + rl;
       if (r < rows_valid) *reinterpret_cast<float4*>(dst + (int64_t)r * row_stride + 4 * c) = v;
     }
+    x3_wave_sync();
   }
 }
 
@@ -108,9 +116,12 @@
   if (tid < 4) L.b3[tid] = tid < 3 ? b3[tid] : 0.0f;
 }
 
-template <int WIDTH, int KS1, bool DIFFUSE>
+__host__ __device__ __forceinline__ int64_t x3_frag_index(int64_t ray, int ks1, int s, int h) { return ((ray * ks1 + s) * 2 + h) * 3; }
+
+template <int WIDTH, int KS1, bool DIFFUSE, bool FRAGS>
 __global__ void __launch_bounds__(X3_THREADS)
 shade_fwd_x3_kernel(const float* __restrict__ feat, int C, int c_view0, int n_view, const float* __restrict__ emb, int E,
+                    const u32x4* __restrict__ frags,
                     const int64_t* __restrict__ ray_id, int64_t M_cap, const int64_t* __restrict__ m_dev,
                     const void* __restrict__ image, float* __restrict__ rgb,
                     float* __restrict__ H1, float* __restrict__ H2, unsigned long long* __restrict__ masks, int experiment) {
@@ -128,12 +139,12 @@
   const int d_in = n_view + E;
   const int64_t last = M > 0 ? M - 1 : 0;
   auto row_of = [&](int64_t tile) { const int64_t r = tile * 32 + (lane & 31); return r < M ? r : last; };
-  float xin[KS1][8];
+  float xin[FRAGS ? 1 : KS1][8];
   auto load_inputs = [&](int64_t tile, int64_t rid) {
     const float* fr = feat + row_of(tile) * C + c_view0;
     const float* er = emb + rid * E - n_view;
 #pragma unroll
-    for (int s = 0; s < KS1; ++s)
+    for (int s = 0; s < (FRAGS ? 0 : KS1); ++s)
 #pragma unroll
       for (int j = 0; j < 8; ++j) {
         const int k = 16 * s + 8 * h + j;
@@ -141,22 +152,53 @@
         xin[s][j] = *((kc < n_view) ? fr + kc : er + kc);
       }
   };
+  const bool f_lo = 8 * h < n_view, f_hi = 8 * h + 4 < n_view;
+  const int fo_lo = f_lo ? 8 * h : 0, fo_hi = f_hi ? 8 * h + 4 : 0;
+  float4 fq[2];
+  u32x4 x3[KS1][3];
+  auto load_feat = [&](int64_t tile) {
+    const float* fr = feat + row_of(tile) * C + c_view0;
+    fq[0] = *reinterpret_cast<const float4*>(fr + fo_lo);
+    fq[1] = *reinterpret_cast<const float4*>(fr + fo_hi);
+  };
+  auto load_frags = [&](int64_t rid) {
+    const u32x4* fp = frags + x3_frag_index(rid, KS1, 0, h);
+#pragma unroll
+    for (int s = 0; s < KS1; ++s)
+#pragma unroll
+      for (int q = 0; q < 3; ++q) x3[s][q] = fp[6 * s + q];
+  };
   int64_t rid_n = 0;
-  if (gw < n_tiles) { load_inputs(gw, ray_id[row_of(gw)]); rid_n = ray_id[row_of(gw + nw)]; }
+  if (gw < n_tiles) {
+    if (FRAGS) { load_feat(gw); load_frags(ray_id[row_of(gw)]); }
+    else load_inputs(gw, ray_id[row_of(gw)]);
+    rid_n = ray_id[row_of(gw + nw)];
+  }
   for (int64_t tile = gw; tile < n_tiles; tile += nw) {
     const int64_t row = tile * 32 + (lane & 31);
     const bool valid = row < M;
     const int rows_valid = (int)(M - tile * 32 < 32 ? M - tile * 32 : 32);
-    u32x4 x3[KS1][3];
-#pragma unroll
-    for (int s = 0; s < KS1; ++s) {
-      float v[8];
-#pragma unroll
-      for (int j = 0; j < 8; ++j) v[j] = (16 * s + 8 * h + j) < d_in ? xin[s][j] : 0.0f;
-      x3_split8(v, x3[s][0], x3[s][1], x3[s][2]);
-    }
-    load_inputs(tile + nw, rid_n);
-    rid_n = ray_id[row_of(tile + 2 * nw)];
+    if (FRAGS) {
+      const float v[8] = {fq[0].x, fq[0].y, fq[0].z, fq[0].w, fq[1].x, fq[1].y, fq[1].z, fq[1].w};
+      u32x4 f3[3];
+      x3_split8(v, f3[0], f3[1], f3[2]);
+#pragma unroll
+      for (int q = 0; q < 3; ++q) {
+        x3[0][q][0] = f_lo ? f3[q][0] : x3[0][q][0]; x3[0][q][1] = f_lo ? f3[q][1] : x3[0][q][1];
+        x3[0][q][2] = f_hi ? f3[q][2] : x3[0][q][2]; x3[0][q][3] = f_hi ? f3[q][3] : x3[0][q][3];
+      }
+      load_feat(tile + nw);
+    } else {
+#pragma unroll
+      for (int s = 0; s < KS1; ++s) {
+        float v[8];
+#pragma unroll
+        for (int j = 0; j < 8; ++j) v[j] = (16 * s + 8 * h + j) < d_in ? xin[FRAGS ? 0 : s][j] : 0.0f;
+        x3_split8(v, x3[s][0], x3[s][1], x3[s][2]);
+      }
+      load_inputs(tile + nw, rid_n);
+      rid_n = ray_id[row_of(tile + 2 * nw)];
+    }
     u32x4 h3[2 * T][3];
     unsigned long long mask1 = 0ull;
 #pragma unroll
@@ -183,6 +225,11 @@
         for (int j = 0; j < 8; ++j) v[j] = acc[8 * s2 + j];
         x3_split8(v, h3[2 * t + s2][0], h3[2 * t + s2][1], h3[2 * t + s2][2]);
       }
+      __builtin_amdgcn_sched_barrier(0);
+    }
+    if (FRAGS) {
+      load_frags(rid_n);
+      rid_n = ray_id[row_of(tile + 2 * nw)];
       __builtin_amdgcn_sched_barrier(0);
     }
     float p[3] = {0.0f, 0.0f, 0.0f};
@@ -1106,10 +1153,21 @@
   return 0;
 }
 
-int dvgo_shade_fwd_x3(const float* feat, int C, const float* emb, int E, const int64_t* ray_id, int64_t M, const int64_t* m_dev,
-                      const float* W1, const float* b1, const float* W2, const float* b2, const float* W3,
-                      const float* b3, int width, int d_in, int diffuse, float* rgb, float* H1, float* H2,
-                      uint64_t* masks, void* scratch, void* scratch_bwd, int experiment, void* stream) {
+int dvgo_shade_frags_usable(int width, int C, int diffuse, int E) {
+  const int c_view0 = diffuse ? 3 : 0, n_view = C - c_view0;
+  if ((width != 128 && width != 64) || E < 0 || n_view + E > 48) return 0;
+  return (n_view % 4 == 0 && n_view >= 4 && n_view <= 16 && C % 4 == 0 && c_view0 % 4 == 0) ? 1 : 0;
+}
+
+int dvgo_shade_frag_ksteps(int width, int d_in) {
+  if (d_in < 0 || d_in > 48) return 0;
+  return width == 128 ? 3 : width == 64 ? (d_in <= 16 ? 1 : 3) : 0;
+}
+
+int dvgo_shade_fwd_x3f(const float* feat, int C, const float* emb, int E, const void* frags, const int64_t* ray_id, int64_t M,
+                       const int64_t* m_dev, const float* W1, const float* b1, const float* W2, const float* b2, const float* W3,
+                       const float* b3, int width, int d_in, int diffuse, float* rgb, float* H1, float* H2,
+                       uint64_t* masks, void* scratch, void* scratch_bwd, int experiment, void* stream) {
   if (M < 0 || C <= 0 || E < 0) return DVGO_EINVAL;
   if (M == 0) return 0;
   if (!feat || !emb || !ray_id || !W1 || !b1 || !W2 || !b2 || !W3 || !b3 || !rgb || !scratch) return DVGO_EINVAL;
@@ -1118,21 +1176,27 @@
   const int n_view = C - c_view0;
   if (n_view < 0 || d_in != n_view + E) return DVGO_EINVAL;
   if ((width != 128 && width != 64) || d_in > 48) return DVGO_ERANGE;
+  const bool fast = frags != nullptr && dvgo_shade_frags_usable(width, C, diffuse, E) != 0;
+  if (fast && ((((uintptr_t)feat) | ((uintptr_t)frags)) & 15u)) return DVGO_EINVAL;
   hipStream_t s = (hipStream_t)stream;
   const int64_t n_tiles = (M + 31) / 32;
   const int64_t cap = 256;
   const int blocks = (int)((n_tiles + X3_WAVES - 1) / X3_WAVES < cap ? (n_tiles + X3_WAVES - 1) / X3_WAVES : cap);
-#define DVGO_SHADE_X3(W, KS, DIFF)                                                                                       \
+#define DVGO_SHADE_X3(W, KS, DIFF, FR)                                                                                   \
   do {                                                                                                                   \
     x3_prep_fwd_kernel<W, KS><<<scratch_bwd ? 64 : 32, 256, 0, s>>>((X3Img<W, KS>*)scratch, (X3BwdImg<W>*)scratch_bwd, W1, b1, W2, b2, W3, b3, d_in); \
-    shade_fwd_x3_kernel<W, KS, DIFF><<<blocks, X3_THREADS, 0, s>>>(feat, C, c_view0, n_view, emb, E, ray_id, M, m_dev, scratch, rgb, \
-                                                                    H1, H2, (unsigned long long*)masks, experiment);     \
+    shade_fwd_x3_kernel<W, KS, DIFF, FR><<<blocks, X3_THREADS, 0, s>>>(feat, C, c_view0, n_view, emb, E, (const u32x4*)frags, ray_id, M, m_dev, \
+                                                                        scratch, rgb, H1, H2, (unsigned long long*)masks, experiment); \
   } while (0)
-  if (width == 128) {
-    if (diffuse) DVGO_SHADE_X3(128, 3, true); else DVGO_SHADE_X3(128, 3, false);
+  if (fast) {
+    if (width == 128) DVGO_SHADE_X3(128, 3, false, true);
+    else if (d_in <= 16) DVGO_SHADE_X3(64, 1, false, true);
+    else DVGO_SHADE_X3(64, 3, false, true);
+  } else if (width == 128) {
+    if (diffuse) DVGO_SHADE_X3(128, 3, true, false); else DVGO_SHADE_X3(128, 3, false, false);
   } else {
-    if (d_in <= 16) { if (diffuse) DVGO_SHADE_X3(64, 1, true); else DVGO_SHADE_X3(64, 1, false); }
-    else            { if (diffuse) DVGO_SHADE_X3(64, 3, true); else DVGO_SHADE_X3(64, 3, false); }
+    if (d_in <= 16) { if (diffuse) DVGO_SHADE_X3(64, 1, true, false); else DVGO_SHADE_X3(64, 1, false, false); }
+    else            { if (diffuse) DVGO_SHADE_X3(64, 3, true, false); else DVGO_SHADE_X3(64, 3, false, false); }
   }
 #undef DVGO_SHADE_X3
   DVGO_LAUNCH_CHECK();
diff --git a/directvoxgo_amd/csrc/x3.h b/directvoxgo_amd/csrc/x3.h
--- a/directvoxgo_amd/csrc/x3.h
+++ b/directvoxgo_amd/csrc/x3.h
@@ -12,15 +12,20 @@
   return __builtin_bit_cast(unsigned int, __builtin_convertvector(v, bf16x2));
 }
 
+__device__ __forceinline__ void x3_split2(float a, float b, unsigned int& w0, unsigned int& w1, unsigned int& w2) {
+  const unsigned int h = x3_pack(a, b);
+  const float ra = a - __uint_as_float(h << 16), rb = b - __uint_as_float(h & 0xffff0000u);
+  const unsigned int m = x3_pack(ra, rb);
+  const float qa = ra - __uint_as_float(m << 16), qb = rb - __uint_as_float(m & 0xffff0000u);
+  w0 = h; w1 = m; w2 = x3_pack(qa, qb);
+}
+
 __device__ __forceinline__ void x3_split8(const float (&v)[8], u32x4& s0, u32x4& s1, u32x4& s2) {
 #pragma unroll
   for (int p = 0; p < 4; ++p) {
-    const float a = v[2 * p], b = v[2 * p + 1];
-    const unsigned int h = x3_pack(a, b);
-    const float ra = a - __uint_as_float(h << 16), rb = b - __uint_as_float(h & 0xffff0000u);
-    const unsigned int m = x3_pack(ra, rb);
-    const float qa = ra - __uint_as_float(m << 16), qb = rb - __uint_as_float(m & 0xffff0000u);
-    s0[p] = h; s1[p] = m; s2[p] = x3_pack(qa, qb);
+    unsigned int w0, w1, w2;
+    x3_split2(v[2 * p], v[2 * p + 1], w0, w1, w2);
+    s0[p] = w0; s1[p] = w1; s2[p] = w2;
   }
 }
 
diff --git a/directvoxgo_amd/shade.py b/directvoxgo_amd/shade.py
--- a/directvoxgo_amd/shade.py
+++ b/directvoxgo_amd/shade.py
@@ -62,6 +62,41 @@
     return emb
 
 
+def frag_layout(rgbnet, C, E, diffuse):
+    layers = head_layers(rgbnet)
+    n_view = C - (3 if diffuse else 0)
+    if layers is None or layers[0].in_features != n_view + E:
+        return None
+    lib = L.lib()
+    width = layers[0].out_features
+    if not lib.dvgo_shade_frags_usable(int(width), int(C), 1 if diffuse else 0, int(E)):
+        return None
+    return n_view, int(lib.dvgo_shade_frag_ksteps(int(width), int(n_view + E)))
+
+
+@torch.no_grad()
+def viewdir_embed_frags(viewdirs, viewfreq, layout):
+    n_view, ks1 = layout
+    N, F = viewdirs.shape[0], viewfreq.shape[0]
+    emb = torch.empty((N, 3 + 6 * F), dtype=torch.float32, device=viewdirs.device)
+    frags = torch.empty((N, ks1, 2, 3, 4), dtype=torch.int32, device=viewdirs.device)
+    with L.device_of(viewdirs):
+        L.call('dvgo_viewdir_embed_frags', ptr(viewdirs.contiguous()), ptr(viewfreq), _int(F), _i64(N), _int(n_view), _int(ks1),
+               ptr(emb), ptr(frags), stream_of(viewdirs))
+    return emb, frags
+
+
+@torch.no_grad()
+def embed_frags(emb, layout):
+    n_view, ks1 = layout
+    emb = emb.contiguous()
+    frags = torch.empty((emb.shape[0], ks1, 2, 3, 4), dtype=torch.int32, device=emb.device)
+    with L.device_of(emb):
+        L.call('dvgo_shade_embed_frags', ptr(emb), _int(emb.shape[1]), _i64(emb.shape[0]), _int(n_view), _int(ks1), ptr(frags),
+               stream_of(emb))
+    return frags
+
+
 def head_layers(rgbnet):
     layers = head_layers_any_din(rgbnet)
     if layers is None or layers[0].in_features > 40:
@@ -95,7 +130,7 @@
 
 class _Shade(torch.autograd.Function):
     @staticmethod
-    def forward(ctx, feat, emb, ray_id, W1, b1, W2, b2, W3, b3, diffuse, train, m_dev):
+    def forward(ctx, feat, emb, ray_id, W1, b1, W2, b2, W3, b3, diffuse, train, m_dev, emb_frags):
         M, C = feat.shape
         E = emb.shape[1]
         width, d_in = W1.shape
@@ -107,8 +142,10 @@
         masks = torch.empty((M, 4), dtype=torch.int64, device=feat.device) if train else None
         scratch = _scratch(width, feat.device)
         scratch_bwd = _scratch(width, feat.device) if (train and (L.lib().dvgo_shade_variant(-1) & 2)) else None
+        if emb_frags is not None and feat.data_ptr() % 16:
+            emb_frags = None
         with L.device_of(feat):
-            L.call('dvgo_shade_fwd', ptr(feat), _int(C), ptr(emb), _int(E), ptr(ray_id), _i64(M), ptr(m_dev), ptr(W1.contiguous()),
+            L.call('dvgo_shade_fwd_frags', ptr(feat), _int(C), ptr(emb), _int(E), ptr(emb_frags), ptr(ray_id), _i64(M), ptr(m_dev), ptr(W1.contiguous()),
                    ptr(b1.contiguous()), ptr(W2.contiguous()), ptr(b2.contiguous()), ptr(W3.contiguous()),
                    ptr(b3.contiguous()), _int(width), _int(d_in), _int(1 if diffuse else 0), ptr(rgb), ptr(H1), ptr(H2),
                    ptr(masks), ptr(scratch), ptr(scratch_bwd), stream_of(feat))
@@ -152,10 +189,10 @@
                        ptr(part), ptr(tot), stream_of(feat))
             return _unpack_record(tot, width, d_in)
 
-        return _weight_grads(ctx.params, wgrad, feat.device, 3, 12, g_feat if ctx.needs_input_grad[0] else None)
-
-
-def shade(rgbnet, feat, emb, ray_id, diffuse, m_dev=None):
+        return _weight_grads(ctx.params, wgrad, feat.device, 3, 13, g_feat if ctx.needs_input_grad[0] else None)
+
+
+def shade(rgbnet, feat, emb, ray_id, diffuse, m_dev=None, emb_frags=None):
     layers = head_layers(rgbnet)
     if layers is None or not feat.is_cuda:
         return None
@@ -164,7 +201,7 @@
     if l1.in_features != feat.shape[1] - c0 + emb.shape[1]:
         return None
     return _Shade.apply(feat, emb, ray_id, l1.weight, l1.bias, l2.weight, l2.bias, l3.weight, l3.bias, diffuse,
-                        torch.is_grad_enabled(), m_dev)
+                        torch.is_grad_enabled(), m_dev, emb_frags)
 
 
 def posenc_supported(rgbnet, n_freq, emb_dim):
diff --git a/directvoxgo_amd/voxel_model.py b/directvoxgo_amd/voxel_model.py
--- a/directvoxgo_amd/voxel_model.py
+++ b/directvoxgo_amd/voxel_model.py
@@ -5,7 +5,7 @@
 
 from .fused import composite, composite_depth, fused_march
 from .ops import Alphas2Weights, MaskCache, Raw2Alpha, grid_sample, segment_coo, total_variation_add_grad
-from .shade import shade, shade_posenc, viewdir_embed
+from .shade import frag_layout, shade, shade_posenc, viewdir_embed, viewdir_embed_frags
 
 
 def _as_f32(x):
@@ -150,8 +150,13 @@
             k0_view = k0[:, 3:]
             k0_diffuse = k0[:, :3]
         if self._fused_head(viewdirs):
-            rgb = shade(self.rgbnet, k0, viewdir_embed(viewdirs, self.viewfreq), ray_id, diffuse=not self.rgbnet_direct,
-                        m_dev=m_dev)
+            diffuse = not self.rgbnet_direct
+            layout = frag_layout(self.rgbnet, k0.shape[1], 3 + 6 * self.viewfreq.shape[0], diffuse)
+            if layout is None:
+                emb, frags = viewdir_embed(viewdirs, self.viewfreq), None
+            else:
+                emb, frags = viewdir_embed_frags(viewdirs, self.viewfreq, layout)
+            rgb = shade(self.rgbnet, k0, emb, ray_id, diffuse=diffuse, m_dev=m_dev, emb_frags=frags)
             if rgb is not None:
                 return rgb
         assert m_dev is None, 'capacity mode needs the fused colour head'
diff --git a/include/dvgo_hip.h b/include/dvgo_hip.h
--- a/include/dvgo_hip.h
+++ b/include/dvgo_hip.h
@@ -201,6 +201,14 @@
                    void* scratch_bwd ,
                    void* stream);
 
+int dvgo_shade_fwd_frags(const float* feat, int C, const float* emb, int E, const void* emb_frags, const int64_t* ray_id, int64_t M,
+                         const int64_t* m_dev, const float* W1, const float* b1, const float* W2, const float* b2,
+                         const float* W3, const float* b3, int width, int d_in, int diffuse,
+                         float* rgb, float* H1, float* H2, uint64_t* masks, void* scratch, void* scratch_bwd, void* stream);
+int dvgo_shade_frags_usable(int width, int C, int diffuse, int E);
+int dvgo_shade_frag_ksteps(int width, int d_in);
+int dvgo_shade_embed_frags(const float* emb, int E, int64_t N, int n_view, int ks1, void* frags, void* stream);
+
 int64_t dvgo_shade_scratch_bytes(int width);
 int dvgo_shade_variant(int flags);
 
@@ -251,6 +259,8 @@
                       float* g_marched, float* g_last, float* g_raw_rgb, float* loss_out, void* stream);
 int dvgo_copy_multi(void* const* dst, const void* const* src, const int64_t* n_dwords, int n_tensors, void* stream);
 int dvgo_viewdir_embed(const float* viewdirs, const float* freq, int n_freq, int64_t N, float* emb, void* stream);
+int dvgo_viewdir_embed_frags(const float* viewdirs, const float* freq, int n_freq, int64_t N, int n_view, int ks1, float* emb,
+                             void* frags, void* stream);
 int dvgo_adam_upd_multi(float* const* params, const float* const* grads, float* const* exp_avg,
                         float* const* exp_avg_sq, const int64_t* numel, int n_tensors, float step_size,
                         float beta1, float beta2, float eps,
```

Result: slower. 2.981 million (-5.7%).
